# z3lx/waifu2x-tensorrt

Measured on AMD Instinct MI355X. Metric: upscaled MPix/s, 1080p->4K swin_unet/art fp16, higher is better.
Workload: dtype f16; 1 GPU; configs[2]: swin_unet/art scale4 noise3 batch4 tile256 fp16, 1920x1080 frame, blend=0.0625 (45 tiles, 12 batches); synthetic-weight graph of that architecture, frame resident in HBM; frames_per_rank=132, parallelism=frame-sharded x1, no collectives; timing barrier over gloo, mode=frames, tiles_per_network_pass=48, tile_groups_per_pass=2

## Files before the change

include/w2x/c_api.h:

```cpp
#ifndef W2X_C_API_H
#define W2X_C_API_H

#include <stddef.h>
#include <stdint.h>

#ifdef __cplusplus
extern "C" {
#endif

typedef struct w2x_engine w2x_engine;

enum { W2X_PRECISION_TF32 = 0, W2X_PRECISION_FP16 = 1, W2X_PRECISION_FP32 = 2 };

enum { W2X_RESIZE_BICUBIC = 0, W2X_RESIZE_BILINEAR = 1 };
enum { W2X_YUV_BT601 = 0, W2X_YUV_BT709 = 1, W2X_YUV_BT2020 = 2 };
enum { W2X_YUV_LIMITED = 0, W2X_YUV_FULL = 1 };

typedef struct w2x_build_config {
    int deviceId, precision;
    int minBatchSize, optBatchSize, maxBatchSize;
    int minChannels, optChannels, maxChannels;
    int minWidth, optWidth, maxWidth;
    int minHeight, optHeight, maxHeight;
} w2x_build_config;
// ... 20 lines not shown
int w2x_render16_resized(w2x_engine* e, const uint16_t* src, int rows, int cols, size_t src_step, uint16_t* dst, int dst_rows, int dst_cols, size_t dst_step, int filter);
int w2x_render_strip(w2x_engine* e, const uint8_t* src, int rows, int cols, size_t src_step, uint8_t* dst, size_t dst_step, int part, int parts);
int w2x_render_sharded(w2x_engine* const* engines, int count, const uint8_t* src, int rows, int cols, size_t src_step, uint8_t* dst, size_t dst_step);
int w2x_shard_plan(int in_w, int in_h, int out_w, int out_h, int tile_in, int tile_out, int scaling, double overlap_x, double overlap_y,
                   int part, int parts, int* out16);
int w2x_shard_compute(w2x_engine* e, const uint8_t* src, int rows, int cols, size_t src_step, int part, int parts);
const void* w2x_shard_slab(w2x_engine* e, size_t* bytes);
int w2x_shard_finish(w2x_engine* e, uint8_t* dst, int out_rows, int out_cols, size_t dst_step, int part, int parts, const void* const* slabs, const int* devices);
int w2x_ipc_export(const void* device_ptr, uint8_t* out64);
void* w2x_ipc_open(const uint8_t* handle64, int device);
void w2x_ipc_close(void* p);
int w2x_render_sequence(w2x_engine* e, const uint8_t* const* srcs, int rows, int cols, size_t src_step, uint8_t* const* dsts, size_t dst_step, int count);
int w2x_render_sequence_resized(w2x_engine* e, const uint8_t* const* srcs, int rows, int cols, size_t src_step, uint8_t* const* dsts, int dst_rows, int dst_cols, size_t dst_step,
                                int count, int filter);
int w2x_render_yuv(w2x_engine* e, const void* const* src_planes, const size_t* src_steps, int rows, int cols, int src_bits,
                   void* const* dst_planes, const size_t* dst_steps, int dst_rows, int dst_cols, int dst_bits, int matrix, int range);
int w2x_render_sequence_yuv(w2x_engine* e, const void* const* src_planes, const size_t* src_steps, int rows, int cols, int src_bits,
                            void* const* dst_planes, const size_t* dst_steps, int dst_rows, int dst_cols, int dst_bits, int count, int matrix, int range);
int w2x_render_yuv_resized(w2x_engine* e, const void* const* src_planes, const size_t* src_steps, int rows, int cols, int src_bits,
                           void* const* dst_planes, const size_t* dst_steps, int dst_rows, int dst_cols, int dst_bits, int matrix, int range, int filter);
int w2x_render_sequence_yuv_resized(w2x_engine* e, const void* const* src_planes, const size_t* src_steps, int rows, int cols, int src_bits,
                                    void* const* dst_planes, const size_t* dst_steps, int dst_rows, int dst_cols, int dst_bits, int count, int matrix, int range, int filter);
int w2x_render_rgba(w2x_engine* e, const uint8_t* src, int rows, int cols, size_t src_step, uint8_t* dst, size_t dst_step, int bleed, int skip_uniform_alpha);
int w2x_alpha_bleed_device(w2x_engine* e, const uint8_t* bgra, int rows, int cols, size_t bgra_step, uint8_t* bgr, size_t bgr_step, int radius);
void* w2x_alloc_host(w2x_engine* e, size_t bytes);
void w2x_free_host(w2x_engine* e, void* data);
int w2x_pin_host(w2x_engine* e, void* data, size_t bytes);
void w2x_unpin_host(w2x_engine* e, void* data);
int w2x_strip_plan(int in_w, int in_h, int out_w, int out_h, int tile_in, int tile_out, int scaling, double overlap_x, double overlap_y,
                   int part, int parts, int* out4);
int w2x_infer(w2x_engine* e, const float* input_nchw, float* output_nchw);
int w2x_output_tile_size(w2x_engine* e);
double w2x_plan_flops(w2x_engine* e);
int w2x_pass_tiles(w2x_engine* e);
float w2x_last_render_ms(w2x_engine* e);
float w2x_bench_resident(w2x_engine* e, int iters);
int w2x_resident_output(w2x_engine* e, void* dst, size_t bytes);
int w2x_profile_frame(w2x_engine* e, double* out, int cap);
int w2x_op_times(w2x_engine* e, double* out, int cap);

int w2x_calculate_tiles(int in_w, int in_h, int out_w, int out_h, int tile_in, int tile_out, int scaling,
                        double overlap_x, double overlap_y, int* in_rects, int* out_rects, int cap);
int w2x_tile_weights(int which, int overlap_x, int overlap_y, int size, float* out);
int w2x_resize_weights(int in, int out, int filter, int* first, float* weights, int cap);
int w2x_yuv_plane_sizes(int rows, int cols, int bits, int* plane_rows, int* plane_cols, size_t* plane_bytes);
int w2x_alpha_bleed(const uint8_t* bgr, size_t bgr_step, const uint8_t* alpha, size_t alpha_step, int rows, int cols, int radius, uint8_t* out, size_t out_step);
int w2x_describe_plan(const char* onnx_path, int batch, int tile, char* buf, size_t cap);
int w2x_describe_plan_precision(const char* onnx_path, int batch, int tile, int precision, char* buf, size_t cap);
int w2x_write_engine_file(const char* onnx_path, int batch, int tile, const char* out_path);
int w2x_validate_engine_file(const char* path, char* buf, size_t cap);
enum { W2X_EXTENT_INTS = 25 };
int w2x_dead_skip_extents(const char* onnx_path, int batch, int tile, int in_w, int in_h, int scaling, double overlap_x, double overlap_y, int tile_index, int tta,
                          int* out, int cap);
int w2x_device_pci_bus_id(int device, char* buf, size_t cap);
void w2x_sha256_hex(const void* data, size_t len, char* out);
const char* w2x_version(void);
int w2x_debug_set(const char* name, int value);

#ifdef __cplusplus
}
#endif
#endif
```

waifu2x-tensorrt_amd/__init__.py:

```python
from .engine import (BuildConfig, RenderConfig, Img2Img, Precision, Severity, lib, lib_path,
                     calculate_tiles, strip_plan, shard_plan, render_sharded, device_pci_bus_id, ipc_open, ipc_close, tile_weights, resize_weights, yuv_plane_sizes, alpha_bleed, describe_plan, dead_skip_extents, write_engine_file, validate_engine_file, sha256_hex, W2xError,
                     debug_switches)

__all__ = ["BuildConfig", "RenderConfig", "Img2Img", "Precision", "Severity", "lib", "lib_path",
           "calculate_tiles", "strip_plan", "shard_plan", "render_sharded", "device_pci_bus_id", "ipc_open", "ipc_close", "tile_weights", "resize_weights", "yuv_plane_sizes", "alpha_bleed", "describe_plan", "dead_skip_extents", "write_engine_file", "validate_engine_file", "sha256_hex", "W2xError", "debug_switches"]
```

waifu2x-tensorrt_amd/csrc/c_api.cpp:

```cpp
#include "../../include/w2x/c_api.h"
#include <mutex>

#include <cstring>
#include <fstream>
#include <vector>
#include <string>

#include "../../include/w2x/img2img.h"
#include "liveness.h"
#include "lower.h"
#include "sha256.h"
#include "tiles.h"
#include "kernels.h"

struct w2x_engine {
    w2x::Img2Img engine;
    w2x_message_fn msg = nullptr; void* msg_user = nullptr;
    w2x_progress_fn prog = nullptr; void* prog_user = nullptr;
};

extern "C" {

w2x_engine* w2x_create(void) { try { return new w2x_engine; } catch (...) { return nullptr; } }
void w2x_destroy(w2x_engine* e) { delete e; }

void w2x_set_message_callback(w2x_engine* e, w2x_message_fn fn, void* user) {
    if (!e) return;
    e->msg = fn; e->msg_user = user;
    if (fn) e->engine.setMessageCallback([e](w2x::Severity s, const std::string& m) { if (e->msg) e->msg((int)s, m.c_str(), e->msg_user); });
    else e->engine.setMessageCallback(nullptr);
}
void w2x_set_progress_callback(w2x_engine* e, w2x_progress_fn fn, void* user) {
    if (!e) return;
    e->prog = fn; e->prog_user = user;
    if (fn) e->engine.setProgressCallback([e](int c, int t, double s) { if (e->prog) e->prog(c, t, s, e->prog_user); });
    else e->engine.setProgressCallback(nullptr);
}

int w2x_build(w2x_engine* e, const char* onnx_path, const w2x_build_config* c) {
    if (!e || !onnx_path || !c) return 0;
    w2x::BuildConfig b;
    b.deviceId = c->deviceId; b.precision = c->precision == W2X_PRECISION_FP16 ? w2x::Precision::FP16 : c->precision == W2X_PRECISION_FP32 ? w2x::Precision::FP32 : w2x::Precision::TF32;
    b.minBatchSize = c->minBatchSize; b.optBatchSize = c->optBatchSize; b.maxBatchSize = c->maxBatchSize;
    b.minChannels = c->minChannels; b.optChannels = c->optChannels; b.maxChannels = c->maxChannels;
    b.minWidth = c->minWidth; b.optWidth = c->optWidth; b.maxWidth = c->maxWidth;
    b.minHeight = c->minHeight; b.optHeight = c->optHeight; b.maxHeight = c->maxHeight;
    return e->engine.build(onnx_path, b) ? 1 : 0;
}

int w2x_load(w2x_engine* e, const char* onnx_path, const w2x_render_config* c) {
    if (!e || !onnx_path || !c) return 0;
    w2x::RenderConfig r;
    r.deviceId = c->deviceId; r.precision = c->precision == W2X_PRECISION_FP16 ? w2x::Precision::FP16 : c->precision == W2X_PRECISION_FP32 ? w2x::Precision::FP32 : w2x::Precision::TF32;
    r.batchSize = c->batchSize; r.channels = c->channels; r.height = c->height; r.width = c->width; r.scaling = c->scaling;
    r.overlapX = c->overlapX; r.overlapY = c->overlapY; r.tta = c->tta != 0; r.ttaBugCompat = c->ttaBugCompat != 0;
    return e->engine.load(onnx_path, r) ? 1 : 0;
}

int w2x_render(w2x_engine* e, const uint8_t* src, int rows, int cols, size_t src_step, uint8_t* dst, size_t dst_step) {
    if (!e) return 0;
    w2x::Image s; s.data = const_cast<uint8_t*>(src); s.rows = rows; s.cols = cols; s.step = src_step;
    w2x::Image d; d.data = dst; d.step = dst_step;
    const int sc = e->engine.scaling();
    d.rows = rows * sc; d.cols = cols * sc;
    return e->engine.render(s, d) ? 1 : 0;
}
// ... 258 lines not shown
        if (!f.is_open()) return 0;
        f.write((const char*)bytes.data(), (std::streamsize)bytes.size());
        return f.good() ? 1 : 0;
    } catch (const std::exception&) { return 0; }
}

int w2x_device_pci_bus_id(int device, char* buf, size_t cap) { return buf && cap >= 16 && w2x::device_pci_bus_id(device, buf, cap) ? 1 : 0; }

void w2x_sha256_hex(const void* data, size_t len, char* out) {
    std::string h = w2x::sha256_hex(data, len);
    memcpy(out, h.c_str(), 65);
}

const char* w2x_version(void) { return "w2x-hip 0.1 (gfx950)"; }

int w2x_dead_skip_extents(const char* onnx_path, int batch, int tile, int in_w, int in_h, int scaling, double overlap_x, double overlap_y, int tile_index, int tta,
                          int* out, int cap) {
    try {
        static std::mutex mu;
        static std::string key;
        static w2x::Plan plan;
        std::lock_guard<std::mutex> lock(mu);
        const std::string k = std::string(onnx_path ? onnx_path : "") + "|" + std::to_string(batch) + "|" + std::to_string(tile);
        if (k != key) { plan = w2x::build_plan(onnx_path, batch, 3, tile, tile, false); plan.userB = batch; key = k; }
        const int nops = (int)plan.ops.size();
        if (!out || cap < nops * W2X_EXTENT_INTS) return -nops;
        int kept_w = plan.Tout, kept_h = plan.Tout;
        bool all = tta != 0 || tile_index < 0 || w2x::switches().no_dead_skip;
        if (tile_index >= 0) {
            const w2x::TileGrid g = w2x::calculate_tiles(in_w, in_h, in_w * scaling, in_h * scaling, tile, tile, plan.Tout, plan.Tout, scaling, overlap_x, overlap_y);
            if (tile_index >= g.count) return 0;
            kept_w = g.out[tile_index].w; kept_h = g.out[tile_index].h;
        }
        const std::vector<w2x::OpExtent> ext = w2x::dead_skip_extents(plan, kept_w, kept_h, all);
        for (int i = 0; i < nops; ++i) {
            const w2x::Op& op = plan.ops[i]; const w2x::OpExtent& e = ext[i];
            int* o = out + (size_t)i * W2X_EXTENT_INTS;
            int in_t = -1, out_t = -1, res_t = -1, kh = 1, kw = 1, stride = 1, x0 = 0, y0 = 0, r = 1;
            if (op.kind == w2x::OP_GEMM) {
                in_t = op.g.a.t; out_t = op.g.out.t; res_t = op.g.res.t; x0 = op.g.a.x0; y0 = op.g.a.y0;
                if (op.g.amode == w2x::A_CONV) { kh = op.g.kh; kw = op.g.kw; stride = op.g.stride; }
                if (op.g.omode == w2x::O_PIXSHUF) r = op.g.r;
            } else if (op.kind == w2x::OP_MLP) { in_t = op.m.x; out_t = op.m.y; }
            else if (op.kind == w2x::OP_SWINATTN) { in_t = op.sa.x; out_t = op.sa.y; }
            auto dim = [&](int t, bool w) { return t >= 0 && t < (int)plan.tensors.size() ? (w ? plan.tensors[t].W : plan.tensors[t].H) : 0; };
            const int v[W2X_EXTENT_INTS] = {op.kind, e.x.n, e.y.n, e.x.c, e.x.w, e.y.c, e.y.w, e.rx, e.ry, e.ws, in_t, out_t, res_t, kh, kw, stride, x0, y0, r,
                                            dim(in_t, true), dim(in_t, false), dim(out_t, true), dim(out_t, false), (int)e.live_units(), (int)e.total_units()};
            for (int k = 0; k < W2X_EXTENT_INTS; ++k) o[k] = v[k];
        }
        return nops;
    } catch (const std::exception&) { return 0; }
}

int w2x_debug_set(const char* name, int value) { return w2x::set_switch(name, value) ? 1 : 0; }

}
```

waifu2x-tensorrt_amd/csrc/engine.cpp:

```cpp
#include <hip/hip_runtime.h>
#include <dlfcn.h>

#include <algorithm>
#include <array>
#include <chrono>
#include <cmath>
#include <cstdio>
#include <cstdlib>
#include <cstring>
#include <deque>
#include <filesystem>
#include <fstream>
#include <map>
#include <sstream>
#include <tuple>

#include "../../include/w2x/img2img.h"
#include "common.h"
#include "fragorder.h"
#include "kernels.h"
#include "liveness.h"
#include "lower.h"
#include "plan.h"
#include "sha256.h"
#include "switches.h"
#include "tiles.h"

#define W2X_LOG(sev, message) impl->log(sev, message, __FUNCTION__, __LINE__)
#define W2X_LOG_AS(who, sev, message) impl->log(sev, message, who, __LINE__)

namespace w2x {

namespace {

inline void hipAssert(hipError_t e) {
    if (e != hipSuccess) throw std::runtime_error(hipGetErrorString(e));
}

std::string hipGetDeviceName(int deviceId) {
    hipDeviceProp_t prop{};
    hipAssert(hipGetDeviceProperties(&prop, deviceId));
    std::string arch = prop.gcnArchName;
    return arch + " x" + std::to_string(prop.multiProcessorCount);
}

int physical_device(int logical) {
    std::vector<int> map;
    if (const char* e = getenv("W2X_DEVICE_MAP")) { std::stringstream ss(e); std::string tok; while (std::getline(ss, tok, ',')) if (!tok.empty()) map.push_back(atoi(tok.c_str())); }
    return logical >= 0 && logical < (int)map.size() ? map[logical] : logical;
}

struct DeviceGuard {
    int prev = -1, dev = -1;
    explicit DeviceGuard(int d) : dev(d) {
        if (d < 0) return;
        if (hipGetDevice(&prev) != hipSuccess) { (void)hipGetLastError(); prev = -1; }
        if (prev != d) hipAssert(hipSetDevice(d));
    }
    ~DeviceGuard() { if (dev >= 0 && prev >= 0 && prev != dev) (void)hipSetDevice(prev); }
    DeviceGuard(const DeviceGuard&) = delete;
    DeviceGuard& operator=(const DeviceGuard&) = delete;
};

std::string device_ordinal_problem(int logical, int physical) {
    int count = 0;
    if (hipGetDeviceCount(&count) != hipSuccess) { (void)hipGetLastError(); count = 0; }
    if (count <= 0) return "no HIP device is visible to this process (hipGetDeviceCount = 0): this library has no CPU path";
    if (physical >= 0 && physical < count) return "";
    std::string m = "device id " + std::to_string(logical);
    if (physical != logical) m += " (W2X_DEVICE_MAP -> " + std::to_string(physical) + ")";
    return m + " does not exist: this process sees " + std::to_string(count) + " HIP device" + (count == 1 ? "" : "s") + " (valid ids 0.." + std::to_string(count - 1) + ")";
}

}
bool device_pci_bus_id(int deviceId, char* buf, size_t cap) {
    const int dev = physical_device(deviceId);
// ... 101 lines not shown
    void log(Severity s, const std::string& m) { if (messageCallback) messageCallback(s, m); }
    void log(Severity s, const std::string& m, const std::string& fn, int line) { if (messageCallback) messageCallback(s, "[" + fn + "@" + std::to_string(line) + "] " + m); }
    void log(int current, int total, double speed) { if (progressCallback) progressCallback(current, total, speed); }

    bool loaded = false;
    int device = -1;
    bool poison = false;
    bool check_general = false;
    bool use_graphs = true;
    Plan plan;
    RenderConfig cfg;
    hipStream_t stream = nullptr;
    hipEvent_t ev0 = nullptr, ev1 = nullptr;
    int (*roctx_push)(const char*) = nullptr; int (*roctx_pop)() = nullptr;
    hipEvent_t ev_shard = nullptr;
    static constexpr int kMaxRenderParts = 4;
    hipEvent_t ev_part[kMaxRenderParts] = {nullptr, nullptr, nullptr, nullptr};
    int pipeline_parts = 3;
    size_t shard_halo_slots = 0;
    int shard_rows = 0, shard_cols = 0;
    hipStream_t gstream[3] = {nullptr, nullptr, nullptr};
    hipEvent_t ev_fork = nullptr, ev_join[3] = {nullptr, nullptr, nullptr};
    int groups = 2;
    std::vector<void*> tensors, blobs;
    std::vector<void*> frag_blobs;
    std::vector<void*> perm_blobs;
    std::vector<int> pool_blocks;
    void* arena_base = nullptr; size_t arena_bytes = 0;
    std::vector<GemmParams> gemm;
    int final_op = -1;
    enum LaunchKind { L_OP, L_HEAD, L_STEM, L_UP, L_MLP32, L_ATTN32 };
    struct Launch {
        LaunchKind kind = L_OP;
        int first = 0, last = 0;
        int timed = 0;
        double flops = 0;
        int family = 0;
        std::array<void*, 4> planes{{nullptr, nullptr, nullptr, nullptr}};
    };
    std::vector<Launch> launches;

    bool deep = false;
    uint8_t* d_frame = nullptr; size_t frame_cap = 0;
    uint8_t* d_out = nullptr; size_t out_cap = 0;
    void* d_slab = nullptr; size_t slab_cap = 0;
    void* d_slab2 = nullptr; size_t slab2_cap = 0;
    hipEvent_t ev_g0[2] = {nullptr, nullptr}, ev_cmp[2] = {nullptr, nullptr};
    bool rolling = false;
    bool rolling_ok = true;
    TileSlot* d_slots = nullptr; size_t slots_cap = 0;
    LiveExt* d_live = nullptr; size_t live_cap = 0, live_stride = 0;
    std::vector<LiveExt> h_live;
    std::map<std::pair<int, int>, std::vector<OpExtent>> live_cache;
    void upload_live(const TileGrid& grid, size_t count, hipStream_t on) {
        const size_t nops = plan.ops.size();
        if (!count || !nops) return;
        if (count > live_stride) {
            ensure(d_live, live_cap, (nops * count + 8) * sizeof(LiveExt));
            live_stride = count;
        }
        const bool all = switches().no_dead_skip || check_general || cfg.tta;
        std::map<std::pair<int, int>, int> tile_at;
        if (!all) for (int t = 0; t < grid.count; ++t) tile_at[{grid.in[t].x, grid.in[t].y}] = t;
        auto extents = [&](int w, int h) -> const std::vector<OpExtent>& {
            auto it = live_cache.find({w, h});
            if (it == live_cache.end()) it = live_cache.emplace(std::make_pair(w, h), dead_skip_extents(plan, w, h, false)).first;
            return it->second;
        };
        const std::vector<OpExtent>& whole = extents(plan.Tout, plan.Tout);
        h_live.resize(nops * count);
        for (size_t st = 0; st < count; ++st) {
            const TileSlot& sl = h_slots[st];
            const std::vector<OpExtent>* e = &whole;
            if (!all && sl.valid && sl.aug == 0) {
                const auto it = tile_at.find({sl.x, sl.y});
                if (it != tile_at.end()) e = &extents(grid.out[it->second].w, grid.out[it->second].h);
            }
            for (size_t i = 0; i < nops; ++i) {
                const OpExtent& x = (*e)[i];
                auto u16 = [](int v) { return (uint16_t)std::min(std::max(v, 0), 65535); };
                h_live[i * count + st] = x.all() ? LiveExt{65535, 0, 65535, 0} : LiveExt{u16(x.x.c), u16(x.x.w), u16(x.y.c), u16(x.y.w)};
            }
        }
        hipAssert(hipMemcpy2DAsync(d_live, live_stride * sizeof(LiveExt), h_live.data(), count * sizeof(LiveExt), count * sizeof(LiveExt), nops, hipMemcpyHostToDevice, on));
    }
    float *d_rampx = nullptr, *d_rampy = nullptr;
    int ovx = 0, ovy = 0;
    float* d_blob_in = nullptr; float* d_blob_out = nullptr;
    uint8_t* d_frame2 = nullptr; size_t frame2_cap = 0;
    uint8_t* d_out2 = nullptr; size_t out2_cap = 0;
    hipStream_t s_up = nullptr, s_dn = nullptr;
    hipEvent_t ev_up[2] = {nullptr, nullptr}, ev_comp[2] = {nullptr, nullptr}, ev_dn[2] = {nullptr, nullptr};
    float* d_canvas = nullptr; size_t canvas_cap = 0;
    struct ResizeTables {
        int inW = 0, inH = 0, outW = 0, outH = 0, filter = 0;
        int *fx = nullptr, *fy = nullptr; float *wx = nullptr, *wy = nullptr;
        int kx = 0, ky = 0, rows_max = 0;
    };
    std::deque<ResizeTables> rs_tables;
    const ResizeTables* rs = nullptr;
    struct YuvJob { YuvCoefs in, out; int in_bits = 8, out_bits = 8, key = 0; };
    const YuvJob* yuv = nullptr;
    uint8_t* d_bgr = nullptr; size_t bgr_cap = 0;
    uint8_t* d_alpha = nullptr; size_t alpha_cap = 0;
    unsigned* d_minmax = nullptr; unsigned* h_minmax = nullptr;
    hipEvent_t ev_minmax = nullptr;
    bool rgba = false;
    std::vector<void*> pinned;
    std::vector<void*> host_allocs;
    std::vector<TileSlot> h_slots;

    bool profiling = false;
    struct Stamp { int kind; hipEvent_t a, b; double flops; int op; };
    std::vector<double> op_ms;
    std::vector<Stamp> stamps;
    void stamp_begin(int kind, double flops, int op = -1) {
        if (!profiling) return;
        Stamp st{kind, nullptr, nullptr, flops, op};
        hipAssert(hipEventCreate(&st.a)); hipAssert(hipEventCreate(&st.b));
        hipAssert(hipEventRecord(st.a, stream));
        stamps.push_back(st);
    }
    void stamp_end() { if (profiling) hipAssert(hipEventRecord(stamps.back().b, stream)); }

    void ensure_copy_streams() {
        if (s_up) return;
        hipAssert(hipStreamCreateWithFlags(&s_up, hipStreamNonBlocking));
        hipAssert(hipStreamCreateWithFlags(&s_dn, hipStreamNonBlocking));
        for (int b = 0; b < 2; ++b) { hipAssert(hipEventCreateWithFlags(&ev_up[b], hipEventDisableTiming)); hipAssert(hipEventCreateWithFlags(&ev_comp[b], hipEventDisableTiming)); hipAssert(hipEventCreateWithFlags(&ev_dn[b], hipEventDisableTiming)); }
    }

    bool one_part_stale = false;
    void one_part_slots() {
        if (!one_part_stale) return;
        const int steps = cfg.tta ? 8 : 1, B = plan.B, S = plan.B / plan.userB;
        const int batchCount = (int)std::lround(std::ceil((double)(last_strip.tile_count * steps) / plan.userB));
        const size_t stepCount = (size_t)((batchCount + S - 1) / S) * B;
        h_slots.resize(stepCount);
        for (size_t st = 0; st < stepCount; ++st) {
            const int ti = (int)(st / steps), aug = (int)(st % steps);
            TileSlot sl{0, 0, aug, 0};
            if (ti < last_strip.tile_count) { sl.x = last_grid.in[last_strip.first_tile + ti].x; sl.y = last_grid.in[last_strip.first_tile + ti].y; sl.valid = 1; }
            h_slots[st] = sl;
        }
        ensure(d_slots, slots_cap, stepCount * sizeof(TileSlot));
        hipAssert(hipMemcpy(d_slots, h_slots.data(), stepCount * sizeof(TileSlot), hipMemcpyHostToDevice));
        upload_live(last_grid, stepCount, stream);
        hipAssert(hipStreamSynchronize(stream));
        ensure(d_slab, slab_cap, stepCount * plan.Tout * plan.Tout * 4 * plan.elt);
        one_part_stale = false;
    }
    int last_rows = 0, last_cols = 0, last_batches = 0;
    TileGrid last_grid;
    StripPlan last_strip;
    float last_ms = 0.f;

    static constexpr int kRgbaKey = 64;
    using GraphKey = std::tuple<const void*, const void*, const void*, const void*, int, int, int, int>;
    struct PassGraphs { hipGraphExec_t g[4] = {nullptr, nullptr, nullptr, nullptr}; int n = 0; };
    std::map<GraphKey, PassGraphs> graphs;
    std::map<GraphKey, int> graph_seen;
    long graph_replays = 0, eager_passes = 0;
    void drop_graphs() {
        for (auto& kv : graphs) for (int k = 0; k < kv.second.n; ++k) if (kv.second.g[k]) (void)hipGraphExecDestroy(kv.second.g[k]);
        graphs.clear(); graph_seen.clear();
    }

    ~Impl() {
        release();
        for (void* h : host_allocs) if (hipHostFree(h) != hipSuccess) (void)hipGetLastError();
    }

    void release() {
        std::unique_ptr<DeviceGuard> guard;
        if (device >= 0) { try { guard.reset(new DeviceGuard(device)); } catch (...) {} }
        drop_graphs();
        if (arena_base) { (void)hipFree(arena_base); arena_base = nullptr; }
        for (void* p : blobs) if (p) (void)hipFree(p);
        for (void* p : frag_blobs) if (p) (void)hipFree(p);
        frag_blobs.clear();
        for (void* p : perm_blobs) if (p) (void)hipFree(p);
        perm_blobs.clear();
        for (const Launch& L : launches) for (void* p : L.planes) if (p) (void)hipFree(p);
        launches.clear();
        tensors.clear(); blobs.clear(); gemm.clear();
        for (void* h : pinned) if (hipHostUnregister(h) != hipSuccess) (void)hipGetLastError();
        pinned.clear();
        for (hipEvent_t* e : {&ev_up[0], &ev_up[1], &ev_comp[0], &ev_comp[1], &ev_dn[0], &ev_dn[1]}) if (*e) { (void)hipEventDestroy(*e); *e = nullptr; }
        if (s_up) { (void)hipStreamDestroy(s_up); s_up = nullptr; }
        if (s_dn) { (void)hipStreamDestroy(s_dn); s_dn = nullptr; }
        frame2_cap = out2_cap = 0;
        for (ResizeTables& t : rs_tables) for (void* q : {(void*)t.fx, (void*)t.fy, (void*)t.wx, (void*)t.wy}) if (q) (void)hipFree(q);
        rs_tables.clear(); rs = nullptr;
        if (d_canvas) { (void)hipFree(d_canvas); d_canvas = nullptr; }
        canvas_cap = 0;
        for (void** q : {(void**)&d_bgr, (void**)&d_alpha, (void**)&d_minmax}) if (*q) { (void)hipFree(*q); *q = nullptr; }
        bgr_cap = alpha_cap = 0; rgba = false;
        if (h_minmax) { if (hipHostFree(h_minmax) != hipSuccess) (void)hipGetLastError(); h_minmax = nullptr; }
        if (ev_minmax) { (void)hipEventDestroy(ev_minmax); ev_minmax = nullptr; }
        for (void** p : {(void**)&d_frame, (void**)&d_out, (void**)&d_frame2, (void**)&d_out2, &d_slab, &d_slab2, (void**)&d_slots, (void**)&d_live, (void**)&d_rampx, (void**)&d_rampy, (void**)&d_blob_in, (void**)&d_blob_out})
            if (*p) { (void)hipFree(*p); *p = nullptr; }
        frame_cap = out_cap = slab_cap = slab2_cap = slots_cap = 0;
        live_cap = live_stride = 0; live_cache.clear();
        shard_rows = shard_cols = 0; shard_halo_slots = 0; rolling = false; one_part_stale = false;
        last_rows = last_cols = last_batches = 0;
        if (ev0) { (void)hipEventDestroy(ev0); ev0 = nullptr; }
        if (ev1) { (void)hipEventDestroy(ev1); ev1 = nullptr; }
        if (ev_shard) { (void)hipEventDestroy(ev_shard); ev_shard = nullptr; }
        for (hipEvent_t& e : ev_part) if (e) { (void)hipEventDestroy(e); e = nullptr; }
        for (hipEvent_t& e : ev_g0) if (e) { (void)hipEventDestroy(e); e = nullptr; }
        for (hipEvent_t& e : ev_cmp) if (e) { (void)hipEventDestroy(e); e = nullptr; }
        if (ev_fork) { (void)hipEventDestroy(ev_fork); ev_fork = nullptr; }
        for (hipEvent_t& e : ev_join) if (e) { (void)hipEventDestroy(e); e = nullptr; }
        for (hipStream_t& st : gstream) if (st) { (void)hipStreamDestroy(st); st = nullptr; }
        if (stream) { (void)hipStreamDestroy(stream); stream = nullptr; }
        loaded = false;
    }

    TView tview(const View& v) const {
        TView t;
        if (v.t < 0) return t;
        const TensorDesc& d = plan.tensors[v.t];
        t.p = tensors[v.t]; t.Hs = d.H; t.Ws = d.W; t.Cs = d.C; t.y0 = v.y0; t.x0 = v.x0;
        return t;
    }

    struct TensorUse { std::array<int, 6> rd; std::array<int, 3> wr; };
    static TensorUse tensor_use(const Op& op) {
        TensorUse u; u.rd.fill(-1); u.wr.fill(-1);
        switch (op.kind) {
            case OP_GEMM: u.rd = {{op.g.a.t, op.g.res.t, op.g.res2.t, op.g.stats_in, op.g.se_scale, op.g.res_scale}}; u.wr = {{op.g.out.t, op.g.stats_out, op.g.pool_out}}; break;
            case OP_ATTN: u.rd[0] = op.at.qkv; u.wr[0] = op.at.out; break;
            case OP_SE: u.rd[0] = op.se.pool; u.wr[0] = op.se.scale; break;
            case OP_SCALE_ADD: u.rd = {{op.se.pool, op.se.scale, -1, -1, -1, -1}}; u.wr[0] = op.se.pool; break;
            case OP_MLP: u.rd[0] = op.m.x; u.wr = {{op.m.y, op.m.stats_out, -1}}; break;
            case OP_SWINATTN: u.rd[0] = op.sa.x; u.wr = {{op.sa.y, op.sa.stats_out, -1}}; break;
            default: break;
        }
        return u;
    }
    struct Lifetimes { std::vector<int> first, last; };
    Lifetimes lifetimes(const std::vector<Launch>& ls) const {
        const int nops = (int)plan.ops.size();
        Lifetimes lt{std::vector<int>(plan.tensors.size(), nops), std::vector<int>(plan.tensors.size(), -1)};
        for (const Launch& L : ls)
            for (int i = L.first; i <= L.last; ++i) {
                const TensorUse u = tensor_use(plan.ops[i]);
                auto touch = [&](int t) { if (t >= 0) { lt.first[t] = std::min(lt.first[t], L.first); lt.last[t] = std::max(lt.last[t], L.last); } };
                for (int t : u.rd) touch(t);
                for (int t : u.wr) touch(t);
            }
        lt.first[plan.in_tensor] = -1;
        lt.last[plan.out_tensor] = nops;
        return lt;
    }
    static bool passes_on(const Lifetimes& lt, int t, int i) { return t >= 0 && lt.first[t] == i && lt.last[t] == i + 1; }
// ... 216 lines not shown
        }
        if (final_op < 0) throw std::runtime_error("plan: the output tensor is not produced by a fused op");
        auto head_supported = [&](const GemmParams& g) {
            return g.wt_frag && g.out.Cs == 4 && g.a.y0 == 0 && g.a.x0 == 0 && g.a.Ws == g.aW && (long)g.a.Hs * g.a.Ws == g.Mrows && g.Mrows % 32 == 0 && g.aW >= 32 && pixgemm_supported(g) &&
                   (!g.has_clip || (f16_to_f32(f32_to_f16(g.clip_lo)) == g.clip_lo && f16_to_f32(f32_to_f16(g.clip_hi)) == g.clip_hi));
        };
        launches.clear();
        for (const Launch& L : candidates) {
            const GemmParams& p = gemm[L.last]; const GemmParams& q = gemm[L.first];
            const bool ok = L.kind == L_HEAD ? head_supported(p) : L.kind == L_STEM ? conv48_stem_supported(p, q) || conv3_stem_supported(p, q) : L.kind == L_UP ? conv3_up_supported(p, q) : true;
            if (ok) launches.push_back(L);
            else for (int i = L.first; i <= L.last; ++i) launches.push_back(launch(L_OP, i, i));
        }
        for (Launch& L : launches)
            if (L.kind == L_MLP32 || L.kind == L_ATTN32) {
                const GemmOp& g1 = plan.ops[L.first].g; const GemmOp& g2 = plan.ops[L.last].g;
                upload_planes(plan.blobs[g1.w].data, g1.N, g1.K, L.planes[0], L.planes[1]);
                upload_planes(plan.blobs[g2.w].data, g2.N, g2.K, L.planes[2], L.planes[3]);
            }
        hipAssert(hipStreamSynchronize(stream));
    }

    int ng_now = 1;
    size_t arena_part() const { return ((arena_bytes / ng_now) + 255) / 256 * 256; }
    uint8_t* group_ptr(const void* full, int grp) const {
        return full ? (uint8_t*)arena_base + (size_t)grp * arena_part() + (size_t)((const uint8_t*)full - (const uint8_t*)arena_base) / ng_now : nullptr;
    }
    void run_network(void* out_override, int live = -1, int grp = -1, hipStream_t s = nullptr, const LiveExt* ext = nullptr) {
        if (!s) s = stream;
        const int cap = grp < 0 ? plan.B : plan.B / ng_now;
        if (live < 0 || live > cap) live = cap;
        auto tp = [&](int t) -> uint8_t* { return t < 0 ? nullptr : grp < 0 ? (uint8_t*)tensors[t] : group_ptr(tensors[t], grp); };
        auto lv = [&](int i) -> const LiveExt* { return ext ? ext + (size_t)i * live_stride : nullptr; };
        auto gp = [&](int i) {
            GemmParams p = gemm[i];
            p.B = live;
            if (grp >= 0) {
                auto shift = [&](auto*& ptr) { ptr = (std::remove_reference_t<decltype(ptr)>)group_ptr(ptr, grp); };
                shift(p.a.p); shift(p.res.p); shift(p.res2.p); shift(p.out.p); shift(p.stats_in); shift(p.stats_out); shift(p.pool_out); shift(p.a_scale); shift(p.res_scale);
            }
            if (i == final_op && out_override) p.out.p = out_override;
            return p;
        };
        for (const Launch& L : launches) try {
            const Op& op = plan.ops[L.first];
            struct Range { Impl* e; bool on; ~Range() { if (on) e->roctx_pop(); } } range{this, roctx_push != nullptr};
            if (range.on) roctx_push(launch_label(L).c_str());
            auto issue = [&](auto&& f) { stamp_begin(L.family, L.flops, L.timed); hipAssert(f()); stamp_end(); };
            switch (L.kind) {
                case L_HEAD: {
                    const GemmParams g = gp(L.last);
                    MlpParams p = mlp_params(op, live, tp);
                    p.live = lv(L.last);
                    p.ti_w = g.wt_frag; p.ti_b = g.bias; p.ti_out = g.out.p; p.ti_Hs = g.out.Hs; p.ti_Ws = g.out.Ws; p.ti_Mrows = g.Mrows; p.ti_aW = g.aW;
                    p.ti_clip = g.has_clip; p.ti_lo = g.clip_lo; p.ti_hi = g.clip_hi;
                    issue([&] { return launch_mlp(p, s); });
                    break;
                }
                case L_STEM: case L_UP: {
                    const GemmParams p = gp(L.last), q = gp(L.first);
                    issue([&] { return L.kind == L_UP ? launch_conv3_up(p, q, s) : q.N == 48 ? launch_conv48_stem(p, q, s) : launch_conv3_stem(p, q, s); });
                    break;
                }
                case L_MLP32: {
                    const GemmParams p = gp(L.first), q = gp(L.last);
                    Mlp32Params m;
                    m.x = (const float*)p.a.p; m.y = (float*)q.out.p; m.M = (long)live * p.Mrows; m.C = p.K; m.stats_in = p.stats_in;
                    m.w1h = L.planes[0]; m.w1l = L.planes[1]; m.w2h = L.planes[2]; m.w2l = L.planes[3];
                    m.b1 = p.bias; m.b2 = q.bias; m.stats_out = q.stats_out; m.eps_out = q.ln_eps;
                    issue([&] { return launch_mlp32(m, s); });
                    break;
                }
                case L_ATTN32: {
                    const GemmParams p = gp(L.first), q = gp(L.last);
                    const AttnOp& a = plan.ops[L.first + 1].at;
                    SwinAttn32Params m;
                    m.x = (const float*)p.a.p; m.y = (float*)q.out.p; m.res = (const float*)q.res.p; m.B = live; m.nwin = a.nwin; m.C = p.K; m.pix_per_item = p.Mrows;
                    m.table_in = p.win_table; m.table_out = q.win_table; m.stats_in = p.stats_in;
                    m.wqkv_h = L.planes[0]; m.wqkv_l = L.planes[1]; m.wproj_h = L.planes[2]; m.wproj_l = L.planes[3];
                    m.bqkv = p.bias; m.bproj = q.bias; m.scale = a.scale; m.bias = (const float*)blobs[a.bias]; m.maskid = (const int*)blobs[a.maskid];
                    m.stats_out = q.stats_out; m.eps_out = q.ln_eps;
                    issue([&] { return launch_swinattn32(m, s); });
                    break;
                }
                case L_OP: switch (op.kind) {
                    case OP_GEMM: {
                        const GemmParams p = gp(L.first);
                        if (op.g.pool_out >= 0) pool_blocks[op.g.pool_out] = plan.elt == 2 && conv3_supported(p) ? conv3_tiles(p) : 0;
                        issue([&] { return plan.elt == 4 ? launch_gemm_f32(p, s, cfg.precision == Precision::FP32) : pixgemm_supported(p) ? launch_pixgemm(p, s) : conv3_supported(p) ? launch_conv3(p, s) : conv3h_supported(p) ? launch_conv3h(p, s) : conv48_supported(p) ? launch_conv48(p, s) : stem_supported(p) ? launch_stem(p, s) : launch_gemm(p, s); });
                        if (check_general && plan.elt == 2 && (pixgemm_supported(p) || conv3_supported(p) || conv3h_supported(p) || conv48_supported(p) || stem_supported(p))) check_against_general(p, L.first, live);
                        break;
                    }
                    case OP_ATTN: {
                        const AttnOp& a = op.at;
                        AttnParams p;
                        p.qkv = tp(a.qkv); p.out = tp(a.out); p.B = live; p.nwin = a.nwin; p.heads = a.heads; p.hd = a.hd;
                        p.ntok = a.ws * a.ws; p.scale = a.scale; p.bias = blobs[a.bias]; p.maskid = (const int*)blobs[a.maskid];
                        issue([&] { return plan.elt == 4 ? launch_attn_f32(p, s) : launch_attn(p, s); });
                        break;
                    }
                    case OP_SWINATTN: {
                        const SwinAttnOp& a = op.sa;
                        const TensorDesc& d = plan.tensors[a.x];
                        SwinAttnParams p;
                        p.x = tp(a.x); p.y = tp(a.y); p.table = (const int*)blobs[a.table]; p.H = a.H; p.W = a.W; p.ry = a.ry; p.rx = a.rx; p.B = live; p.nwin = a.nwin; p.C = a.C; p.hd = a.hd;
                        p.wqkv = blobs[a.wqkv]; p.bqkv = (const float*)blobs[a.bqkv]; p.scale = a.scale; p.bias32 = (const float*)blobs[a.bias]; p.maskid = (const int*)blobs[a.maskid];
// ... 50 lines not shown
        return p;
    }
    void check_against_general(const GemmParams& p, int i, int live) {
        const Op& op = plan.ops[i];
        const TensorDesc& od = plan.tensors[op.g.out.t];
        const size_t n = (size_t)live * od.H * od.W * od.C;
        std::vector<uint16_t> a(n), b(n);
        void* tmp = nullptr;
        hipAssert(hipMalloc(&tmp, n * 2));
        hipAssert(hipStreamSynchronize(stream));
        hipAssert(hipMemcpy(a.data(), p.out.p, n * 2, hipMemcpyDeviceToHost));
        hipAssert(hipMemcpy(tmp, p.out.p, n * 2, hipMemcpyDeviceToDevice));
        GemmParams q = p; q.out.p = tmp; q.pool_out = nullptr;
        hipAssert(launch_gemm(q, stream));
        hipAssert(hipStreamSynchronize(stream));
        hipAssert(hipMemcpy(b.data(), tmp, n * 2, hipMemcpyDeviceToHost));
        hipAssert(hipFree(tmp));
        double md = 0; size_t at = 0, bad = 0;
        for (size_t k = 0; k < n; ++k) { const double d = std::fabs(f16_to_f32(a[k]) - f16_to_f32(b[k])); if (d > 0.01) ++bad; if (d > md) { md = d; at = k; } }
        log(Severity::warn, "pixgemm check op " + std::to_string(i) + " [" + op.name + "]: max|d|=" + std::to_string(md) + " at pixel " + std::to_string(at / od.C) +
            " ch " + std::to_string(at % od.C) + " (x=" + std::to_string(at / od.C % od.W) + ", y=" + std::to_string(at / od.C / od.W % od.H) + "), " + std::to_string(bad) + " of " + std::to_string(n) + " off by > 0.01");
    }

    template <class T> void ensure(T*& p, size_t& cap, size_t bytes) {
        if (bytes <= cap) return;
        drop_graphs();
        if (p) hipAssert(hipFree(p));
        p = nullptr; cap = 0;
        hipAssert(hipMalloc((void**)&p, bytes));
        cap = bytes;
    }

    void run_frame(int rows, int cols, const TileGrid& grid, bool report, const StripPlan& sp) {
        run_passes(rows, cols, sp.tile_count, 0, report, 0, true);
        if (rs) { compose_canvas(rows, cols, grid, stream); if (yuv) resample_yuv(stream); else resample(stream); return; }
        if (yuv) { compose_yuv(rows, cols, grid, stream); return; }
        compose_rect(rows, cols, grid, sp.x0, sp.x1, 0, 0, sp.first_tile);
    }

    bool can_roll(int tile_count) const {
        const int steps = cfg.tta ? 8 : 1, B = plan.B;
        const int last_live = tile_count * steps - (tile_count * steps - 1) / B * B;
        return rolling_ok && groups == 2 && use_graphs && !profiling && !check_general && !poison && gstream[0] && last_live >= 8 && B % 2 == 0;
    }
    void run_rolling_frame(int rows, int cols, const TileGrid& grid, const StripPlan& sp, int which, hipEvent_t out_free) {
        for (int k = 0; k < 2; ++k) {
            if (!ev_g0[k]) hipAssert(hipEventCreateWithFlags(&ev_g0[k], hipEventDisableTiming));
            if (!ev_cmp[k]) hipAssert(hipEventCreateWithFlags(&ev_cmp[k], hipEventDisableTiming));
        }
        struct Swap { Impl* e; void* slab; size_t cap; bool on; ~Swap() { if (on) { std::swap(e->d_slab, e->d_slab2); std::swap(e->slab_cap, e->slab2_cap); } e->rolling = false; } } sw{this, d_slab, slab_cap, which == 1};
        if (which == 1) { std::swap(d_slab, d_slab2); std::swap(slab_cap, slab2_cap); }
        rolling = true;
        hipAssert(hipStreamWaitEvent(stream, ev_cmp[which], 0));
        run_passes(rows, cols, sp.tile_count, 0, false, 0, true);
        hipAssert(hipEventRecord(ev_g0[which], stream));
        hipStream_t s2 = gstream[0];
        hipAssert(hipStreamWaitEvent(s2, ev_g0[which], 0));
        if (rs) {
            compose_canvas(rows, cols, grid, s2);
            hipAssert(hipEventRecord(ev_cmp[which], s2));
            if (out_free) hipAssert(hipStreamWaitEvent(s2, out_free, 0));
            if (yuv) resample_yuv(s2); else resample(s2);
            return;
        }
        if (out_free) hipAssert(hipStreamWaitEvent(s2, out_free, 0));
        if (yuv) compose_yuv(rows, cols, grid, s2);
        else compose_rect(rows, cols, grid, sp.x0, sp.x1, 0, 0, sp.first_tile, s2);
        hipAssert(hipEventRecord(ev_cmp[which], s2));
    }
    void end_rolling() { hipAssert(hipEventRecord(ev_join[0], gstream[0])); hipAssert(hipStreamWaitEvent(stream, ev_join[0], 0)); }
    void drain_after_error() {
        rolling = false;
        for (hipStream_t st : {s_up, s_dn, gstream[0], stream}) if (st && hipStreamSynchronize(st) != hipSuccess) (void)hipGetLastError();
    }

    void run_passes(int rows, int cols, int tile_count, size_t slab_slot0, bool report, size_t slots_off, bool fresh, int batch0 = 0, int batch_total = 0, int pass0 = 0, int pass1 = -1) {
        const int B = plan.B, T = plan.T, To = plan.Tout;
        const int steps = cfg.tta ? 8 : 1;
        const int userB = plan.userB, S = B / userB;
        const int batchCount = (int)std::lround(std::ceil((double)(tile_count * steps) / userB));
        const int passCount = (batchCount + S - 1) / S;
        const size_t slot_bytes = (size_t)To * To * 4 * plan.elt;
        if (poison && fresh) {
            hipAssert(hipMemsetAsync(arena_base, 0x7E, arena_bytes, stream));
            hipAssert(hipMemsetAsync(d_slab, 0x7E, slab_cap, stream));
        }
        const bool graphable = use_graphs && !profiling && !check_general;
        for (int bi = pass0; bi < (pass1 < 0 ? passCount : std::min(pass1, passCount)); ++bi) {
            const auto t0 = std::chrono::steady_clock::now();
            const int live = std::max(0, std::min(B, tile_count * steps - bi * B));
            void* const slab_out = (uint8_t*)d_slab + (slab_slot0 + (size_t)bi * B) * slot_bytes;
            GatherParams gp0;
            gp0.frame = d_frame; gp0.rows = rows; gp0.cols = cols; gp0.step = (size_t)cols * 3 * (deep ? 2 : 1); gp0.deep = deep ? 1 : 0;
            gp0.out = tensors[plan.in_tensor]; gp0.slots = d_slots + slots_off + (size_t)bi * B; gp0.B = B; gp0.T = T; gp0.fp32 = plan.elt == 4;
            const int NG = groups;
            struct NgReset { int& r; ~NgReset() { r = 1; } } ng_reset{ng_now};
            ng_now = NG;
            const bool split = NG > 1 && !profiling && !check_general && live >= 4 * NG && B % NG == 0 && (size_t)NG * arena_part() <= arena_bytes + 1024;
            ng_now = 1;
            int first[5] = {0, 0, 0, 0, 0};
            for (int grp = 0; grp < NG; ++grp) first[grp + 1] = first[grp] + live / NG + (grp < live % NG ? 1 : 0);
            if (split) {
                if (!ev_fork) hipAssert(hipEventCreateWithFlags(&ev_fork, hipEventDisableTiming));
                for (int k = 0; k + 1 < NG; ++k) if (!gstream[k]) {
                    hipAssert(hipStreamCreateWithFlags(&gstream[k], hipStreamNonBlocking));
                    hipAssert(hipEventCreateWithFlags(&ev_join[k], hipEventDisableTiming));
                }
            }
            auto group_stream = [&](int grp) { return grp ? gstream[grp - 1] : stream; };
            auto gather = [&](const GatherParams& gp, hipStream_t gs) {
                if (rgba) {
                    GatherRgbaParams rp;
                    rp.bgr = d_bgr; rp.bgr_step = (size_t)cols * 3; rp.alpha = d_alpha; rp.alpha_step = (size_t)cols; rp.rows = rows; rp.cols = cols;
                    rp.out = gp.out; rp.fp32 = gp.fp32; rp.slots = gp.slots; rp.B = gp.B; rp.T = gp.T;
                    hipAssert(launch_gather_rgba(rp, gs));
                    return;
                }
                if (!yuv) { hipAssert(launch_gather(gp, gs)); return; }
                GatherYuvParams yp;
                yp.src = yuv_layout(d_frame, rows, cols, yuv->in_bits); yp.k = yuv->in;
                yp.out = gp.out; yp.fp32 = gp.fp32; yp.slots = gp.slots; yp.B = gp.B; yp.T = gp.T;
                hipAssert(launch_gather_yuv(yp, gs));
            };
            auto gather_group = [&](int grp, hipStream_t gs) {
                GatherParams gp = gp0;
                gp.out = group_ptr(tensors[plan.in_tensor], grp); gp.slots = gp0.slots + (size_t)first[grp]; gp.B = first[grp + 1] - first[grp];
                gather(gp, gs);
            };
            const LiveExt* const ext0 = d_live && slots_off + (size_t)(bi + 1) * B <= live_stride ? d_live + slots_off + (size_t)bi * B : nullptr;
            auto network_group = [&](int grp, hipStream_t gs) { run_network((uint8_t*)slab_out + (size_t)first[grp] * slot_bytes, first[grp + 1] - first[grp], grp, gs, ext0 ? ext0 + first[grp] : nullptr); };
            auto fork = [&] { hipAssert(hipEventRecord(ev_fork, stream)); for (int grp = 1; grp < NG; ++grp) hipAssert(hipStreamWaitEvent(gstream[grp - 1], ev_fork, 0)); };
            auto join = [&] { for (int grp = 1; grp < NG; ++grp) { hipAssert(hipEventRecord(ev_join[grp - 1], gstream[grp - 1])); hipAssert(hipStreamWaitEvent(stream, ev_join[grp - 1], 0)); } };
            auto run_pass = [&] {
                if (!split) {
                    stamp_begin(3, 0);
                    gather(gp0, stream);
                    stamp_end();
                    run_network(slab_out, live, -1, nullptr, ext0);
                    return;
                }
                ng_now = NG;
                for (int grp = 0; grp < NG; ++grp) gather_group(grp, stream);
                fork();
                for (int grp = 0; grp < NG; ++grp) network_group(grp, group_stream(grp));
                join();
                ng_now = 1;
            };
            auto run_group = [&](int grp) { ng_now = NG; gather_group(grp, group_stream(grp)); network_group(grp, group_stream(grp)); ng_now = 1; };
            const bool per_group = split;
            const bool no_join = rolling && split;
            auto run_eager = [&] { if (per_group) { fork(); for (int grp = 0; grp < NG; ++grp) run_group(grp); if (!no_join) join(); } else { if (rolling && gstream[0]) { join(); } run_pass(); } };
            if (!graphable) run_eager();
            else {
                const GraphKey key{d_frame, d_slots + slots_off + (size_t)bi * B, slab_out, arena_base, rows, cols, live, rgba ? kRgbaKey : yuv ? yuv->key : deep ? 1 : 0};
                auto replay = [&](const PassGraphs& pg) {
                    if (pg.n == 1) { if (rolling && gstream[0]) join(); hipAssert(hipGraphLaunch(pg.g[0], stream)); return; }
                    fork();
                    for (int grp = 0; grp < pg.n; ++grp) hipAssert(hipGraphLaunch(pg.g[grp], group_stream(grp)));
                    if (!no_join) join();
                };
                auto it = graphs.find(key);
                if (it != graphs.end()) { replay(it->second); ++graph_replays; }
                else if (graph_seen.size() >= 4096 && !graph_seen.count(key)) { graph_seen.clear(); run_eager(); ++eager_passes; }
                else if (graph_seen[key]++ == 0 && !(rolling && !graphs.empty())) { run_eager(); ++eager_passes; }
                else {
                    if (graphs.size() >= 1024) drop_graphs();
                    PassGraphs pg;
                    std::string why;
                    const int ncap = per_group ? NG : 1;
                    for (int c = 0; c < ncap && why.empty(); ++c) {
                        hipStream_t cs = per_group ? group_stream(c) : stream;
                        hipGraph_t graph = nullptr; hipGraphExec_t exec = nullptr;
                        hipError_t ge = hipStreamBeginCapture(cs, hipStreamCaptureModeThreadLocal);
                        if (ge != hipSuccess) { why = std::string("begin capture: ") + hipGetErrorString(ge); break; }
                        try { if (per_group) run_group(c); else run_pass(); } catch (const std::exception& e) { why = std::string("capture: ") + e.what(); }
                        ge = hipStreamEndCapture(cs, &graph);
                        if (why.empty() && ge != hipSuccess) why = std::string("end capture: ") + hipGetErrorString(ge);
                        if (why.empty()) { ge = hipGraphInstantiate(&exec, graph, nullptr, nullptr, 0); if (ge != hipSuccess) why = std::string("instantiation: ") + hipGetErrorString(ge); }
                        if (graph) (void)hipGraphDestroy(graph);
                        if (why.empty()) pg.g[pg.n++] = exec;
                    }
                    if (!why.empty()) {
                        (void)hipGetLastError();
                        for (int c = 0; c < pg.n; ++c) (void)hipGraphExecDestroy(pg.g[c]);
                        use_graphs = false;
                        log(Severity::warn, "hipGraph " + why + " - passes stay on plain launches");
                        run_eager(); ++eager_passes;
                    } else {
                        graphs[key] = pg;
                        replay(pg); ++graph_replays;
                    }
                }
            }
            if (report) {
                const auto t1 = std::chrono::steady_clock::now();
                const double ms = std::chrono::duration<double, std::milli>(t1 - t0).count();
                for (int k = bi * S; k < std::min((bi + 1) * S, batchCount); ++k)
                    log(batch0 + k + 1, batch_total > 0 ? batch_total : batchCount, 1000.0 * S / std::max(ms, 1e-6));
            }
        }
        last_batches = batch0 + batchCount;
    }

    void compose_rect(int rows, int cols, const TileGrid& grid, int x0, int x1, int y0, int y1, long first_tile, hipStream_t on = nullptr) {
        const int To = plan.Tout;
        ComposeParams cp;
        cp.tiles = d_slab; cp.fp32 = plan.elt == 4; cp.dst = d_out; cp.dst_step = (size_t)cols * cfg.scaling * 3 * (deep ? 2 : 1); cp.deep = deep ? 1 : 0;
        cp.outW = cols * cfg.scaling; cp.outH = rows * cfg.scaling; cp.To = To;
        cp.nx = grid.nx; cp.ny = grid.ny; cp.stride_x = To - grid.outOvX; cp.stride_y = To - grid.outOvY;
        const bool overlapping = cfg.overlapX != 0 || cfg.overlapY != 0;
        cp.ovx = overlapping ? ovx : 0; cp.ovy = overlapping ? ovy : 0;
        cp.ramp_x = d_rampx; cp.ramp_y = d_rampy; cp.tta = cfg.tta ? 1 : 0; cp.tta_bug_compat = cfg.ttaBugCompat ? 1 : 0;
        cp.x0 = x0; cp.x1 = x1; cp.y0 = y0; cp.y1 = y1; cp.first_tile = first_tile;
        stamp_begin(4, 0);
        hipAssert(launch_compose(cp, on ? on : stream));
        stamp_end();
    }

    void compose_canvas(int rows, int cols, const TileGrid& grid, hipStream_t on) {
        const int To = plan.Tout;
        ComposeParams cp;
        cp.tiles = d_slab; cp.fp32 = plan.elt == 4;
        cp.outW = cols * cfg.scaling; cp.outH = rows * cfg.scaling; cp.To = To;
        cp.nx = grid.nx; cp.ny = grid.ny; cp.stride_x = To - grid.outOvX; cp.stride_y = To - grid.outOvY;
        const bool overlapping = cfg.overlapX != 0 || cfg.overlapY != 0;
        cp.ovx = overlapping ? ovx : 0; cp.ovy = overlapping ? ovy : 0;
        cp.ramp_x = d_rampx; cp.ramp_y = d_rampy; cp.tta = cfg.tta ? 1 : 0; cp.tta_bug_compat = cfg.ttaBugCompat ? 1 : 0;
        hipAssert(launch_compose_canvas(cp, d_canvas, on));
    }
    void compose_yuv(int rows, int cols, const TileGrid& grid, hipStream_t on) {
        const int To = plan.Tout;
        ComposeYuvParams yp;
        ComposeParams& cp = yp.c;
        cp.tiles = d_slab; cp.fp32 = plan.elt == 4;
        cp.outW = cols * cfg.scaling; cp.outH = rows * cfg.scaling; cp.To = To;
        cp.nx = grid.nx; cp.ny = grid.ny; cp.stride_x = To - grid.outOvX; cp.stride_y = To - grid.outOvY;
        const bool overlapping = cfg.overlapX != 0 || cfg.overlapY != 0;
        cp.ovx = overlapping ? ovx : 0; cp.ovy = overlapping ? ovy : 0;
        cp.ramp_x = d_rampx; cp.ramp_y = d_rampy; cp.tta = cfg.tta ? 1 : 0; cp.tta_bug_compat = cfg.ttaBugCompat ? 1 : 0;
        yp.dst = yuv_layout(d_out, cp.outH, cp.outW, yuv->out_bits); yp.k = yuv->out;
        stamp_begin(4, 0);
        hipAssert(launch_compose_yuv(yp, on));
        stamp_end();
    }
    void upload_and_bleed(const Image& src, int radius) {
        const int rows = src.rows, cols = src.cols;
        ensure(d_frame, frame_cap, (size_t)rows * cols * 4);
        ensure(d_bgr, bgr_cap, (size_t)rows * cols * 3);
        ensure(d_alpha, alpha_cap, (size_t)rows * cols);
        if (!d_minmax) hipAssert(hipMalloc((void**)&d_minmax, 2 * sizeof(unsigned)));
        hipAssert(hipMemcpy2DAsync(d_frame, (size_t)cols * 4, src.data, src.step, (size_t)cols * 4, rows, hipMemcpyHostToDevice, stream));
        hipAssert(hipMemsetAsync(d_minmax, 0, 2 * sizeof(unsigned), stream));
        AlphaBleedParams bp;
        bp.bgra = d_frame; bp.step = (size_t)cols * 4; bp.rows = rows; bp.cols = cols; bp.radius = radius;
        bp.bgr = d_bgr; bp.bgr_step = (size_t)cols * 3; bp.alpha = d_alpha; bp.alpha_step = (size_t)cols; bp.minmax = d_minmax;
        hipAssert(launch_alpha_bleed(bp, stream));
    }
    void compose_rgba(int rows, int cols, const TileGrid& grid, size_t alpha_slot0, bool uniform, unsigned value) {
        const int To = plan.Tout;
        ComposeRgbaParams rp;
        ComposeParams& cp = rp.c;
        cp.tiles = d_slab; cp.fp32 = plan.elt == 4; cp.dst = d_out; cp.dst_step = (size_t)cols * cfg.scaling * 4;
        cp.outW = cols * cfg.scaling; cp.outH = rows * cfg.scaling; cp.To = To;
        cp.nx = grid.nx; cp.ny = grid.ny; cp.stride_x = To - grid.outOvX; cp.stride_y = To - grid.outOvY;
        const bool overlapping = cfg.overlapX != 0 || cfg.overlapY != 0;
        cp.ovx = overlapping ? ovx : 0; cp.ovy = overlapping ? ovy : 0;
        cp.ramp_x = d_rampx; cp.ramp_y = d_rampy; cp.tta = cfg.tta ? 1 : 0; cp.tta_bug_compat = cfg.ttaBugCompat ? 1 : 0;
        rp.alpha_tiles = uniform ? nullptr : (const uint8_t*)d_slab + alpha_slot0 * (size_t)To * To * 4 * plan.elt;
        rp.alpha_value = value;
        hipAssert(launch_compose_rgba(rp, stream));
    }
    void sequence_slots(const TileGrid& grid, const StripPlan& sp) {
        const int steps = cfg.tta ? 8 : 1, B = plan.B, S = plan.B / plan.userB;
        const int batchCount = (int)std::lround(std::ceil((double)(sp.tile_count * steps) / plan.userB));
        const int stepCount = ((batchCount + S - 1) / S) * B;
        h_slots.resize(stepCount);
        for (int st = 0; st < stepCount; ++st) {
            int ti = st / steps, aug = st % steps;
            TileSlot sl{0, 0, aug, 0};
            if (ti < sp.tile_count) { sl.x = grid.in[ti].x; sl.y = grid.in[ti].y; sl.valid = 1; }
            h_slots[st] = sl;
        }
        ensure(d_slots, slots_cap, (size_t)stepCount * sizeof(TileSlot));
        hipAssert(hipMemcpyAsync(d_slots, h_slots.data(), (size_t)stepCount * sizeof(TileSlot), hipMemcpyHostToDevice, stream));
        upload_live(grid, (size_t)stepCount, stream);
        ensure(d_slab, slab_cap, (size_t)stepCount * plan.Tout * plan.Tout * 4 * plan.elt);
        hipAssert(hipStreamSynchronize(stream));
    }
    template <class Up, class Down>
    float run_sequence(int count, int rows, int cols, const TileGrid& grid, const StripPlan& sp, const Up& up, const Down& down) {
        uint8_t* const frames[2] = {d_frame, d_frame2};
        uint8_t* const outs[2] = {d_out, d_out2};
        struct Restore { Impl* im; uint8_t* f; uint8_t* o; ~Restore() { im->d_frame = f; im->d_out = o; } } restore{this, frames[0], outs[0]};
        const bool roll = count > 1 && can_roll(sp.tile_count);
        if (roll) ensure(d_slab2, slab2_cap, slab_cap);
        hipAssert(hipStreamSynchronize(stream));
        hipAssert(hipEventRecord(ev0, stream));
        for (int i = 0; i < count; ++i) {
            const int b = i & 1;
            if (i >= 2) hipAssert(hipStreamWaitEvent(s_up, ev_comp[b], 0));
            up(i, frames[b], s_up);
            hipAssert(hipEventRecord(ev_up[b], s_up));
            hipAssert(hipStreamWaitEvent(stream, ev_up[b], 0));
            d_frame = frames[b]; d_out = outs[b];
            if (roll) {
                run_rolling_frame(rows, cols, grid, sp, b, i >= 2 ? ev_dn[b] : nullptr);
                hipAssert(hipEventRecord(ev_comp[b], gstream[0]));
            } else {
                if (i >= 2) hipAssert(hipStreamWaitEvent(stream, ev_dn[b], 0));
                run_frame(rows, cols, grid, false, sp);
                hipAssert(hipEventRecord(ev_comp[b], stream));
            }
            hipAssert(hipStreamWaitEvent(s_dn, ev_comp[b], 0));
            down(i, outs[b], s_dn);
            hipAssert(hipEventRecord(ev_dn[b], s_dn));
        }
        if (roll) end_rolling();
        hipAssert(hipEventRecord(ev1, stream));
        hipAssert(hipStreamSynchronize(s_dn));
        hipAssert(hipStreamSynchronize(stream));
        hipAssert(hipStreamSynchronize(s_up));
        float total_ms = 0.f;
        hipAssert(hipEventElapsedTime(&total_ms, ev0, ev1));
        return total_ms;
    }
    static YuvPlanes yuv_layout(uint8_t* base, int rows, int cols, int bits) {
        const size_t bps = bits > 8 ? 2 : 1;
        const int cw = (cols + 1) / 2, ch = (rows + 1) / 2;
        YuvPlanes f;
        f.rows = rows; f.cols = cols; f.bits = bits;
        f.step[0] = ((size_t)cols * bps + 15) / 16 * 16; f.step[1] = f.step[2] = ((size_t)cw * bps + 15) / 16 * 16;
        f.p[0] = base; f.p[1] = base + f.step[0] * rows; f.p[2] = f.p[1] + f.step[1] * ch;
        return f;
    }
    static size_t yuv_bytes(int rows, int cols, int bits) { const YuvPlanes f = yuv_layout(nullptr, rows, cols, bits); return f.step[0] * rows + 2 * f.step[1] * ((rows + 1) / 2); }
    void resample(hipStream_t on) {
        ResampleParams rp;
        rp.canvas = d_canvas; rp.inW = rs->inW; rp.inH = rs->inH;
        rp.dst = d_out; rp.dst_step = (size_t)rs->outW * 3 * (deep ? 2 : 1); rp.deep = deep ? 1 : 0;
        rp.outW = rs->outW; rp.outH = rs->outH;
        rp.fx = rs->fx; rp.wx = rs->wx; rp.kx = rs->kx; rp.fy = rs->fy; rp.wy = rs->wy; rp.ky = rs->ky; rp.rows_max = rs->rows_max;
        hipAssert(launch_resample(rp, on));
    }
    void resample_yuv(hipStream_t on) {
        ResampleYuvParams rp;
        rp.canvas = d_canvas; rp.inW = rs->inW; rp.inH = rs->inH;
        rp.outW = rs->outW; rp.outH = rs->outH;
        rp.fx = rs->fx; rp.wx = rs->wx; rp.kx = rs->kx; rp.fy = rs->fy; rp.wy = rs->wy; rp.ky = rs->ky; rp.rows_max = rs->rows_max;
        rp.dst = yuv_layout(d_out, rs->outH, rs->outW, yuv->out_bits); rp.k = yuv->out;
        hipAssert(launch_resample_yuv(rp, on));
    }
    const ResizeTables* resize_tables(int inW, int inH, int outW, int outH, int filter) {
        for (const ResizeTables& t : rs_tables) if (t.inW == inW && t.inH == inH && t.outW == outW && t.outH == outH && t.filter == filter) return &t;
        if (rs_tables.size() >= 16) {
            for (ResizeTables& t : rs_tables) for (void* q : {(void*)t.fx, (void*)t.fy, (void*)t.wx, (void*)t.wy}) if (q) hipAssert(hipFree(q));
            rs_tables.clear();
        }
// ... 138 lines not shown
    impl->poison = sw.poison;
    impl->check_general = sw.check_general;
    impl->use_graphs = !sw.no_graph;
    impl->rolling_ok = !sw.no_rolling;
    impl->pipeline_parts = std::min(Impl::kMaxRenderParts, std::max(1, sw.render_parts));
    if (const std::string nd = switches_nondefault(); !nd.empty()) W2X_LOG(warn, "Switches off their defaults: " + nd + ".");
    if (sw.roctx && !impl->roctx_push) {
        if (void* h = dlopen("libroctx64.so", RTLD_NOW | RTLD_GLOBAL)) {
            impl->roctx_push = (int (*)(const char*))dlsym(h, "roctxRangePushA");
            impl->roctx_pop = (int (*)())dlsym(h, "roctxRangePop");
            if (!impl->roctx_push || !impl->roctx_pop) impl->roctx_push = nullptr;
        }
        if (!impl->roctx_push) W2X_LOG(warn, "W2X_ROCTX is set but libroctx64.so could not be loaded: no marker ranges.");
    }
    try {
        impl->plan = Plan::deserialize((const uint8_t*)engineBuffer.data(), engineBuffer.size());
    } catch (const std::exception& e) {
        W2X_LOG(error, "Failed to deserialize engine from buffer: " + std::string(e.what()) + ".");
        return false;
    }
    if (!optimized) {
        W2X_LOG(warn, "Engine \"" + enginePath + "\" is compatible with but not optimized for the render configuration; specialising the plan for batch " +
                          std::to_string(config.batchSize) + ", tile " + std::to_string(config.width) + "x" + std::to_string(config.height) + ".");
        try {
            impl->plan = lower_for_shape(modelPath, config.batchSize, config.channels, config.height, config.width, config.precision != Precision::FP16);
        } catch (const std::exception& e) {
            W2X_LOG(error, "Failed to set input tensor shape: " + std::string(e.what()) + ".");
            return false;
        }
    }
    const Plan& plan = impl->plan;
    if ((plan.elt == 4) != (config.precision != Precision::FP16)) {
        W2X_LOG(error, "Failed to deserialize engine from buffer: precision of the plan differs from the engine's configuration.");
        return false;
    }
    if (plan.userB != config.batchSize || plan.B % std::max(plan.userB, 1) || plan.Cin != config.channels || plan.T != config.height || plan.T != config.width) {
        W2X_LOG(error, "Failed to set input tensor shape.");
        return false;
    }
    hipAssert(hipStreamCreateWithFlags(&impl->stream, hipStreamNonBlocking));
    hipAssert(hipEventCreate(&impl->ev0));
    hipAssert(hipEventCreate(&impl->ev1));
    impl->groups = sw.groups;
    impl->ensure_copy_streams();
    if (impl->groups > 1) { hipAssert(hipStreamCreateWithFlags(&impl->gstream[0], hipStreamNonBlocking)); hipAssert(hipEventCreateWithFlags(&impl->ev_join[0], hipEventDisableTiming)); }
    try {
        impl->upload_plan(config.precision);
    } catch (const std::exception& e) {
        W2X_LOG(error, "Failed to allocate resources: " + std::string(e.what()) + ".");
        impl->release();
        return false;
    }
    impl->cfg = config;
    int folds[Impl::L_ATTN32 + 1] = {};
    for (const Impl::Launch& L : impl->launches) ++folds[L.kind];
    W2X_LOG(info, "Loaded \"" + enginePath + "\": " + std::to_string(plan.ops.size()) + " ops, " + std::to_string(plan.B) + " tiles per pass, activation arena " +
                      std::to_string(impl->arena_bytes >> 20) + " MiB" +
                      (folds[Impl::L_STEM] ? ", " + std::to_string(folds[Impl::L_STEM]) + " stem folded into the launch of the convolution behind it" : "") +
                      (folds[Impl::L_UP] ? ", " + std::to_string(folds[Impl::L_UP]) + " transposed convolution folded into the launch of the convolution behind it" : "") +
                      (folds[Impl::L_HEAD] ? ", image head folded into the last MLP launch" : "") +
                      (folds[Impl::L_ATTN32] + folds[Impl::L_MLP32] ? ", " + std::to_string(folds[Impl::L_ATTN32]) + " attention and " + std::to_string(folds[Impl::L_MLP32]) + " MLP branches as fused fp32-row launches." : "."));
    impl->ovx = (int)std::lround(plan.T * config.scaling * config.overlapX);
    impl->ovy = (int)std::lround(plan.T * config.scaling * config.overlapY);
    if (config.overlapX != 0 || config.overlapY != 0) {
        auto rx = blend_ramp(impl->ovx), ry = blend_ramp(impl->ovy);
        hipAssert(hipMalloc((void**)&impl->d_rampx, std::max<size_t>(rx.size(), 1) * sizeof(float)));
        hipAssert(hipMalloc((void**)&impl->d_rampy, std::max<size_t>(ry.size(), 1) * sizeof(float)));
        hipAssert(hipMemcpy(impl->d_rampx, rx.data(), rx.size() * sizeof(float), hipMemcpyHostToDevice));
        hipAssert(hipMemcpy(impl->d_rampy, ry.data(), ry.size() * sizeof(float), hipMemcpyHostToDevice));
    }
    impl->loaded = true;
    return true;
} catch (const std::exception& e) {
    W2X_LOG(error, "Engine load failed unexpectedly: " + std::string(e.what()) + ".");
    impl->release();
    return false;
}

bool Img2Img::render(const Image& src, Image& dst) { return renderPart(src, dst, 0, 1, "render"); }

bool Img2Img::renderResized(const Image& src, Image& dst, ResizeFilter filter) {
    return renderPart(src, dst, 0, 1, "renderResized", filter == ResizeFilter::Bilinear ? 1 : 0);
}

bool Img2Img::renderStrip(const Image& src, Image& dst, int part, int parts) { return renderPart(src, dst, part, parts, "renderStrip"); }

bool Img2Img::renderPart(const Image& src, Image& dst, int part, int parts, const char* who, int resizeFilter) try {
    if (!impl->loaded) { W2X_LOG_AS(who, error, "Render called before a successful load."); return false; }
    DeviceGuard guard(impl->device);
    if (parts <= 0 || part < 0 || part >= parts) { W2X_LOG_AS(who, error, "Invalid strip index."); return false; }
    const RenderConfig& cfg = impl->cfg;
    const Plan& plan = impl->plan;
    const int rows = src.rows, cols = src.cols, s = cfg.scaling;
    if ((src.depth != 8 && src.depth != 16) || dst.depth != src.depth) { W2X_LOG_AS(who, error, "Input and output images must both be 8-bit or both 16-bit."); return false; }
    const size_t bps = src.depth / 8;
    if (!src.data || rows <= 0 || cols <= 0 || src.step < (size_t)cols * 3 * bps) { W2X_LOG_AS(who, error, "Input image is empty or has an invalid step."); return false; }
    const bool resized = resizeFilter >= 0 && !(dst.rows == rows * s && dst.cols == cols * s);
    if (resized) {
        const std::string why = impl->resize_problem(src, dst, resizeFilter);
        if (!why.empty()) { W2X_LOG_AS(who, error, why); return false; }
        if (!dst.data || dst.step < (size_t)dst.cols * 3 * bps) { W2X_LOG_AS(who, error, "Output image is empty or has an invalid step."); return false; }
    } else if (!dst.data || dst.rows != rows * s || dst.cols != cols * s || dst.step < (size_t)dst.cols * 3 * bps) {
        W2X_LOG_AS(who, error, "Output image has invalid size: expected " + std::to_string(cols * s) + "x" + std::to_string(rows * s) + ".");
        return false;
    }
    hipStream_t stream = impl->stream;
// ... 5 lines not shown
        impl->ensure_canvas((size_t)rows * s * cols * s * 3 * sizeof(float));
    }
    impl->deep = bps == 2;
    TileGrid grid = calculate_tiles(cols, rows, cols * s, rows * s, plan.T, plan.T, plan.Tout, plan.Tout, s, cfg.overlapX, cfg.overlapY);
    if (grid.count <= 0) { W2X_LOG_AS(who, error, "Tile grid is empty."); return false; }
    for (const Rect& r : grid.out) if (r.w <= 0 || r.h <= 0) { W2X_LOG_AS(who, error, "Tile grid does not fit the output (scaling does not match the model)."); return false; }
    const StripPlan sp = strip_plan(grid, cols * s, plan.Tout, part, parts);
    if (sp.tile_count == 0) return true;
    const int steps = cfg.tta ? 8 : 1, B = plan.B, S = plan.B / plan.userB;
    constexpr int kMaxParts = Impl::kMaxRenderParts;
    int npart = 1;
    int first_of[kMaxParts + 1] = {0, sp.tile_count, 0, 0, 0};
    if (parts == 1 && !resized && impl->pipeline_parts > 1 && sp.tile_count >= 16 && grid.outOvX < plan.Tout - grid.outOvX && grid.outOvY < plan.Tout - grid.outOvY) {
        int q = 1; while ((q * steps) % plan.userB) ++q;
        const int want = std::min({impl->pipeline_parts, kMaxParts, sp.tile_count / 8});
        int n = 0;
        const int body = want >= 2 ? (sp.tile_count - std::max(8, sp.tile_count / 5)) / q * q : 0;
        for (int k = 1; k < want; ++k) {
            const int t = k + 1 == want ? body : (int)((long)k * body / (want - 1)) / q * q;
            if (t > first_of[n] && t < sp.tile_count) first_of[++n] = t;
        }
        first_of[++n] = sp.tile_count;
        npart = n;
    }
    int tiles_of[kMaxParts] = {}, batches_of[kMaxParts] = {}, batches_before[kMaxParts] = {};
    size_t slots_off[kMaxParts] = {}; size_t stepTotal = 0; int batch_total = 0;
    for (int k = 0; k < npart; ++k) {
        tiles_of[k] = first_of[k + 1] - first_of[k];
        batches_of[k] = (int)std::lround(std::ceil((double)(tiles_of[k] * steps) / plan.userB));
        batches_before[k] = batch_total; batch_total += batches_of[k];
        slots_off[k] = stepTotal;
        stepTotal += (size_t)((batches_of[k] + S - 1) / S) * B;
    }
    int x_split = cols;
    if (npart > 1) {
        int xm = 0;
        for (int t = 0; t < first_of[1]; ++t) xm = std::max(xm, grid.in[sp.first_tile + t].x + plan.T);
        if (xm > 0 && xm < cols - 64) x_split = xm;
    }
    hipAssert(hipMemcpy2DAsync(impl->d_frame, (size_t)cols * 3 * bps, src.data, src.step, (size_t)x_split * 3 * bps, rows, hipMemcpyHostToDevice, stream));
    impl->h_slots.resize(stepTotal);
    for (int k = 0; k < npart; ++k) {
        const int t0 = first_of[k];
        const size_t n = (k + 1 < npart ? slots_off[k + 1] : stepTotal) - slots_off[k];
        for (size_t st = 0; st < n; ++st) {
            const int ti = (int)(st / steps), aug = (int)(st % steps);
            TileSlot sl{0, 0, aug, 0};
            if (ti < tiles_of[k]) { sl.x = grid.in[sp.first_tile + t0 + ti].x; sl.y = grid.in[sp.first_tile + t0 + ti].y; sl.valid = 1; }
            impl->h_slots[slots_off[k] + st] = sl;
        }
    }
    impl->ensure(impl->d_slots, impl->slots_cap, stepTotal * sizeof(TileSlot));
    hipAssert(hipMemcpyAsync(impl->d_slots, impl->h_slots.data(), stepTotal * sizeof(TileSlot), hipMemcpyHostToDevice, stream));
    impl->upload_live(grid, stepTotal, stream);
    const size_t one_part_steps = (size_t)(((int)std::lround(std::ceil((double)(sp.tile_count * steps) / plan.userB)) + S - 1) / S) * B;
    impl->ensure(impl->d_slab, impl->slab_cap, std::max((size_t)first_of[npart - 1] * steps + (stepTotal - slots_off[npart - 1]), one_part_steps) * plan.Tout * plan.Tout * 4 * plan.elt);

    hipAssert(hipEventRecord(impl->ev0, stream));
    if (npart == 1) {
        impl->run_frame(rows, cols, grid, true, sp);
        hipAssert(hipEventRecord(impl->ev1, stream));
        const int dx0 = resized ? 0 : sp.x0, dx1 = resized ? dst.cols : sp.x1;
        hipAssert(hipMemcpy2DAsync(dst.data + (size_t)dx0 * 3 * bps, dst.step, impl->d_out + (size_t)dx0 * 3 * bps, (size_t)dst.cols * 3 * bps, (size_t)(dx1 - dx0) * 3 * bps, dst.rows, hipMemcpyDeviceToHost, stream));
        hipAssert(hipStreamSynchronize(stream));
    } else {
        impl->ensure_copy_streams();
        for (int k = 0; k < npart; ++k) if (!impl->ev_part[k]) hipAssert(hipEventCreateWithFlags(&impl->ev_part[k], hipEventDisableTiming));
        ShardPlan part_plan[kMaxParts];
        for (int k = 0; k < npart; ++k) {
            ShardPlan q; q.first_tile = first_of[k]; q.tile_count = tiles_of[k];
            const int sx = plan.Tout - grid.outOvX, sy = plan.Tout - grid.outOvY;
            auto x_of = [&](int i) { return i >= grid.nx ? cols * s : i * sx; };
            auto y_of = [&](int j) { return j >= grid.ny ? rows * s : j * sy; };
            auto add = [&](int i0, int i1, int j0, int j1) { if (i0 < i1 && j0 < j1) q.rect[q.nrect++] = Rect{x_of(i0), y_of(j0), x_of(i1) - x_of(i0), y_of(j1) - y_of(j0)}; };
            const int t0 = q.first_tile, t1 = t0 + q.tile_count;
            const int c0 = t0 / grid.ny, r0 = t0 % grid.ny, c1 = t1 / grid.ny, r1 = t1 % grid.ny;
            if (c0 == c1) add(c0, c0 + 1, r0, r1);
            else { int full0 = c0; if (r0) { add(c0, c0 + 1, r0, grid.ny); full0 = c0 + 1; } add(full0, c1, 0, grid.ny); if (r1) add(c1, c1 + 1, 0, r1); }
            part_plan[k] = q;
        }
        hipStream_t dn = impl->s_up;
        auto download_part = [&](int k) {
            hipAssert(hipStreamWaitEvent(dn, impl->ev_part[k], 0));
            for (int r = 0; r < part_plan[k].nrect; ++r) {
                const Rect& rc = part_plan[k].rect[r];
                hipAssert(hipMemcpy2DAsync(dst.data + (size_t)rc.y * dst.step + (size_t)rc.x * 3 * bps, dst.step, impl->d_out + ((size_t)rc.y * dst.cols + rc.x) * 3 * bps, (size_t)dst.cols * 3 * bps,
                                           (size_t)rc.w * 3 * bps, rc.h, hipMemcpyDeviceToHost, dn));
            }
        };
        bool roll = true;
        for (int k = 0; k < npart; ++k) roll = roll && impl->can_roll(tiles_of[k]);
        struct Unroll { Impl* e; ~Unroll() { e->rolling = false; } } unroll{impl.get()};
        if (roll) for (int k = 0; k < 2; ++k) if (!impl->ev_g0[k]) hipAssert(hipEventCreateWithFlags(&impl->ev_g0[k], hipEventDisableTiming));
        for (int k = 0; k < npart; ++k) {
            if (k == 1 && x_split < cols) hipAssert(hipStreamWaitEvent(stream, impl->ev_up[0], 0));
            impl->rolling = roll;
            impl->run_passes(rows, cols, tiles_of[k], (size_t)first_of[k] * steps, true, slots_off[k], k == 0, batches_before[k], batch_total);
            impl->rolling = false;
            if (k == 0 && x_split < cols) {
                hipAssert(hipMemcpy2DAsync(impl->d_frame + (size_t)x_split * 3 * bps, (size_t)cols * 3 * bps, src.data + (size_t)x_split * 3 * bps, src.step, (size_t)(cols - x_split) * 3 * bps, rows,
                                           hipMemcpyHostToDevice, impl->s_dn));
                hipAssert(hipEventRecord(impl->ev_up[0], impl->s_dn));
            }
            hipStream_t cs = stream;
            if (roll) {
                cs = impl->gstream[0];
                hipAssert(hipEventRecord(impl->ev_g0[k & 1], stream));
// ... 231 lines not shown

bool ipc_export(const void* device_ptr, uint8_t out[64]) {
    static_assert(sizeof(hipIpcMemHandle_t) <= 64, "handle size");
    hipIpcMemHandle_t h;
    if (!device_ptr || hipIpcGetMemHandle(&h, const_cast<void*>(device_ptr)) != hipSuccess) { (void)hipGetLastError(); return false; }
    memset(out, 0, 64); memcpy(out, &h, sizeof(h));
    return true;
}
void* ipc_open(const uint8_t handle[64], int deviceId) {
    const int dev = physical_device(deviceId);
    if (!device_ordinal_problem(deviceId, dev).empty()) return nullptr;
    DeviceGuard guard(dev);
    hipIpcMemHandle_t h; memcpy(&h, handle, sizeof(h));
    void* p = nullptr;
    if (hipIpcOpenMemHandle(&p, h, hipIpcMemLazyEnablePeerAccess) != hipSuccess) { (void)hipGetLastError(); return nullptr; }
    return p;
}
void ipc_close(void* p) { if (p && hipIpcCloseMemHandle(p) != hipSuccess) (void)hipGetLastError(); }

bool Img2Img::renderSequence(const Image* srcs, Image* dsts, int count) { return runSequence(srcs, dsts, count, -1, "renderSequence"); }

bool Img2Img::renderSequenceResized(const Image* srcs, Image* dsts, int count, ResizeFilter filter) {
    return runSequence(srcs, dsts, count, filter == ResizeFilter::Bilinear ? 1 : 0, "renderSequenceResized");
}

bool Img2Img::runSequence(const Image* srcs, Image* dsts, int count, int resizeFilter, const char* who) try {
    if (!impl->loaded) { W2X_LOG_AS(who, error, "Render called before a successful load."); return false; }
    if (count <= 0) return true;
    DeviceGuard guard(impl->device);
    const RenderConfig& cfg = impl->cfg;
    const Plan& plan = impl->plan;
    const int rows = srcs[0].rows, cols = srcs[0].cols, s = cfg.scaling;
    for (int i = 0; i < count; ++i) if (srcs[i].depth != 8 || dsts[i].depth != 8) { W2X_LOG_AS(who, error, std::string(who) + " takes 8-bit frames (16-bit images go through render())."); return false; }
    const int out_rows = resizeFilter >= 0 ? dsts[0].rows : rows * s, out_cols = resizeFilter >= 0 ? dsts[0].cols : cols * s;
    const bool resized = resizeFilter >= 0 && !(out_rows == rows * s && out_cols == cols * s);
    if (resized) {
        const std::string why = impl->resize_problem(srcs[0], dsts[0], resizeFilter);
        if (!why.empty()) { W2X_LOG_AS(who, error, why); return false; }
    }
    impl->deep = false;
    for (int i = 0; i < count; ++i) {
        if (!srcs[i].data || srcs[i].rows != rows || srcs[i].cols != cols || srcs[i].step < (size_t)cols * 3 || rows <= 0 || cols <= 0) { W2X_LOG_AS(who, error, "Input images must be non-empty and of one size."); return false; }
        if (!dsts[i].data || dsts[i].rows != out_rows || dsts[i].cols != out_cols || dsts[i].step < (size_t)out_cols * 3) { W2X_LOG_AS(who, error, "Output image has invalid size: expected " + std::to_string(out_cols) + "x" + std::to_string(out_rows) + "."); return false; }
    }
    hipStream_t stream = impl->stream;
    impl->ensure_copy_streams();
    const size_t in_bytes = (size_t)rows * cols * 3, out_bytes = (size_t)out_rows * out_cols * 3;
    impl->ensure(impl->d_frame, impl->frame_cap, in_bytes);   impl->ensure(impl->d_frame2, impl->frame2_cap, in_bytes);
    impl->ensure(impl->d_out, impl->out_cap, out_bytes);      impl->ensure(impl->d_out2, impl->out2_cap, out_bytes);
    TileGrid grid = calculate_tiles(cols, rows, cols * s, rows * s, plan.T, plan.T, plan.Tout, plan.Tout, s, cfg.overlapX, cfg.overlapY);
    if (grid.count <= 0) { W2X_LOG_AS(who, error, "Tile grid is empty."); return false; }
    for (const Rect& r : grid.out) if (r.w <= 0 || r.h <= 0) { W2X_LOG_AS(who, error, "Tile grid does not fit the output (scaling does not match the model)."); return false; }
    const StripPlan sp = strip_plan(grid, cols * s, plan.Tout, 0, 1);
    impl->sequence_slots(grid, sp);

    struct ResizeScope { Img2Img::Impl* e; ~ResizeScope() { e->rs = nullptr; } } resize_scope{impl.get()};
    if (resized) {
        impl->rs = impl->resize_tables(cols * s, rows * s, out_cols, out_rows, resizeFilter);
        impl->ensure_canvas((size_t)rows * s * cols * s * 3 * sizeof(float));
    }
    const float total_ms = impl->run_sequence(count, rows, cols, grid, sp,
        [&](int i, uint8_t* dev, hipStream_t on) { hipAssert(hipMemcpy2DAsync(dev, (size_t)cols * 3, srcs[i].data, srcs[i].step, (size_t)cols * 3, rows, hipMemcpyHostToDevice, on)); },
        [&](int i, uint8_t* dev, hipStream_t on) { hipAssert(hipMemcpy2DAsync(dsts[i].data, dsts[i].step, dev, (size_t)out_cols * 3, (size_t)out_cols * 3, out_rows, hipMemcpyDeviceToHost, on)); });
    impl->last_ms = total_ms / count;
    impl->last_rows = rows; impl->last_cols = cols; impl->last_grid = grid; impl->last_strip = sp;
    if (resized) impl->last_rows = impl->last_cols = 0;
    return true;
} catch (const std::exception& e) {
    impl->drain_after_error();
    W2X_LOG_AS(who, error, "Render failed unexpectedly: " + std::string(e.what()) + ".");
    return false;
}

bool Img2Img::renderYuv(const YuvImage& src, YuvImage& dst, YuvFormat format) { return runSequenceYuv(&src, &dst, 1, format, -1, "renderYuv"); }

bool Img2Img::renderSequenceYuv(const YuvImage* srcs, YuvImage* dsts, int count, YuvFormat format) {
    return runSequenceYuv(srcs, dsts, count, format, -1, "renderSequenceYuv");
}

bool Img2Img::renderYuvResized(const YuvImage& src, YuvImage& dst, YuvFormat format, ResizeFilter filter) {
    return runSequenceYuv(&src, &dst, 1, format, filter == ResizeFilter::Bilinear ? 1 : filter == ResizeFilter::Bicubic ? 0 : 2, "renderYuvResized");
}

bool Img2Img::renderSequenceYuvResized(const YuvImage* srcs, YuvImage* dsts, int count, YuvFormat format, ResizeFilter filter) {
    return runSequenceYuv(srcs, dsts, count, format, filter == ResizeFilter::Bilinear ? 1 : filter == ResizeFilter::Bicubic ? 0 : 2, "renderSequenceYuvResized");
}

bool Img2Img::runSequenceYuv(const YuvImage* srcs, YuvImage* dsts, int count, YuvFormat format, int resizeFilter, const char* who) try {
    if (!impl->loaded) { W2X_LOG_AS(who, error, "Render called before a successful load."); return false; }
    if (count <= 0) return true;
    if (!srcs || !dsts) { W2X_LOG_AS(who, error, "No frames given."); return false; }
    DeviceGuard guard(impl->device);
    const RenderConfig& cfg = impl->cfg;
    const Plan& plan = impl->plan;
    const int matrix = (int)format.matrix, range = (int)format.range;
    if (matrix < 0 || matrix > 2) { W2X_LOG_AS(who, error, "Unknown YUV matrix " + std::to_string(matrix) + "."); return false; }
    if (range < 0 || range > 1) { W2X_LOG_AS(who, error, "Unknown YUV range " + std::to_string(range) + "."); return false; }
    const int rows = srcs[0].rows, cols = srcs[0].cols, s = cfg.scaling, in_bits = srcs[0].bits, out_bits = dsts[0].bits;
    if ((in_bits != 8 && in_bits != 10) || (out_bits != 8 && out_bits != 10)) { W2X_LOG_AS(who, error, "YUV frames must have 8 or 10 bits."); return false; }
    if (rows <= 0 || cols <= 0) { W2X_LOG_AS(who, error, "Input image is empty."); return false; }
    const int out_rows = resizeFilter >= 0 ? dsts[0].rows : rows * s, out_cols = resizeFilter >= 0 ? dsts[0].cols : cols * s;
    const bool resized = resizeFilter >= 0 && !(out_rows == rows * s && out_cols == cols * s);
    if (resizeFilter >= 0) {
        const std::string why = impl->resize_problem(rows, cols, out_rows, out_cols, resizeFilter);
        if (!why.empty()) { W2X_LOG_AS(who, error, why); return false; }
    }
    auto planes_ok = [](const YuvImage& f) {
// ... 281 lines not shown
```

waifu2x-tensorrt_amd/csrc/k_mlp96q.hip:

```cpp
#include "kernels.h"
#ifndef W2X_GELU_DEG
#define W2X_GELU_DEG 4
#endif

#include <algorithm>

#ifndef W2X_MLP_EXP
#define W2X_MLP_EXP 0
#endif
#ifndef W2X_MLP_PREFETCH
#define W2X_MLP_PREFETCH 1
#endif
#ifndef W2X_MLP96_PRIO
#define W2X_MLP96_PRIO 1
#endif
#ifndef W2X_MLP_STAGGER
#define W2X_MLP_STAGGER 0
#endif
#ifndef W2X_MLP_PFCH
#define W2X_MLP_PFCH 5
#endif

namespace w2x {
namespace {

typedef _Float16 half8 __attribute__((ext_vector_type(8)));
typedef _Float16 half4 __attribute__((ext_vector_type(4)));
typedef _Float16 half2v __attribute__((ext_vector_type(2)));
typedef float float4v __attribute__((ext_vector_type(4)));
typedef float float2v __attribute__((ext_vector_type(2)));
typedef float float16v __attribute__((ext_vector_type(16)));
typedef unsigned uint4v __attribute__((ext_vector_type(4)));

constexpr size_t kMaxBufBytes = 0xFFF00000u;
__device__ __forceinline__ __amdgpu_buffer_rsrc_t make_rsrc(const void* p, unsigned bytes) {
    return __builtin_amdgcn_make_buffer_rsrc(const_cast<void*>(p), 0, bytes, 0x00020000);
}

__device__ __forceinline__ float2v splat2(float c) { return (float2v){c, c}; }
#ifdef W2X_GELU_SCALAR
__device__ __forceinline__ float gelu_fast1(float x) {
    const float u = fminf(fabsf(x), 6.5f);
    float q = fmaf(-2.992485764e-05f, u, 7.398797018e-04f);
    q = fmaf(q, u, -7.977479093e-03f);
    q = fmaf(q, u, 5.323820859e-02f);
    q = fmaf(q, u, 4.589156733e-01f);
    q = fmaf(q, u, 1.151147085e+00f);
    return fmaf(-0.5f * u, __builtin_amdgcn_exp2f(-(q * u)), fmaxf(x, 0.f));
}
__device__ __forceinline__ float2v gelu_fast2(float2v x) { return (float2v){gelu_fast1(x[0]), gelu_fast1(x[1])}; }
#else
__device__ __forceinline__ float2v gelu_fast2(float2v x) {
    const float2v u = {fminf(fabsf(x[0]), 6.5f), fminf(fabsf(x[1]), 6.5f)};
// ... 231 lines not shown
            const int nch = ch + 1 < NCH ? ch + 1 : 0;
#pragma unroll
            for (int i = 0; i < NF; ++i) {
                if (!(W2X_MLP_EXP & 4)) acc2[i >> 1] = __builtin_amdgcn_mfma_f32_32x32x16_f16(wr[i], a2[i & 1], acc2[i >> 1], 0, 0, 0);
                else acc2[i >> 1][i] += (float)a2[i & 1][0] + (float)wr[i][1];
                if (!(W2X_MLP_EXP & 8)) wr[i] = *(const half8*)(WL + (size_t)(nch * NF + i) * 512);
                W2X_RING_FENCE();
            }
        }
#if defined(W2X_MLP96_PRIO) && (W2X_MLP96_PRIO == 1 || W2X_MLP96_PRIO >= 4)
        __builtin_amdgcn_s_setprio(0);
#elif defined(W2X_MLP96_PRIO) && W2X_MLP96_PRIO == 2
        __builtin_amdgcn_s_setprio(1);
#endif
        W2X_PHASE_FENCE();
        half8 wfh[2][3];
        if (TOIMG) {
#pragma unroll
            for (int t = 0; t < 2; ++t)
#pragma unroll
                for (int ks = 0; ks < 3; ++ks) wfh[t][ks] = *(const half8*)((const _Float16*)p.ti_w + lane * 8 + (size_t)(t * 3 + ks) * 512);
            W2X_RING_FENCE();
        }
        half8 xres[NP];
#pragma unroll
        for (int k = 0; k < NP; ++k) {
            const int idx = k * 64 + lane, r = idx / PPR, c = idx - r * PPR;
            xres[k] = *(const half8*)(Xw + r * LDX + c * 8);
        }
        W2X_PHASE_FENCE();
#pragma unroll
        for (int nt = 0; nt < NT; ++nt)
#pragma unroll
            for (int q = 0; q < 4; ++q)
                *(half4*)(Xw + r32 * LDX + nt * 32 + q * 8 + h * 4) = (half4){(_Float16)acc2[nt][4 * q], (_Float16)acc2[nt][4 * q + 1], (_Float16)acc2[nt][4 * q + 2], (_Float16)acc2[nt][4 * q + 3]};
        W2X_PHASE_FENCE();
        const unsigned yo = (unsigned)row0 * (C * 2) + lane * 16u;
#pragma unroll
        for (int k = 0; k < NP; ++k) {
            const int idx = k * 64 + lane, r = idx / PPR, c = idx - r * PPR;
            const half8 o = *(const half8*)(Xw + r * LDX + c * 8) + xres[k];
            if (TOIMG) *(half8*)(Xw + r * LDX + c * 8) = o;
            else if (!(W2X_MLP_EXP & 32)) __builtin_amdgcn_raw_buffer_store_b128(__builtin_bit_cast(uint4v, o), YB, yo + k * 1024u, 0, W2X_ST_AUX);
        }
        if (TOIMG) {
            W2X_PHASE_FENCE();
            const int fr16 = lane & 15, g4 = lane >> 4;
            const _Float16* Wt = (const _Float16*)p.ti_w + lane * 8;
            const int row0i = __builtin_amdgcn_readfirstlane((int)(row0 + p.ti_row0));
            const int bimg = row0i / p.ti_Mrows, ml0 = row0i - bimg * p.ti_Mrows;
            const int oy0 = ml0 / p.ti_aW, ox0 = ml0 - oy0 * p.ti_aW;
            _Float16* __restrict__ Og = (_Float16*)p.ti_out + (size_t)bimg * p.ti_Hs * p.ti_Ws * 4;
            const half2v lo2 = {(_Float16)p.ti_lo, (_Float16)p.ti_lo}, hi2 = {(_Float16)p.ti_hi, (_Float16)p.ti_hi};
#pragma unroll
            for (int th = 0; th < 2; ++th) {
                half8 wf[2][3];
#pragma unroll
                for (int t = 0; t < 2; ++t)
#pragma unroll
                    for (int ks = 0; ks < 3; ++ks) wf[t][ks] = th == 0 ? wfh[t][ks] : *(const half8*)(Wt + (size_t)((2 + t) * 3 + ks) * 512);
                float4v acc[2][2];
#pragma unroll
                for (int t = 0; t < 2; ++t) {
                    const float4v b = *(const float4v*)(p.ti_b + (2 * th + t) * 16 + g4 * 4);
#pragma unroll
                    for (int tt = 0; tt < 2; ++tt) acc[t][tt] = b;
                }
#pragma unroll
                for (int tt = 0; tt < 2; ++tt)
#pragma unroll
                    for (int ks = 0; ks < 3; ++ks) {
                        const half8 xa = *(const half8*)(Xw + (tt * 16 + fr16) * LDX + ks * 32 + g4 * 8);
#pragma unroll
                        for (int t = 0; t < 2; ++t) acc[t][tt] = __builtin_amdgcn_mfma_f32_16x16x32_f16(wf[t][ks], xa, acc[t][tt], 0, 0, 0);
                    }
#pragma unroll
                for (int tt = 0; tt < 2; ++tt) {
                    int ox = ox0 + tt * 16 + fr16, oy = oy0;
                    if (ox >= p.ti_aW) { ox -= p.ti_aW; ++oy; }
                    const bool ok = row0 + tt * 16 + fr16 < p.M;
#pragma unroll
                    for (int t = 0; t < 2; ++t) {
                        half2v v01 = {(_Float16)acc[t][tt][0], (_Float16)acc[t][tt][1]}, v23 = {(_Float16)acc[t][tt][2], (_Float16)acc[t][tt][3]};
                        if (p.ti_clip) {
                            asm("v_pk_max_f16 %0, %1, %2\n\tv_pk_min_f16 %0, %0, %3" : "=&v"(v01) : "v"(v01), "v"(lo2), "v"(hi2));
                            asm("v_pk_max_f16 %0, %1, %2\n\tv_pk_min_f16 %0, %0, %3" : "=&v"(v23) : "v"(v23), "v"(lo2), "v"(hi2));
                        }
                        const half4 px = {v01[0], v01[1], v23[0], v23[1]};
                        if (ok) *(half4*)(Og + ((size_t)(oy * 4 + 2 * th + t) * p.ti_Ws + ox * 4 + g4) * 4) = px;
                    }
                }
            }
        }
        if (!TOIMG && p.stats_out) {
#pragma unroll
            for (int k = 0; k < NP; ++k) {
                const int idx = k * 64 + lane, r = idx / PPR, c = idx - r * PPR;
                *(half8*)(Xw + r * LDX + c * 8) = *(const half8*)(Xw + r * LDX + c * 8) + xres[k];
            }
        }
        W2X_PHASE_FENCE();
        if (!TOIMG && p.stats_out && lane < nrows) {
            float s = 0.f, q = 0.f;
#pragma unroll
            for (int c = 0; c < PPR; ++c) sum_sq8(*(const half8*)(Xw + lane * LDX + c * 8), s, q);
            const float mean = s * (1.f / C);
            p.stats_out[2 * (row0 + lane)] = mean;
            p.stats_out[2 * (row0 + lane) + 1] = __builtin_amdgcn_rsqf(fmaxf(q * (1.f / C) - mean * mean, 0.f) + p.eps_out);
        }
        W2X_PHASE_FENCE();
    }
#undef W2X_FETCH
}

}

bool mlp96q_supported(const MlpParams& p) { return p.C == C && p.w1_frag && p.w2_frag && p.frag32 && (!p.ti_w || (p.ti_b && p.ti_out && !p.stats_out && p.ti_Mrows > 0 && p.ti_Mrows % RW == 0 && p.ti_aW >= RW && p.M < 0x7FFFFFFFl &&
                                                                 (!p.ti_clip || ((float)(_Float16)p.ti_lo == p.ti_lo && (float)(_Float16)p.ti_hi == p.ti_hi)))); }

hipError_t launch_mlp96q(const MlpParams& p, hipStream_t s) {
    static unsigned lds_ok = 0;
    static unsigned lds_ok_t = 0;
    if (hipError_t e = p.ti_w ? ensure_dynamic_lds((const void*)mlp96q_kernel<true>, SMEM96Q, lds_ok_t) : ensure_dynamic_lds((const void*)mlp96q_kernel<false>, SMEM96Q, lds_ok); e != hipSuccess) return e;
    static int cus[32] = {0};
    int dev = 0;
    if (hipError_t e = hipGetDevice(&dev); e != hipSuccess) return e;
    int ncu = __atomic_load_n(&cus[dev & 31], __ATOMIC_RELAXED);
    if (ncu == 0) {
        if (hipError_t e = hipDeviceGetAttribute(&ncu, hipDeviceAttributeMultiprocessorCount, dev); e != hipSuccess) return e;
        __atomic_store_n(&cus[dev & 31], ncu, __ATOMIC_RELAXED);
    }
    const long max_tiles = std::min<long>((long)(kMaxBufBytes / (RW * C * 2)), 0xFFFFFFFFl / (RW * C * 2) - (long)ncu * NWV);
    const long max_rows = max_tiles * RW;
    for (long r0 = 0; r0 < p.M; r0 += max_rows) {
        MlpParams q = p;
        q.M = std::min(max_rows, p.M - r0);
        q.x = (const char*)p.x + (size_t)r0 * C * 2; q.y = (char*)p.y + (size_t)r0 * C * 2;
        if (p.stats_out) q.stats_out = p.stats_out + 2 * r0;
        q.live_row0 = p.live_row0 + r0;
        const long ntiles = (q.M + RW - 1) / RW;
        const int grid = (int)std::min<long>((ntiles + NWV - 1) / NWV, ncu);
        if ((ntiles + (long)grid * NWV) * (long)(RW * C * 2) > 0xFFFFFFFFl) return hipErrorInvalidValue;
        if (p.ti_w) {
            q.ti_row0 = r0;
            hipLaunchKernelGGL(mlp96q_kernel<true>, dim3(grid), dim3(NTHR), SMEM96Q, s, q, (int)ntiles);
        } else hipLaunchKernelGGL(mlp96q_kernel<false>, dim3(grid), dim3(NTHR), SMEM96Q, s, q, (int)ntiles);
        if (hipError_t e = hipGetLastError(); e != hipSuccess) return e;
    }
    return hipSuccess;
}

}
```

waifu2x-tensorrt_amd/csrc/k_prepost.hip:

```cpp
#include "kernels.h"
#include "prepost_device.h"

namespace w2x {
namespace {

template <typename P>
__global__ __launch_bounds__(256) void gather_kernel(const GatherParams p) {
    const int T = p.T;
    const long total = (long)p.B * T * T;
    const float inv255 = (float)(1.0 / 255.0), inv65535 = (float)(1.0 / 65535.0);
    for (long i = (long)blockIdx.x * blockDim.x + threadIdx.x; i < total; i += (long)gridDim.x * blockDim.x) {
        int b = (int)(i / ((long)T * T));
        int rem = (int)(i - (long)b * T * T);
        int y = rem / T, x = rem - y * T;
        TileSlot sl = p.slots[b];
        P v = make_px<P>(0.f, 0.f, 0.f);
        if (sl.valid) {
            int sy, sx;
            aug_src(sl.aug, T - 1, y, x, sy, sx);
            int fy = min(max(sl.y + sy, 0), p.rows - 1);
            int fx = min(max(sl.x + sx, 0), p.cols - 1);
            if (!p.deep) {
                const uint8_t* px = p.frame + (size_t)fy * p.step + (size_t)fx * 3;
                v = make_px<P>((float)px[2] * inv255, (float)px[1] * inv255, (float)px[0] * inv255);
            } else {
                const uint16_t* px = (const uint16_t*)(p.frame + (size_t)fy * p.step) + (size_t)fx * 3;
                v = make_px<P>((float)px[2] * inv65535, (float)px[1] * inv65535, (float)px[0] * inv65535);
            }
        }
        *((P*)p.out + i) = v;
    }
}

template <typename P>
__device__ __forceinline__ unsigned compose_pixel(const ComposeParams& p, const P* tiles, int X, int Y) {
    float a0, a1, a2;
    compose_pixel_sums<P>(p, tiles, X, Y, a0, a1, a2);
    return quantize_bgr(a0, a1, a2);
}

typedef _Float16 half8 __attribute__((ext_vector_type(8)));

#ifndef W2X_COMPOSE_ROWS
#define W2X_COMPOSE_ROWS 4
#endif
#ifndef W2X_COMPOSE_THREADS
#define W2X_COMPOSE_THREADS 64
#endif
constexpr int kComposeRows = W2X_COMPOSE_ROWS, kComposeThreads = W2X_COMPOSE_THREADS;
template <typename P>
__global__ __launch_bounds__(kComposeThreads) void compose_kernel(const ComposeParams p) {
    constexpr bool kHalf = sizeof(P) == 8;
    const int x1 = p.x1 > 0 ? p.x1 : p.outW, sw = x1 - p.x0;
    const int gw = (sw + 3) >> 2;
    const int xg = blockIdx.x * kComposeThreads + threadIdx.x;
    if (xg >= gw) return;
    const P* tiles = (const P*)p.tiles;
    const int To = p.To, n = To - 1;
    const int X = p.x0 + 4 * xg;
    const int np = min(4, x1 - X);
    int a0 = X - To + 1; a0 = a0 <= 0 ? 0 : (a0 + p.stride_x - 1) / p.stride_x;
    int b0 = X + 3 - To + 1; b0 = b0 <= 0 ? 0 : (b0 + p.stride_x - 1) / p.stride_x;
    const int a1 = min(p.nx - 1, X / p.stride_x), b1 = min(p.nx - 1, (X + 3) / p.stride_x);
    const bool fast_col = kHalf && np == 4 && !p.tta && !p.deep && a0 == b0 && a1 == b1;
    const int Y0 = p.y0 + blockIdx.y * kComposeRows, Y1 = min(p.y1 > 0 ? p.y1 : p.outH, Y0 + kComposeRows);
    for (int Y = Y0; Y < Y1; ++Y) {
        uint8_t* d = p.dst + (size_t)Y * p.dst_step + (size_t)X * 3;
        unsigned px[4] = {0u, 0u, 0u, 0u};
        if (p.deep) {
            uint16_t* d16 = (uint16_t*)(p.dst + (size_t)Y * p.dst_step) + (size_t)X * 3;
            for (int k = 0; k < np; ++k) {
                float r, g, b;
                compose_pixel_sums<P>(p, tiles, X + k, Y, r, g, b);
                d16[3 * k] = (uint16_t)min(max(__float2int_rn(b * 65535.f), 0), 65535);
                d16[3 * k + 1] = (uint16_t)min(max(__float2int_rn(g * 65535.f), 0), 65535);
                d16[3 * k + 2] = (uint16_t)min(max(__float2int_rn(r * 65535.f), 0), 65535);
            }
            continue;
        }
        const bool fast = fast_col && (((size_t)d) & 3) == 0;
        if (fast) {
            int j0 = Y - To + 1; j0 = j0 <= 0 ? 0 : (j0 + p.stride_y - 1) / p.stride_y;
            const int j1 = min(p.ny - 1, Y / p.stride_y);
            float acc[4][3] = {};
            for (int ti = a0; ti <= a1; ++ti) {
                const int ox = ti * p.stride_x, lx = X - ox;
                const int rw = ox + To > p.outW ? p.outW - ox : To;
                for (int tj = j0; tj <= j1; ++tj) {
                    const int oy = tj * p.stride_y, ly = Y - oy;
                    const int rh = oy + To > p.outH ? p.outH - oy : To;
                    const long tile = (long)ti * p.ny + tj - p.first_tile;
                    const half4* tp = (const half4*)p.tiles + tile * (long)To * To + (long)ly * To + lx;
                    half4 h[4];
                    if ((((size_t)tp) & 15) == 0) { const half8 u0 = *(const half8*)tp, u1 = *(const half8*)(tp + 2);
                        h[0] = (half4){u0[0], u0[1], u0[2], u0[3]}; h[1] = (half4){u0[4], u0[5], u0[6], u0[7]}; h[2] = (half4){u1[0], u1[1], u1[2], u1[3]}; h[3] = (half4){u1[4], u1[5], u1[6], u1[7]}; }
                    else { h[0] = tp[0]; h[1] = tp[1]; h[2] = tp[2]; h[3] = tp[3]; }
                    const bool wl = ox > 0, wt = oy > 0 && ly < p.ovy, wr = ox + rw < p.outW, wb = oy + rh < p.outH && n - ly < p.ovy;
                    const float fy_t = wt ? p.ramp_y[ly] : 1.f, fy_b = wb ? p.ramp_y[n - ly] : 1.f;
#pragma unroll
                    for (int k = 0; k < 4; ++k) {
                        float v0 = (float)h[k][0], v1 = (float)h[k][1], v2 = (float)h[k][2];
                        if (p.ovx || p.ovy) {
                            const int lk = lx + k;
                            if (wl && lk < p.ovx) { float w = p.ramp_x[lk]; v0 *= w; v1 *= w; v2 *= w; }
                            if (wt) { v0 *= fy_t; v1 *= fy_t; v2 *= fy_t; }
                            if (wr && n - lk < p.ovx) { float w = p.ramp_x[n - lk]; v0 *= w; v1 *= w; v2 *= w; }
                            if (wb) { v0 *= fy_b; v1 *= fy_b; v2 *= fy_b; }
                        }
                        acc[k][0] += v0; acc[k][1] += v1; acc[k][2] += v2;
                    }
                }
            }
#pragma unroll
            for (int k = 0; k < 4; ++k) px[k] = quantize_bgr(acc[k][0], acc[k][1], acc[k][2]);
            unsigned* dw = (unsigned*)d;
            dw[0] = px[0] | px[1] << 24;
            dw[1] = px[1] >> 8 | px[2] << 16;
            dw[2] = px[2] >> 16 | px[3] << 8;
        } else {
            for (int k = 0; k < np; ++k) {
                const unsigned v = compose_pixel<P>(p, tiles, X + k, Y);
                d[3 * k] = (uint8_t)v; d[3 * k + 1] = (uint8_t)(v >> 8); d[3 * k + 2] = (uint8_t)(v >> 16);
            }
        }
    }
}

template <typename P>
__global__ __launch_bounds__(256) void compose_canvas_kernel(const ComposeParams p, float* canvas) {
    const int x1 = p.x1 > 0 ? p.x1 : p.outW, y1 = p.y1 > 0 ? p.y1 : p.outH;
    const int X = p.x0 + blockIdx.x * 256 + threadIdx.x;
    if (X >= x1) return;
    const size_t plane = (size_t)p.outW * p.outH;
    for (int Y = p.y0 + blockIdx.y; Y < y1; Y += gridDim.y) {
        float r, g, b;
        compose_pixel_sums<P>(p, (const P*)p.tiles, X, Y, r, g, b);
        const size_t i = (size_t)Y * p.outW + X;
        canvas[i] = r; canvas[plane + i] = g; canvas[2 * plane + i] = b;
    }
}

__device__ __forceinline__ float yuv_sample(const YuvPlanes& f, int pl, int y, int x) {
    const uint8_t* row = f.p[pl] + (size_t)y * f.step[pl];
    return f.bits > 8 ? (float)((const uint16_t*)row)[x] : (float)row[x];
}

template <typename P>
__global__ __launch_bounds__(256) void gather_yuv_kernel(const GatherYuvParams p) {
    const int T = p.T;
    const long total = (long)p.B * T * T;
    const int rows = p.src.rows, cols = p.src.cols, ch = (rows + 1) >> 1, cw = (cols + 1) >> 1;
    const YuvCoefs& k = p.k;
    for (long i = (long)blockIdx.x * blockDim.x + threadIdx.x; i < total; i += (long)gridDim.x * blockDim.x) {
        int b = (int)(i / ((long)T * T));
        int rem = (int)(i - (long)b * T * T);
        int y = rem / T, x = rem - y * T;
        TileSlot sl = p.slots[b];
        P v = make_px<P>(0.f, 0.f, 0.f);
        if (sl.valid) {
            int sy, sx;
            aug_src(sl.aug, T - 1, y, x, sy, sx);
            const int fy = min(max(sl.y + sy, 0), rows - 1), fx = min(max(sl.x + sx, 0), cols - 1);
            const int ck = fy >> 1, cj = fx >> 1;
            const bool odd_y = fy & 1;
            const int r0 = odd_y ? ck : max(ck - 1, 0), r1 = odd_y ? min(ck + 1, ch - 1) : ck;
            const float w0 = odd_y ? 0.75f : 0.25f, w1 = odd_y ? 0.25f : 0.75f;
            const int c1 = (fx & 1) ? min(cj + 1, cw - 1) : cj;
            const float u = w0 * (0.5f * (yuv_sample(p.src, 1, r0, cj) + yuv_sample(p.src, 1, r0, c1))) + w1 * (0.5f * (yuv_sample(p.src, 1, r1, cj) + yuv_sample(p.src, 1, r1, c1)));
            const float w = w0 * (0.5f * (yuv_sample(p.src, 2, r0, cj) + yuv_sample(p.src, 2, r0, c1))) + w1 * (0.5f * (yuv_sample(p.src, 2, r1, cj) + yuv_sample(p.src, 2, r1, c1)));
            const float Y = (yuv_sample(p.src, 0, fy, fx) - k.y_off) * k.y_mul, cb = (u - k.c_off) * k.c_mul, cr = (w - k.c_off) * k.c_mul;
            const float R = Y + k.r_cr * cr, G = Y + k.g_cb * cb + k.g_cr * cr, B = Y + k.b_cb * cb;
            v = make_px<P>(fminf(fmaxf(R, 0.f), 1.f), fminf(fmaxf(G, 0.f), 1.f), fminf(fmaxf(B, 0.f), 1.f));
        }
        *((P*)p.out + i) = v;
    }
}

__device__ __forceinline__ unsigned yuv_code(float off, float scale, float v, int maxcode) { return (unsigned)min(max(__float2int_rn(off + scale * v), 0), maxcode); }
// ... 147 lines not shown
        const int cp = (int)(i % pc);
        const int b = (int)(i / pc / HW);
        float4v v = *((float4v*)x + i);
        const float* sc = scale + b * Cs + cp * 4;
#pragma unroll
        for (int e = 0; e < 4; ++e) v[e] *= sc[e];
        *((float4v*)x + i) = v;
    }
}

template <typename P>
__global__ __launch_bounds__(256) void blob_to_nhwc_kernel(const float* nchw, P* out, int B, int T) {
    const long total = (long)B * T * T;
    for (long i = (long)blockIdx.x * blockDim.x + threadIdx.x; i < total; i += (long)gridDim.x * blockDim.x) {
        int b = (int)(i / ((long)T * T));
        long rem = i - (long)b * T * T;
        const float* s = nchw + (long)b * 3 * T * T + rem;
        out[i] = make_px<P>(s[0], s[(long)T * T], s[2L * T * T]);
    }
}

template <typename P>
__global__ __launch_bounds__(256) void nhwc_to_blob_kernel(const P* in, float* nchw, int B, int T) {
    const long total = (long)B * T * T;
    for (long i = (long)blockIdx.x * blockDim.x + threadIdx.x; i < total; i += (long)gridDim.x * blockDim.x) {
        int b = (int)(i / ((long)T * T));
        long rem = i - (long)b * T * T;
        const P v = in[i];
        float* d = nchw + (long)b * 3 * T * T + rem;
        d[0] = (float)v[0]; d[(long)T * T] = (float)v[1]; d[2L * T * T] = (float)v[2];
    }
}

inline unsigned grid_for(long total) { long g = (total + 255) / 256; return (unsigned)(g > 8192 ? 8192 : (g < 1 ? 1 : g)); }

}

hipError_t launch_gather(const GatherParams& p, hipStream_t s) {
    const dim3 grid(grid_for((long)p.B * p.T * p.T));
    if (p.fp32) hipLaunchKernelGGL(gather_kernel<float4v>, grid, dim3(256), 0, s, p);
    else hipLaunchKernelGGL(gather_kernel<half4>, grid, dim3(256), 0, s, p);
    return hipGetLastError();
}
hipError_t launch_compose(const ComposeParams& p, hipStream_t s) {
    const int gw = (((p.x1 > 0 ? p.x1 : p.outW) - p.x0) + 3) / 4;
    if (gw <= 0 || p.outH <= 0) return hipSuccess;
    const int nrows = (p.y1 > 0 ? p.y1 : p.outH) - p.y0;
    if (nrows <= 0) return hipSuccess;
    const dim3 grid((unsigned)((gw + kComposeThreads - 1) / kComposeThreads), (unsigned)((nrows + kComposeRows - 1) / kComposeRows));
    if (p.fp32) hipLaunchKernelGGL(compose_kernel<float4v>, grid, dim3(kComposeThreads), 0, s, p);
    else hipLaunchKernelGGL(compose_kernel<half4>, grid, dim3(kComposeThreads), 0, s, p);
    return hipGetLastError();
}
hipError_t launch_compose_canvas(const ComposeParams& p, float* canvas, hipStream_t s) {
    const int w = (p.x1 > 0 ? p.x1 : p.outW) - p.x0, h = (p.y1 > 0 ? p.y1 : p.outH) - p.y0;
    if (w <= 0 || h <= 0) return hipSuccess;
    const dim3 grid((unsigned)((w + 255) / 256), (unsigned)(h < 65535 ? h : 65535));
    if (p.fp32) hipLaunchKernelGGL(compose_canvas_kernel<float4v>, grid, dim3(256), 0, s, p, canvas);
    else hipLaunchKernelGGL(compose_canvas_kernel<half4>, grid, dim3(256), 0, s, p, canvas);
    return hipGetLastError();
}
hipError_t launch_gather_yuv(const GatherYuvParams& p, hipStream_t s) {
    const dim3 grid(grid_for((long)p.B * p.T * p.T));
    if (p.fp32) hipLaunchKernelGGL(gather_yuv_kernel<float4v>, grid, dim3(256), 0, s, p);
    else hipLaunchKernelGGL(gather_yuv_kernel<half4>, grid, dim3(256), 0, s, p);
    return hipGetLastError();
}
hipError_t launch_compose_yuv(const ComposeYuvParams& p, hipStream_t s) {
    const int cw = (p.c.outW + 1) / 2, ch = (p.c.outH + 1) / 2;
    if (cw <= 0 || ch <= 0) return hipSuccess;
    const int runs = (cw + kYuvSites - 1) / kYuvSites;
    const dim3 grid((unsigned)((runs + kYuvThreads - 1) / kYuvThreads), (unsigned)(ch < 65535 ? ch : 65535));
    if (p.c.fp32) hipLaunchKernelGGL(compose_yuv_kernel<float4v>, grid, dim3(kYuvThreads), 0, s, p);
    else hipLaunchKernelGGL(compose_yuv_kernel<half4>, grid, dim3(kYuvThreads), 0, s, p);
    return hipGetLastError();
}
hipError_t launch_se(const SeParams& p, hipStream_t s) {
    const int threads = 1024, slices = threads / p.C > 0 ? threads / p.C : 1;
    hipLaunchKernelGGL(se_kernel, dim3(p.B), dim3(threads), (p.C + p.Cmid + slices * p.C) * sizeof(float), s, p);
    return hipGetLastError();
}
hipError_t launch_scale(void* x, const float* scale, int B, int HW, int Cs, bool fp32, hipStream_t s) {
    if (fp32) hipLaunchKernelGGL(scale32_kernel, dim3(grid_for((long)B * HW * (Cs / 4))), dim3(256), 0, s, (float*)x, scale, B, (long)HW, Cs);
    else hipLaunchKernelGGL(scale_kernel, dim3(grid_for((long)B * HW * (Cs / 8))), dim3(256), 0, s, (_Float16*)x, scale, B, (long)HW, Cs);
    return hipGetLastError();
}
hipError_t launch_blob_to_nhwc(const float* nchw, void* out, int B, int T, bool fp32, hipStream_t s) {
    const dim3 grid(grid_for((long)B * T * T));
    if (fp32) hipLaunchKernelGGL(blob_to_nhwc_kernel<float4v>, grid, dim3(256), 0, s, nchw, (float4v*)out, B, T);
    else hipLaunchKernelGGL(blob_to_nhwc_kernel<half4>, grid, dim3(256), 0, s, nchw, (half4*)out, B, T);
    return hipGetLastError();
}
hipError_t launch_nhwc_to_blob(const void* in, float* nchw, int B, int T, bool fp32, hipStream_t s) {
    const dim3 grid(grid_for((long)B * T * T));
    if (fp32) hipLaunchKernelGGL(nhwc_to_blob_kernel<float4v>, grid, dim3(256), 0, s, (const float4v*)in, nchw, B, T);
    else hipLaunchKernelGGL(nhwc_to_blob_kernel<half4>, grid, dim3(256), 0, s, (const half4*)in, nchw, B, T);
    return hipGetLastError();
}

}
```

waifu2x-tensorrt_amd/csrc/kernels.h:

```cpp
#pragma once
#include <hip/hip_runtime.h>

#include "support.h"
#include "switches.h"
#include <cstdint>

namespace w2x {

constexpr int kGemmBM = 128;

inline hipError_t ensure_dynamic_lds(const void* fn, int bytes, unsigned& done_mask) {
    int dev = 0;
    hipError_t e = hipGetDevice(&dev);
    if (e != hipSuccess) return e;
    const unsigned bit = 1u << (dev & 31);
    if (__atomic_load_n(&done_mask, __ATOMIC_ACQUIRE) & bit) return hipSuccess;
    e = hipFuncSetAttribute(fn, hipFuncAttributeMaxDynamicSharedMemorySize, bytes);
    if (e == hipSuccess) __atomic_fetch_or(&done_mask, bit, __ATOMIC_RELEASE);
    return e;
}

#ifndef W2X_ST_AUX
#define W2X_ST_AUX 2
#endif
#ifndef W2X_LD_LAST_AUX
#define W2X_LD_LAST_AUX 2
#endif
#ifdef __HIPCC__
template <class T> __device__ __forceinline__ void w2x_store_out(T* p, const T v) {
#if W2X_ST_AUX == 2
    __builtin_nontemporal_store(v, p);
#else
    *p = v;
#endif
}
#endif

struct LiveExt { uint16_t cx, wx, cy, wy; };
#ifdef __HIPCC__
__device__ __forceinline__ LiveExt live_ext_load(const LiveExt* t, int slot) {
    typedef const unsigned long long __attribute__((address_space(4)))* cptr;
    const unsigned long long v = ((cptr)(unsigned long long)t)[slot];
    return LiveExt{(uint16_t)v, (uint16_t)(v >> 16), (uint16_t)(v >> 32), (uint16_t)(v >> 48)};
}
__device__ __forceinline__ bool live_token(const LiveExt e, int x, int y, int W, int H) { return (x < e.cx || x >= W - e.wx) && (y < e.cy || y >= H - e.wy); }
__device__ __forceinline__ bool live_rows(const LiveExt* t, long r0, int n, int W, int H) {
    const int HW = W * H;
    if (n > HW) return true;
    const int img = (int)(r0 / HW);
    int r = (int)(r0 - (long)img * HW);
    LiveExt e = live_ext_load(t, img);
    for (int left = n; left > 0;) {
        if (r >= HW) { r -= HW; e = live_ext_load(t, img + 1); }
        const int y = r / W, x0 = r - y * W, x1 = x0 + left < W ? x0 + left : W;
        if ((y < e.cy || y >= H - e.wy) && (x0 < e.cx || x1 > W - e.wx)) return true;
        left -= x1 - x0; r += x1 - x0;
    }
    return false;
}
#endif

struct TView {
    void* p = nullptr;
    int Hs = 0, Ws = 0, Cs = 0;
    int y0 = 0, x0 = 0;
};

struct GemmParams {
    TView a;
    int amode = 0, kh = 1, kw = 1, stride = 1;
    int B = 0, Mrows = 0, aW = 0;
    const int* win_table = nullptr;
    int K = 0, N = 0, Kw = 0;
    const void* wt = nullptr;
    const void* wt_frag = nullptr;
    const void* wt_perm = nullptr;
    const float* bias = nullptr;
    const float* csum = nullptr;
    const float* stats_in = nullptr;
    int ln = 0;
    int act = 0; float alpha = 0.f;
    int has_clip = 0; float clip_lo = 0.f, clip_hi = 0.f;
    const float* a_scale = nullptr;
    const float* res_scale = nullptr;
    TView res, res2;
    TView out;
    int omode = 0, r = 1, Cout = 0;
    float* stats_out = nullptr; float ln_eps = 1e-5f;
    float* pool_out = nullptr;
};

struct AttnParams {
    const void* qkv = nullptr; void* out = nullptr;
    int B = 0, nwin = 0, heads = 0, hd = 0, ntok = 0;
    float scale = 1.f;
    const void* bias = nullptr;
    const int* maskid = nullptr;
};

struct MlpParams {
    const void* x = nullptr; void* y = nullptr;
    long M = 0; int C = 0;
    const void* w1 = nullptr;
    const float* b1 = nullptr;
    const void* w2 = nullptr;
    const float* b2 = nullptr;
    float eps = 1e-5f;
    float* stats_out = nullptr; float eps_out = 1e-5f;
    const void* w1_frag = nullptr; const void* w2_frag = nullptr;
    bool frag32 = false;
    const void* ti_w = nullptr;
    const float* ti_b = nullptr;
    void* ti_out = nullptr; int ti_Hs = 0, ti_Ws = 0, ti_Mrows = 0, ti_aW = 0;
    int ti_clip = 0; float ti_lo = 0.f, ti_hi = 0.f;
    long ti_row0 = 0;
    const LiveExt* live = nullptr; int live_W = 0, live_H = 0;
    long live_row0 = 0;
};

struct SwinAttnParams {
    const void* x = nullptr; void* y = nullptr;
    const int* table = nullptr;
    int H = 0, W = 0, ry = -1, rx = -1;
    int B = 0, nwin = 0, C = 0, hd = 0;
    const void* wqkv = nullptr;
    const float* bqkv = nullptr;
    float scale = 1.f;
    const float* bias32 = nullptr;
    const int* maskid = nullptr;
    const void* wproj = nullptr;
    const float* bproj = nullptr;
    float eps = 1e-5f;
    float* stats_out = nullptr; float eps_out = 1e-5f;
    const void* wqkv_frag = nullptr; const void* wproj_frag = nullptr;
    const LiveExt* live = nullptr;
};

struct SeParams {
    const float* pool = nullptr; float* scale = nullptr;
    int B = 0, C = 0, Cs = 0, Cmid = 0; float inv_count = 0.f;
    int nblocks = 0, Mrows = 0;
    const float *w1 = nullptr, *b1 = nullptr, *w2 = nullptr, *b2 = nullptr;
};

struct TileSlot { int x, y, aug, valid; };

struct GatherParams {
    const uint8_t* frame = nullptr; int rows = 0, cols = 0; size_t step = 0;
    int deep = 0;
    void* out = nullptr;
    int fp32 = 0;
    const TileSlot* slots = nullptr;
    int B = 0, T = 0;
};

struct ComposeParams {
    const void* tiles = nullptr;
    int fp32 = 0;
    uint8_t* dst = nullptr; size_t dst_step = 0;
    int deep = 0;
    int outW = 0, outH = 0;
    int To = 0;
    int nx = 0, ny = 0;
    int stride_x = 0, stride_y = 0;
    int ovx = 0, ovy = 0;
    const float* ramp_x = nullptr;
    const float* ramp_y = nullptr;
    int tta = 0;
    int tta_bug_compat = 0;
    int x0 = 0, x1 = 0; long first_tile = 0;
// ... 1 lines not shown
};

hipError_t launch_gemm(const GemmParams& p, hipStream_t s);
bool pixgemm_supported(const GemmParams& p);
hipError_t launch_pixgemm(const GemmParams& p, hipStream_t s);
bool conv3_supported(const GemmParams& p);
bool stem_supported(const GemmParams& p);
hipError_t launch_stem(const GemmParams& p, hipStream_t s);
hipError_t launch_conv3(const GemmParams& p, hipStream_t s);
bool conv3h_supported(const GemmParams& p);
hipError_t launch_conv3h(const GemmParams& p, hipStream_t s);
bool conv48_supported(const GemmParams& p);
hipError_t launch_conv48(const GemmParams& p, hipStream_t s);
bool conv48_stem_supported(const GemmParams& p, const GemmParams& ps);
hipError_t launch_conv48_stem(const GemmParams& p, const GemmParams& ps, hipStream_t s);
bool conv3_stem_supported(const GemmParams& p, const GemmParams& ps);
hipError_t launch_conv3_stem(const GemmParams& p, const GemmParams& ps, hipStream_t s);
bool conv3_up_supported(const GemmParams& p, const GemmParams& q);
hipError_t launch_conv3_up(const GemmParams& p, const GemmParams& q, hipStream_t s);
int conv3_tiles(const GemmParams& p);
hipError_t launch_attn(const AttnParams& p, hipStream_t s);
hipError_t launch_gemm_f32(const GemmParams& p, hipStream_t s, bool exact);
hipError_t launch_attn_f32(const AttnParams& p, hipStream_t s);
struct Mlp32Params {
    const float* x = nullptr; float* y = nullptr;
    long M = 0; int C = 0;
    const float* stats_in = nullptr;
    const void *w1h = nullptr, *w1l = nullptr, *w2h = nullptr, *w2l = nullptr;
    const float *b1 = nullptr, *b2 = nullptr;
    float* stats_out = nullptr; float eps_out = 1e-5f;
};
bool mlp32_supported(int C);
hipError_t launch_mlp32(const Mlp32Params& p, hipStream_t s);
struct SwinAttn32Params {
    const float* x = nullptr; float* y = nullptr; const float* res = nullptr;
    int B = 0, nwin = 0, C = 0;
    long pix_per_item = 0;
    const int* table_in = nullptr; const int* table_out = nullptr;
    const float* stats_in = nullptr;
    const void *wqkv_h = nullptr, *wqkv_l = nullptr, *wproj_h = nullptr, *wproj_l = nullptr;
    const float *bqkv = nullptr, *bproj = nullptr;
    float scale = 1.f;
    const float* bias = nullptr; const int* maskid = nullptr;
    float* stats_out = nullptr; float eps_out = 1e-5f;
};
bool swinattn32_supported(int C, int heads, int hd, int ntok);
hipError_t launch_swinattn32(const SwinAttn32Params& p, hipStream_t s);
hipError_t launch_mlp(const MlpParams& p, hipStream_t s);
hipError_t launch_swin_attn(const SwinAttnParams& p, hipStream_t s);
hipError_t launch_se(const SeParams& p, hipStream_t s);
hipError_t launch_scale(void* x, const float* scale, int B, int HW, int Cs, bool fp32, hipStream_t s);
hipError_t launch_gather(const GatherParams& p, hipStream_t s);
hipError_t launch_compose(const ComposeParams& p, hipStream_t s);
hipError_t launch_compose_canvas(const ComposeParams& p, float* canvas, hipStream_t s);
struct ResampleParams {
    const float* canvas = nullptr; int inW = 0, inH = 0;
    uint8_t* dst = nullptr; size_t dst_step = 0; int deep = 0;
    int outW = 0, outH = 0;
    const int* fx = nullptr; const float* wx = nullptr; int kx = 0;
    const int* fy = nullptr; const float* wy = nullptr; int ky = 0;
    int rows_max = 0;
};
constexpr int kResampleRows = 16, kResampleCols = 64;
int resample_rows_max(const int* fy, int outH, int inH, int ky);
hipError_t launch_resample(const ResampleParams& p, hipStream_t s);
struct YuvPlanes {
    uint8_t* p[3] = {nullptr, nullptr, nullptr}; size_t step[3] = {0, 0, 0};
    int rows = 0, cols = 0, bits = 8;
};
struct YuvCoefs {
    float y_off = 0.f, y_mul = 0.f, c_off = 0.f, c_mul = 0.f;
    float y_scale = 0.f, c_scale = 0.f;
    float kr = 0.f, kg = 0.f, kb = 0.f;
    float r_cr = 0.f, g_cb = 0.f, g_cr = 0.f, b_cb = 0.f;
    float cb_div = 0.f, cr_div = 0.f;
    int maxcode = 255;
};
inline YuvCoefs yuv_coefs(int matrix, int full_range, int bits) {
    const double kr = matrix == 0 ? 0.299 : matrix == 1 ? 0.2126 : 0.2627, kb = matrix == 0 ? 0.114 : matrix == 1 ? 0.0722 : 0.0593, kg = 1.0 - kr - kb;
    const double q = (double)(1 << (bits - 8)), top = (double)((1 << bits) - 1);
    const double y_off = full_range ? 0.0 : 16.0 * q, y_scale = full_range ? top : 219.0 * q;
    const double c_off = full_range ? (double)(1 << (bits - 1)) : 128.0 * q, c_scale = full_range ? top : 224.0 * q;
    YuvCoefs k;
    k.y_off = (float)y_off; k.y_mul = (float)(1.0 / y_scale); k.c_off = (float)c_off; k.c_mul = (float)(1.0 / c_scale);
    k.y_scale = (float)y_scale; k.c_scale = (float)c_scale;
    k.kr = (float)kr; k.kg = (float)kg; k.kb = (float)kb;
    k.r_cr = (float)(2.0 * (1.0 - kr)); k.b_cb = (float)(2.0 * (1.0 - kb));
    k.g_cb = (float)(-2.0 * (1.0 - kb) * kb / kg); k.g_cr = (float)(-2.0 * (1.0 - kr) * kr / kg);
    k.cb_div = (float)(1.0 / (2.0 * (1.0 - kb))); k.cr_div = (float)(1.0 / (2.0 * (1.0 - kr)));
    k.maxcode = (1 << bits) - 1;
    return k;
}
struct GatherYuvParams {
    YuvPlanes src; YuvCoefs k;
    void* out = nullptr; int fp32 = 0;
    const TileSlot* slots = nullptr;
    int B = 0, T = 0;
};
hipError_t launch_gather_yuv(const GatherYuvParams& p, hipStream_t s);
struct ComposeYuvParams {
    ComposeParams c;
    YuvPlanes dst; YuvCoefs k;
};
constexpr int kYuvSites = 4, kYuvThreads = 64;
hipError_t launch_compose_yuv(const ComposeYuvParams& p, hipStream_t s);
struct AlphaBleedParams {
// ... 60 lines not shown
```

waifu2x-tensorrt_amd/csrc/prepost_device.h:

```cpp
#pragma once
#include "kernels.h"

namespace w2x {
namespace {

typedef _Float16 half4 __attribute__((ext_vector_type(4)));
typedef _Float16 half8 __attribute__((ext_vector_type(8)));
typedef float float4v __attribute__((ext_vector_type(4)));
template <typename P> __device__ __forceinline__ P make_px(float r, float g, float b);
template <> __device__ __forceinline__ half4 make_px<half4>(float r, float g, float b) { return (half4){(_Float16)r, (_Float16)g, (_Float16)b, (_Float16)0.f}; }
template <> __device__ __forceinline__ float4v make_px<float4v>(float r, float g, float b) { return (float4v){r, g, b, 0.f}; }

__device__ __forceinline__ void aug_src(int k, int n, int y, int x, int& sy, int& sx) {
    switch (k) {
        default: sy = y; sx = x; break;
        case 1: sy = n - y; sx = x; break;
        case 2: sy = y; sx = n - x; break;
        case 3: sy = x; sx = n - y; break;
        case 4: sy = n - y; sx = n - x; break;
        case 5: sy = n - x; sx = y; break;
        case 6: sy = n - x; sx = n - y; break;
        case 7: sy = x; sx = y; break;
    }
}
__device__ __forceinline__ void deaug_src(int k, int n, int y, int x, int& sy, int& sx) {
    switch (k) {
        default: sy = y; sx = x; break;
        case 1: sy = n - y; sx = x; break;
        case 2: sy = y; sx = n - x; break;
        case 3: sy = n - x; sx = y; break;
        case 4: sy = n - y; sx = n - x; break;
        case 5: sy = x; sx = n - y; break;
        case 6: sy = n - x; sx = n - y; break;
        case 7: sy = x; sx = y; break;
    }
}

__device__ __forceinline__ unsigned quantize_bgr(float r, float g, float b) {
    const unsigned B = (unsigned)min(max(__float2int_rn(b * 255.f), 0), 255), G = (unsigned)min(max(__float2int_rn(g * 255.f), 0), 255),
                   R = (unsigned)min(max(__float2int_rn(r * 255.f), 0), 255);
    return B | G << 8 | R << 16;
}
template <typename P>
__device__ __forceinline__ void compose_pixel_sums(const ComposeParams& p, const P* tiles, int X, int Y, float& r0, float& r1, float& r2) {
    const int To = p.To, n = To - 1;
    const int steps = p.tta ? 8 : 1;
    int i0 = X - To + 1; i0 = i0 <= 0 ? 0 : (i0 + p.stride_x - 1) / p.stride_x;
    int i1 = min(p.nx - 1, X / p.stride_x);
    int j0 = Y - To + 1; j0 = j0 <= 0 ? 0 : (j0 + p.stride_y - 1) / p.stride_y;
    int j1 = min(p.ny - 1, Y / p.stride_y);
    float acc0 = 0.f, acc1 = 0.f, acc2 = 0.f;
    for (int ti = i0; ti <= i1; ++ti) {
        const int ox = ti * p.stride_x, lx = X - ox;
        const int rw = ox + To > p.outW ? p.outW - ox : To;
        for (int tj = j0; tj <= j1; ++tj) {
            const int oy = tj * p.stride_y, ly = Y - oy;
// ... 35 lines not shown
```

waifu2x-tensorrt_amd/csrc/support.cpp:

```cpp
#include "support.h"

namespace w2x {

bool swin_attn_supported(int C, int heads, int hd, int ws) {
    return ws == 6 && heads * hd == C && ((C == 96 && hd == 16) || (C == 192 && hd == 32));
}
bool mlp_supported(int C) { return C == 96 || C == 192; }
bool gemm_row_stats_supported(int N) { return N == 32 || N == 48 || N == 64 || N == 96 || N == 128 || N == 192; }
bool attn_supported(int hd, int ntok) {
    if (ntok != 36 && ntok != 64) return false;
    return hd == 8 || hd == 16 || hd == 24 || hd == 32 || hd == 48 || hd == 64;
}

}

#include <algorithm>
#include <cstdlib>
#include <cstring>

#include "switches.h"

namespace w2x {

namespace {
struct Field { const char* name; int Switches::*i; bool Switches::*b; const char* env; int lo, hi; };
const Field kFields[] = {
    {"superbatch", &Switches::superbatch, nullptr, "W2X_SUPERBATCH", 0, 4096},
    {"groups", &Switches::groups, nullptr, "W2X_GROUPS", 1, 4},
    {"render_parts", &Switches::render_parts, nullptr, "W2X_RENDER_PARTS", 1, 4},
    {"no_graph", nullptr, &Switches::no_graph, "W2X_NO_GRAPH", 0, 1},
    {"no_rolling", nullptr, &Switches::no_rolling, "W2X_NO_ROLLING", 0, 1},
    {"poison", nullptr, &Switches::poison, "W2X_POISON", 0, 1},
    {"check_general", nullptr, &Switches::check_general, "W2X_CHECK_GENERAL", 0, 1},
    {"roctx", nullptr, &Switches::roctx, "W2X_ROCTX", 0, 1},
    {"no_fuse", nullptr, &Switches::no_fuse, nullptr, 0, 1},
    {"no_fuse_attn", nullptr, &Switches::no_fuse_attn, nullptr, 0, 1},
    {"no_se_fold", nullptr, &Switches::no_se_fold, nullptr, 0, 1},
    {"no_fuse_head", nullptr, &Switches::no_fuse_head, nullptr, 0, 1},
    {"no_fuse_stem", nullptr, &Switches::no_fuse_stem, nullptr, 0, 1},
    {"no_fuse_up", nullptr, &Switches::no_fuse_up, nullptr, 0, 1},
    {"no_conv3h_walk", nullptr, &Switches::no_conv3h_walk, nullptr, 0, 1},
    {"no_pixgemm", nullptr, &Switches::no_pixgemm, nullptr, 0, 1},
    {"no_conv3", nullptr, &Switches::no_conv3, nullptr, 0, 1},
    {"no_conv3h", nullptr, &Switches::no_conv3h, nullptr, 0, 1},
    {"no_conv48", nullptr, &Switches::no_conv48, nullptr, 0, 1},
    {"no_stem", nullptr, &Switches::no_stem, nullptr, 0, 1},
    {"attn_valu", nullptr, &Switches::attn_valu, nullptr, 0, 1},
    {"no_dead_skip", nullptr, &Switches::no_dead_skip, nullptr, 0, 1},
};
void assign(Switches& s, const Field& f, long v) {
    v = std::min<long>(f.hi, std::max<long>(f.lo, v));
    if (f.i) s.*(f.i) = (int)v; else s.*(f.b) = v != 0;
}
}

Switches& switches() { static Switches s; return s; }

void switches_from_env() {
    Switches& s = switches();
    const Switches d;
    for (const Field& f : kFields) {
        if (!f.env) continue;
        const char* e = getenv(f.env);
        if (f.i) s.*(f.i) = e ? (int)std::min<long>(f.hi, std::max<long>(f.lo, atol(e))) : d.*(f.i);
        else s.*(f.b) = e != nullptr;
    }
}

bool set_switch(const char* name, long value) {
    if (!name) return false;
    for (const Field& f : kFields) if (!strcmp(f.name, name)) { assign(switches(), f, value); return true; }
    return false;
}

std::string switches_nondefault() {
    const Switches& s = switches();
    const Switches d;
    std::string out;
    for (const Field& f : kFields) {
        const bool same = f.i ? s.*(f.i) == d.*(f.i) : s.*(f.b) == d.*(f.b);
        if (same) continue;
        if (!out.empty()) out += ' ';
        out += f.name;
        if (f.i) out += "=" + std::to_string(s.*(f.i));
    }
    return out;
}

}
```

waifu2x-tensorrt_amd/csrc/switches.h:

```cpp
#pragma once
#include <string>

namespace w2x {

struct Switches {
    int superbatch = 0;
    int groups = 2;
    int render_parts = 3;
    bool no_graph = false;
    bool no_rolling = false;
    bool poison = false;
    bool check_general = false;
    bool roctx = false;
    bool no_fuse = false;
    bool no_fuse_attn = false;
    bool no_se_fold = false;
    bool no_fuse_head = false;
    bool no_fuse_stem = false;
    bool no_fuse_up = false;
    bool no_conv3h_walk = false;
    bool no_pixgemm = false, no_conv3 = false, no_conv3h = false, no_conv48 = false, no_stem = false;
    bool attn_valu = false;
    bool no_dead_skip = false;
};

Switches& switches();
void switches_from_env();
bool set_switch(const char* name, long value);
std::string switches_nondefault();

}
```

waifu2x-tensorrt_amd/engine.py:

```python
from __future__ import annotations

import ctypes as C
import enum
import os
from dataclasses import dataclass

import numpy as np

_HERE = os.path.dirname(os.path.abspath(__file__))
lib_path = os.path.join(_HERE, "libw2x.so")


class W2xError(RuntimeError):
    pass


class Precision(enum.IntEnum):
    TF32 = 0
    FP16 = 1
    FP32 = 2


RESIZE_FILTERS = {"bicubic": 0, "bilinear": 1}

# ... 104 lines not shown
    L.w2x_set_progress_callback.argtypes = [vp, _PROG_FN, vp]
    L.w2x_build.argtypes = [vp, C.c_char_p, C.POINTER(_BuildConfig)]; L.w2x_build.restype = C.c_int
    L.w2x_load.argtypes = [vp, C.c_char_p, C.POINTER(_RenderConfig)]; L.w2x_load.restype = C.c_int
    L.w2x_render.argtypes = [vp, vp, C.c_int, C.c_int, C.c_size_t, vp, C.c_size_t]; L.w2x_render.restype = C.c_int
    L.w2x_render16.argtypes = [vp, vp, C.c_int, C.c_int, C.c_size_t, vp, C.c_size_t]; L.w2x_render16.restype = C.c_int
    L.w2x_render_resized.argtypes = [vp, vp, C.c_int, C.c_int, C.c_size_t, vp, C.c_int, C.c_int, C.c_size_t, C.c_int]; L.w2x_render_resized.restype = C.c_int
    L.w2x_render16_resized.argtypes = [vp, vp, C.c_int, C.c_int, C.c_size_t, vp, C.c_int, C.c_int, C.c_size_t, C.c_int]; L.w2x_render16_resized.restype = C.c_int
    L.w2x_render_sequence_resized.argtypes = [vp, vp, C.c_int, C.c_int, C.c_size_t, vp, C.c_int, C.c_int, C.c_size_t, C.c_int, C.c_int]; L.w2x_render_sequence_resized.restype = C.c_int
    L.w2x_resize_weights.argtypes = [C.c_int, C.c_int, C.c_int, vp, vp, C.c_int]; L.w2x_resize_weights.restype = C.c_int
    L.w2x_render_yuv.argtypes = [vp, vp, vp, C.c_int, C.c_int, C.c_int, vp, vp, C.c_int, C.c_int, C.c_int, C.c_int, C.c_int]; L.w2x_render_yuv.restype = C.c_int
    L.w2x_render_sequence_yuv.argtypes = [vp, vp, vp, C.c_int, C.c_int, C.c_int, vp, vp, C.c_int, C.c_int, C.c_int, C.c_int, C.c_int, C.c_int]
    L.w2x_render_sequence_yuv.restype = C.c_int
    L.w2x_render_yuv_resized.argtypes = L.w2x_render_yuv.argtypes + [C.c_int]; L.w2x_render_yuv_resized.restype = C.c_int
    L.w2x_render_sequence_yuv_resized.argtypes = L.w2x_render_sequence_yuv.argtypes + [C.c_int]; L.w2x_render_sequence_yuv_resized.restype = C.c_int
    L.w2x_render_rgba.argtypes = [vp, vp, C.c_int, C.c_int, C.c_size_t, vp, C.c_size_t, C.c_int, C.c_int]; L.w2x_render_rgba.restype = C.c_int
    L.w2x_alpha_bleed_device.argtypes = [vp, vp, C.c_int, C.c_int, C.c_size_t, vp, C.c_size_t, C.c_int]; L.w2x_alpha_bleed_device.restype = C.c_int
    L.w2x_alpha_bleed.argtypes = [vp, C.c_size_t, vp, C.c_size_t, C.c_int, C.c_int, C.c_int, vp, C.c_size_t]; L.w2x_alpha_bleed.restype = C.c_int
    L.w2x_yuv_plane_sizes.argtypes = [C.c_int, C.c_int, C.c_int, vp, vp, vp]; L.w2x_yuv_plane_sizes.restype = C.c_int
    L.w2x_render_strip.argtypes = [vp, vp, C.c_int, C.c_int, C.c_size_t, vp, C.c_size_t, C.c_int, C.c_int]; L.w2x_render_strip.restype = C.c_int
    L.w2x_render_sequence.argtypes = [vp, vp, C.c_int, C.c_int, C.c_size_t, vp, C.c_size_t, C.c_int]; L.w2x_render_sequence.restype = C.c_int
    L.w2x_alloc_host.argtypes = [vp, C.c_size_t]; L.w2x_alloc_host.restype = vp
    L.w2x_free_host.argtypes = [vp, vp]; L.w2x_free_host.restype = None
    L.w2x_pin_host.argtypes = [vp, vp, C.c_size_t]; L.w2x_pin_host.restype = C.c_int
    L.w2x_unpin_host.argtypes = [vp, vp]; L.w2x_unpin_host.restype = None
    L.w2x_strip_plan.argtypes = [C.c_int] * 7 + [C.c_double, C.c_double, C.c_int, C.c_int, vp]; L.w2x_strip_plan.restype = C.c_int
    L.w2x_render_sharded.argtypes = [vp, C.c_int, vp, C.c_int, C.c_int, C.c_size_t, vp, C.c_size_t]; L.w2x_render_sharded.restype = C.c_int
    L.w2x_shard_compute.argtypes = [vp, vp, C.c_int, C.c_int, C.c_size_t, C.c_int, C.c_int]; L.w2x_shard_compute.restype = C.c_int
    L.w2x_shard_slab.argtypes = [vp, vp]; L.w2x_shard_slab.restype = vp
    L.w2x_shard_finish.argtypes = [vp, vp, C.c_int, C.c_int, C.c_size_t, C.c_int, C.c_int, vp, vp]; L.w2x_shard_finish.restype = C.c_int
    L.w2x_ipc_export.argtypes = [vp, vp]; L.w2x_ipc_export.restype = C.c_int
    L.w2x_ipc_open.argtypes = [vp, C.c_int]; L.w2x_ipc_open.restype = vp
    L.w2x_ipc_close.argtypes = [vp]; L.w2x_ipc_close.restype = None
    L.w2x_shard_plan.argtypes = [C.c_int] * 7 + [C.c_double, C.c_double, C.c_int, C.c_int, vp]; L.w2x_shard_plan.restype = C.c_int
    L.w2x_infer.argtypes = [vp, vp, vp]; L.w2x_infer.restype = C.c_int
    L.w2x_output_tile_size.argtypes = [vp]; L.w2x_output_tile_size.restype = C.c_int
    L.w2x_pass_tiles.argtypes = [vp]; L.w2x_pass_tiles.restype = C.c_int
    L.w2x_plan_flops.argtypes = [vp]; L.w2x_plan_flops.restype = C.c_double
    L.w2x_last_render_ms.argtypes = [vp]; L.w2x_last_render_ms.restype = C.c_float
    L.w2x_bench_resident.argtypes = [vp, C.c_int]; L.w2x_bench_resident.restype = C.c_float
    L.w2x_resident_output.argtypes = [vp, vp, C.c_size_t]; L.w2x_resident_output.restype = C.c_int
    L.w2x_profile_frame.argtypes = [vp, vp, C.c_int]; L.w2x_profile_frame.restype = C.c_int
    L.w2x_op_times.argtypes = [vp, vp, C.c_int]; L.w2x_op_times.restype = C.c_int
    L.w2x_calculate_tiles.argtypes = [C.c_int] * 7 + [C.c_double, C.c_double, vp, vp, C.c_int]; L.w2x_calculate_tiles.restype = C.c_int
    L.w2x_tile_weights.argtypes = [C.c_int, C.c_int, C.c_int, C.c_int, vp]; L.w2x_tile_weights.restype = C.c_int
    L.w2x_describe_plan.argtypes = [C.c_char_p, C.c_int, C.c_int, C.c_char_p, C.c_size_t]; L.w2x_describe_plan.restype = C.c_int
    L.w2x_describe_plan_precision.argtypes = [C.c_char_p, C.c_int, C.c_int, C.c_int, C.c_char_p, C.c_size_t]; L.w2x_describe_plan_precision.restype = C.c_int
    L.w2x_write_engine_file.argtypes = [C.c_char_p, C.c_int, C.c_int, C.c_char_p]; L.w2x_write_engine_file.restype = C.c_int
    L.w2x_validate_engine_file.argtypes = [C.c_char_p, C.c_char_p, C.c_size_t]; L.w2x_validate_engine_file.restype = C.c_int
    L.w2x_device_pci_bus_id.argtypes = [C.c_int, C.c_char_p, C.c_size_t]; L.w2x_device_pci_bus_id.restype = C.c_int
    L.w2x_sha256_hex.argtypes = [vp, C.c_size_t, C.c_char_p]
    L.w2x_version.restype = C.c_char_p
    L.w2x_debug_set.argtypes = [C.c_char_p, C.c_int]; L.w2x_debug_set.restype = C.c_int
    L.w2x_dead_skip_extents.argtypes = [C.c_char_p] + [C.c_int] * 5 + [C.c_double, C.c_double, C.c_int, C.c_int, vp, C.c_int]; L.w2x_dead_skip_extents.restype = C.c_int
    _lib = L
    return L


EXPORTED_SYMBOLS = [
    "w2x_create", "w2x_destroy", "w2x_set_message_callback", "w2x_set_progress_callback", "w2x_build", "w2x_load",
    "w2x_render", "w2x_render16", "w2x_infer", "w2x_output_tile_size", "w2x_plan_flops", "w2x_pass_tiles", "w2x_last_render_ms", "w2x_bench_resident", "w2x_resident_output", "w2x_profile_frame", "w2x_op_times",
    "w2x_render_resized", "w2x_render16_resized", "w2x_render_sequence_resized", "w2x_resize_weights",
    "w2x_render_yuv", "w2x_render_sequence_yuv", "w2x_yuv_plane_sizes", "w2x_render_yuv_resized", "w2x_render_sequence_yuv_resized",
    "w2x_render_rgba", "w2x_alpha_bleed_device", "w2x_alpha_bleed", "w2x_dead_skip_extents",
    "w2x_render_strip", "w2x_strip_plan", "w2x_render_sharded", "w2x_shard_plan", "w2x_shard_compute", "w2x_shard_slab", "w2x_shard_finish", "w2x_ipc_export", "w2x_ipc_open", "w2x_ipc_close", "w2x_render_sequence", "w2x_alloc_host", "w2x_free_host", "w2x_pin_host", "w2x_unpin_host", "w2x_calculate_tiles", "w2x_tile_weights", "w2x_describe_plan", "w2x_describe_plan_precision", "w2x_write_engine_file", "w2x_validate_engine_file", "w2x_device_pci_bus_id", "w2x_sha256_hex", "w2x_version", "w2x_debug_set"]


class Img2Img:

    def __init__(self):
        self._L = lib()
        self._h = self._L.w2x_create()
        if not self._h:
            raise W2xError("w2x_create failed")
        self.messages: list[tuple[int, str]] = []
        self._user_msg = None
        self._user_prog = None
        self._msg_cb = _MSG_FN(self._on_msg)
        self._prog_cb = _PROG_FN(self._on_prog)
        self._L.w2x_set_message_callback(self._h, self._msg_cb, None)
        self._L.w2x_set_progress_callback(self._h, self._prog_cb, None)

    def _on_msg(self, sev, msg, _):
        m = msg.decode(errors="replace")
        self.messages.append((sev, m))
        if self._user_msg:
            self._user_msg(Severity(sev), m)

    def _on_prog(self, cur, total, speed, _):
        if self._user_prog:
            self._user_prog(cur, total, speed)

    def close(self):
        if self._h:
            self._L.w2x_destroy(self._h)
            self._h = None

    def __del__(self):
        try:
            self.close()
        except Exception:
            pass

    def setMessageCallback(self, cb):
        self._user_msg = cb

    def setProgressCallback(self, cb):
        self._user_prog = cb

    def last_error(self) -> str:
        errs = [m for s, m in self.messages if s <= Severity.error]
        return errs[-1] if errs else ""

    def build(self, path: str, config: BuildConfig) -> bool:
        c = _BuildConfig(*[int(getattr(config, f[0])) for f in _BuildConfig._fields_])
        return bool(self._L.w2x_build(self._h, os.fsencode(path), C.byref(c)))

# ... 441 lines not shown
    if taps <= 0:
        raise W2xError(f"invalid resize {in_size} -> {out_size}")
    first = np.zeros(out_size, np.int32)
    w = np.zeros((out_size, taps), np.float32)
    if L.w2x_resize_weights(int(in_size), int(out_size), fid, first.ctypes.data, w.ctypes.data, w.size) != taps:
        raise W2xError("w2x_resize_weights failed")
    return first, w


def alpha_bleed(bgr: np.ndarray, alpha: np.ndarray, radius: int) -> np.ndarray:
    if bgr.dtype != np.uint8 or bgr.ndim != 3 or bgr.shape[2] != 3 or (bgr.size and (bgr.strides[2] != 1 or bgr.strides[1] != 3)):
        raise ValueError("bgr must be a uint8 [rows, cols, 3] array with packed pixels")
    if alpha.dtype != np.uint8 or alpha.shape != bgr.shape[:2] or (alpha.size and alpha.strides[1] != 1):
        raise ValueError("alpha must be a uint8 [rows, cols] array of the frame's size with packed rows")
    out = np.empty(bgr.shape, np.uint8)
    if not lib().w2x_alpha_bleed(bgr.ctypes.data if bgr.size else None, bgr.strides[0], alpha.ctypes.data if alpha.size else None, alpha.strides[0],
                                 bgr.shape[0], bgr.shape[1], int(radius), out.ctypes.data if out.size else None, out.strides[0]):
        raise W2xError(f"invalid alpha bleed: a {bgr.shape[1]}x{bgr.shape[0]} frame at radius {radius}")
    return out


def yuv_plane_sizes(rows: int, cols: int, bits: int):
    pr, pc, pb = (C.c_int * 3)(), (C.c_int * 3)(), (C.c_size_t * 3)()
    if not lib().w2x_yuv_plane_sizes(int(rows), int(cols), int(bits), pr, pc, pb):
        raise W2xError(f"invalid YUV frame {rows}x{cols} at {bits} bits")
    return list(pr), list(pc), list(pb)


def describe_plan(onnx_path, batch, tile, precision=None) -> str:
    L = lib()
    buf = C.create_string_buffer(1 << 20)
    ok = L.w2x_describe_plan_precision(os.fsencode(onnx_path), batch, tile, int(Precision.FP16 if precision is None else precision), buf, len(buf))
    s = buf.value.decode(errors="replace")
    if not ok:
        raise W2xError(s)
    return s


EXTENT_FIELDS = ("kind", "W", "H", "cx", "wx", "cy", "wy", "rx", "ry", "ws", "t_in", "t_out", "t_res", "kh", "kw", "stride", "x0", "y0", "r",
                 "in_W", "in_H", "out_W", "out_H", "live_units", "total_units")


def dead_skip_extents(onnx_path, batch, tile, in_w, in_h, scaling, overlap, tile_index, tta=False) -> list[dict]:
    L = lib()
    n = -L.w2x_dead_skip_extents(os.fsencode(onnx_path), batch, tile, in_w, in_h, scaling, float(overlap[0]), float(overlap[1]), int(tile_index), int(bool(tta)), None, 0)
    if n <= 0:
        raise W2xError("w2x_dead_skip_extents failed")
    out = np.zeros((n, len(EXTENT_FIELDS)), np.int32)
    if L.w2x_dead_skip_extents(os.fsencode(onnx_path), batch, tile, in_w, in_h, scaling, float(overlap[0]), float(overlap[1]), int(tile_index), int(bool(tta)), out.ctypes.data, out.size) != n:
        raise W2xError("w2x_dead_skip_extents failed")
    return [dict(zip(EXTENT_FIELDS, (int(v) for v in row))) for row in out]


def write_engine_file(onnx_path, batch, tile, out_path) -> bool:
    return bool(lib().w2x_write_engine_file(os.fsencode(onnx_path), batch, tile, os.fsencode(out_path)))


def validate_engine_file(path) -> tuple[bool, str]:
    buf = C.create_string_buffer(4096)
    ok = lib().w2x_validate_engine_file(os.fsencode(path), buf, len(buf))
    return bool(ok), buf.value.decode(errors="replace")


def sha256_hex(data: bytes) -> str:
    L = lib()
    out = C.create_string_buffer(65)
    L.w2x_sha256_hex(data, len(data), out)
    return out.value.decode()
```

Measured before the change: 4643 MPix/s.

## Write final head output directly to frame interior, compose only seam regions

The final MLP/head GEMM now writes tile interiors that need no blending straight into the uint8 output frame, using per-slot DirectSlot tables that hold base pointers and 4-pixel block spans. The compose pass is then limited to seam rectangles between tiles, using a cached SeamRect table and a new compose_seam kernel. This avoids writing the fp16 slab and reading it back for most output pixels. The cost is extra table uploads, more graph-key variants, a wait on out_free before rolling passes, and more complexity in the head kernel epilogue.

```diff
diff --git a/include/w2x/c_api.h b/include/w2x/c_api.h
--- a/include/w2x/c_api.h
+++ b/include/w2x/c_api.h
@@ -96,6 +96,7 @@
 enum { W2X_EXTENT_INTS = 25 };
 int w2x_dead_skip_extents(const char* onnx_path, int batch, int tile, int in_w, int in_h, int scaling, double overlap_x, double overlap_y, int tile_index, int tta,
                           int* out, int cap);
+int w2x_direct_span(int tile_out, int stride, int n, int ramp, int out, int index, int align4, int* b0, int* b1);
 int w2x_device_pci_bus_id(int device, char* buf, size_t cap);
 void w2x_sha256_hex(const void* data, size_t len, char* out);
 const char* w2x_version(void);
diff --git a/waifu2x-tensorrt_amd/__init__.py b/waifu2x-tensorrt_amd/__init__.py
--- a/waifu2x-tensorrt_amd/__init__.py
+++ b/waifu2x-tensorrt_amd/__init__.py
@@ -1,6 +1,6 @@
 from .engine import (BuildConfig, RenderConfig, Img2Img, Precision, Severity, lib, lib_path,
-                     calculate_tiles, strip_plan, shard_plan, render_sharded, device_pci_bus_id, ipc_open, ipc_close, tile_weights, resize_weights, yuv_plane_sizes, alpha_bleed, describe_plan, dead_skip_extents, write_engine_file, validate_engine_file, sha256_hex, W2xError,
+                     calculate_tiles, strip_plan, shard_plan, render_sharded, device_pci_bus_id, ipc_open, ipc_close, tile_weights, resize_weights, yuv_plane_sizes, alpha_bleed, describe_plan, dead_skip_extents, direct_span, write_engine_file, validate_engine_file, sha256_hex, W2xError,
                      debug_switches)
 
 __all__ = ["BuildConfig", "RenderConfig", "Img2Img", "Precision", "Severity", "lib", "lib_path",
-           "calculate_tiles", "strip_plan", "shard_plan", "render_sharded", "device_pci_bus_id", "ipc_open", "ipc_close", "tile_weights", "resize_weights", "yuv_plane_sizes", "alpha_bleed", "describe_plan", "dead_skip_extents", "write_engine_file", "validate_engine_file", "sha256_hex", "W2xError", "debug_switches"]
+           "calculate_tiles", "strip_plan", "shard_plan", "render_sharded", "device_pci_bus_id", "ipc_open", "ipc_close", "tile_weights", "resize_weights", "yuv_plane_sizes", "alpha_bleed", "describe_plan", "dead_skip_extents", "direct_span", "write_engine_file", "validate_engine_file", "sha256_hex", "W2xError", "debug_switches"]
diff --git a/waifu2x-tensorrt_amd/csrc/c_api.cpp b/waifu2x-tensorrt_amd/csrc/c_api.cpp
--- a/waifu2x-tensorrt_amd/csrc/c_api.cpp
+++ b/waifu2x-tensorrt_amd/csrc/c_api.cpp
@@ -12,6 +12,7 @@
 #include "sha256.h"
 #include "tiles.h"
 #include "kernels.h"
+#include "prepost_device.h"
 
 struct w2x_engine {
     w2x::Img2Img engine;
@@ -376,6 +377,13 @@
     } catch (const std::exception&) { return 0; }
 }
 
+int w2x_direct_span(int tile_out, int stride, int n, int ramp, int out, int index, int align4, int* b0, int* b1) {
+    if (!b0 || !b1) return 0;
+    const w2x::BlockSpan s = w2x::direct_span(tile_out, stride, n, ramp, out, index, align4 != 0);
+    *b0 = s.b0; *b1 = s.b1;
+    return 1;
+}
+
 int w2x_debug_set(const char* name, int value) { return w2x::set_switch(name, value) ? 1 : 0; }
 
 }
diff --git a/waifu2x-tensorrt_amd/csrc/engine.cpp b/waifu2x-tensorrt_amd/csrc/engine.cpp
--- a/waifu2x-tensorrt_amd/csrc/engine.cpp
+++ b/waifu2x-tensorrt_amd/csrc/engine.cpp
@@ -22,6 +22,7 @@
 #include "liveness.h"
 #include "lower.h"
 #include "plan.h"
+#include "prepost_device.h"
 #include "sha256.h"
 #include "switches.h"
 #include "tiles.h"
@@ -229,8 +230,9 @@
     LiveExt* d_live = nullptr; size_t live_cap = 0, live_stride = 0;
     std::vector<LiveExt> h_live;
     std::map<std::pair<int, int>, std::vector<OpExtent>> live_cache;
-    void upload_live(const TileGrid& grid, size_t count, hipStream_t on) {
+    void upload_live(const TileGrid& grid, size_t count, hipStream_t on, int direct_rows = 0, int direct_cols = 0) {
         const size_t nops = plan.ops.size();
+        direct_on = false;
         if (!count || !nops) return;
         if (count > live_stride) {
             ensure(d_live, live_cap, (nops * count + 8) * sizeof(LiveExt));
@@ -260,6 +262,86 @@
             }
         }
         hipAssert(hipMemcpy2DAsync(d_live, live_stride * sizeof(LiveExt), h_live.data(), count * sizeof(LiveExt), count * sizeof(LiveExt), nops, hipMemcpyHostToDevice, on));
+        upload_direct(grid, count, on, direct_rows > 0 && direct_cols > 0, direct_rows, direct_cols);
+    }
+    bool head_direct = false;
+    bool direct_on = false;
+    int direct_which = 0;
+    DirectSlot* d_direct = nullptr; size_t direct_cap = 0;
+    std::vector<DirectSlot> h_direct;
+    struct SeamTable { SeamRect* d = nullptr; int nrect = 0, units = 0; };
+    std::map<std::array<int, 13>, SeamTable> seam_tables;
+    void drop_seam_tables() {
+        for (auto& kv : seam_tables) if (kv.second.d) (void)hipFree(kv.second.d);
+        seam_tables.clear();
+    }
+    struct DirectGeom { int To, nx, ny, sx, sy, rx, ry, outW, outH; };
+    DirectGeom direct_geom(int rows, int cols, const TileGrid& grid) const {
+        const bool overlapping = cfg.overlapX != 0 || cfg.overlapY != 0;
+        return DirectGeom{plan.Tout, grid.nx, grid.ny, plan.Tout - grid.outOvX, plan.Tout - grid.outOvY, overlapping ? ovx : 0, overlapping ? ovy : 0, cols * cfg.scaling, rows * cfg.scaling};
+    }
+    void upload_direct(const TileGrid& grid, size_t count, hipStream_t on, bool want, int rows, int cols) {
+        direct_on = false;
+        if (!want || !head_direct || switches().no_direct_head || check_general || cfg.tta || deep || yuv || rgba || rs || !d_out) return;
+        const DirectGeom g = direct_geom(rows, cols, grid);
+        const size_t step = (size_t)g.outW * 3;
+        if (g.sx <= 0 || g.sy <= 0 || (step & 3) || step * g.outH > 0xFFF00000u || ((size_t)d_out & 3) || ((size_t)d_out2 & 3) || g.To / 4 > 65535) return;
+        ensure(d_direct, direct_cap, 2 * live_stride * sizeof(DirectSlot));
+        std::map<std::pair<int, int>, int> tile_at;
+        for (int t = 0; t < grid.count; ++t) tile_at[{grid.in[t].x, grid.in[t].y}] = t;
+        h_direct.assign(2 * count, DirectSlot{});
+        for (size_t st = 0; st < count; ++st) {
+            const TileSlot& sl = h_slots[st];
+            if (!sl.valid || sl.aug != 0) continue;
+            const auto it = tile_at.find({sl.x, sl.y});
+            if (it == tile_at.end()) continue;
+            const int ti = it->second / grid.ny, tj = it->second % grid.ny;
+            const BlockSpan bx = direct_span(g.To, g.sx, g.nx, g.rx, g.outW, ti, true), by = direct_span(g.To, g.sy, g.ny, g.ry, g.outH, tj, false);
+            if (bx.b1 <= bx.b0 || by.b1 <= by.b0) continue;
+            for (int w = 0; w < 2; ++w) {
+                uint8_t* const out = w ? d_out2 : d_out;
+                if (!out) continue;
+                DirectSlot& e = h_direct[w * count + st];
+                e.base = (unsigned long long)(size_t)(out + (size_t)tj * g.sy * step + (size_t)ti * g.sx * 3); e.step = (unsigned)step;
+                e.limit = (unsigned)(step * g.outH - ((size_t)tj * g.sy * step + (size_t)ti * g.sx * 3));
+                e.bx0 = (unsigned short)bx.b0; e.bx1 = (unsigned short)bx.b1; e.by0 = (unsigned short)by.b0; e.by1 = (unsigned short)by.b1;
+            }
+        }
+        hipAssert(hipMemcpy2DAsync(d_direct, live_stride * sizeof(DirectSlot), h_direct.data(), count * sizeof(DirectSlot), count * sizeof(DirectSlot), 2, hipMemcpyHostToDevice, on));
+        direct_on = true;
+    }
+    const SeamTable& seam_table(const DirectGeom& g, int x0, int x1, int y0, int y1) {
+        const std::array<int, 13> key{g.To, g.nx, g.ny, g.sx, g.sy, g.rx, g.ry, g.outW, g.outH, x0, x1, y0, y1};
+        auto it = seam_tables.find(key);
+        if (it != seam_tables.end()) return it->second;
+        if (seam_tables.size() >= 64) {
+            for (hipStream_t st : {gstream[0], stream}) if (st) hipAssert(hipStreamSynchronize(st));
+            drop_seam_tables();
+        }
+        std::vector<BlockSpan> DX(g.nx), DY(g.ny);
+        for (int i = 0, at = 0; i < g.nx; ++i) { DX[i] = direct_span_px(g.To, g.sx, g.nx, g.rx, g.outW, i, true, at); at = DX[i].b1; }
+        for (int j = 0, at = 0; j < g.ny; ++j) { DY[j] = direct_span_px(g.To, g.sy, g.ny, g.ry, g.outH, j, false, at); at = DY[j].b1; }
+        std::vector<SeamRect> rects;
+        int units = 0;
+        auto add = [&](int ax0, int ax1, int ay0, int ay1) {
+            ax0 = std::max(ax0, x0); ax1 = std::min(ax1, x1); ay0 = std::max(ay0, y0); ay1 = std::min(ay1, y1);
+            if (ax0 >= ax1 || ay0 >= ay1) return;
+            const int gw = (ax1 - ax0 + 3) / 4;
+            int tw = 1; while (tw < gw && tw < 64) tw *= 2;
+            const int cu = (gw + tw - 1) / tw, rows_per_unit = 64 / tw * kSeamRows, ru = (ay1 - ay0 + rows_per_unit - 1) / rows_per_unit;
+            rects.push_back(SeamRect{ax0, ax1, ay0, ay1, tw, cu, units, 0});
+            units += cu * ru;
+        };
+        for (int k = 0; k <= g.nx; ++k) add(k ? DX[k - 1].b1 : 0, k < g.nx ? DX[k].b0 : g.outW, 0, g.outH);
+        for (int i = 0; i < g.nx; ++i) if (DX[i].b1 > DX[i].b0)
+            for (int m = 0; m <= g.ny; ++m) add(DX[i].b0, DX[i].b1, m ? DY[m - 1].b1 : 0, m < g.ny ? DY[m].b0 : g.outH);
+        SeamTable t;
+        t.nrect = (int)rects.size(); t.units = units;
+        if (t.nrect) {
+            hipAssert(hipMalloc((void**)&t.d, rects.size() * sizeof(SeamRect)));
+            if (hipError_t e = hipMemcpy(t.d, rects.data(), rects.size() * sizeof(SeamRect), hipMemcpyHostToDevice); e != hipSuccess) { (void)hipFree(t.d); hipAssert(e); }
+        }
+        return seam_tables.emplace(key, t).first->second;
     }
     float *d_rampx = nullptr, *d_rampy = nullptr;
     int ovx = 0, ovy = 0;
@@ -322,7 +404,7 @@
         }
         ensure(d_slots, slots_cap, stepCount * sizeof(TileSlot));
         hipAssert(hipMemcpy(d_slots, h_slots.data(), stepCount * sizeof(TileSlot), hipMemcpyHostToDevice));
-        upload_live(last_grid, stepCount, stream);
+        upload_live(last_grid, stepCount, stream, last_rows, last_cols);
         hipAssert(hipStreamSynchronize(stream));
         ensure(d_slab, slab_cap, stepCount * plan.Tout * plan.Tout * 4 * plan.elt);
         one_part_stale = false;
@@ -333,6 +415,7 @@
     float last_ms = 0.f;
 
     static constexpr int kRgbaKey = 64;
+    static constexpr int kDirectKey = 128;
     using GraphKey = std::tuple<const void*, const void*, const void*, const void*, int, int, int, int>;
     struct PassGraphs { hipGraphExec_t g[4] = {nullptr, nullptr, nullptr, nullptr}; int n = 0; };
     std::map<GraphKey, PassGraphs> graphs;
@@ -379,6 +462,8 @@
             if (*p) { (void)hipFree(*p); *p = nullptr; }
         frame_cap = out_cap = slab_cap = slab2_cap = slots_cap = 0;
         live_cap = live_stride = 0; live_cache.clear();
+        if (d_direct) { (void)hipFree(d_direct); d_direct = nullptr; }
+        direct_cap = 0; direct_on = false; direct_which = 0; head_direct = false; drop_seam_tables();
         shard_rows = shard_cols = 0; shard_halo_slots = 0; rolling = false; one_part_stale = false;
         last_rows = last_cols = last_batches = 0;
         if (ev0) { (void)hipEventDestroy(ev0); ev0 = nullptr; }
@@ -701,6 +786,7 @@
                     const GemmParams g = gp(L.last);
                     MlpParams p = mlp_params(op, live, tp);
                     p.live = lv(L.last);
+                    if (direct_on && ext && L.last == final_op) p.direct = d_direct + (size_t)direct_which * live_stride + (ext - d_live);
                     p.ti_w = g.wt_frag; p.ti_b = g.bias; p.ti_out = g.out.p; p.ti_Hs = g.out.Hs; p.ti_Ws = g.out.Ws; p.ti_Mrows = g.Mrows; p.ti_aW = g.aW;
                     p.ti_clip = g.has_clip; p.ti_lo = g.clip_lo; p.ti_hi = g.clip_hi;
                     issue([&] { return launch_mlp(p, s); });
@@ -857,6 +943,7 @@
         if (which == 1) { std::swap(d_slab, d_slab2); std::swap(slab_cap, slab2_cap); }
         rolling = true;
         hipAssert(hipStreamWaitEvent(stream, ev_cmp[which], 0));
+        if (direct_on && out_free) hipAssert(hipStreamWaitEvent(stream, out_free, 0));
         run_passes(rows, cols, sp.tile_count, 0, false, 0, true);
         hipAssert(hipEventRecord(ev_g0[which], stream));
         hipStream_t s2 = gstream[0];
@@ -957,7 +1044,7 @@
             auto run_eager = [&] { if (per_group) { fork(); for (int grp = 0; grp < NG; ++grp) run_group(grp); if (!no_join) join(); } else { if (rolling && gstream[0]) { join(); } run_pass(); } };
             if (!graphable) run_eager();
             else {
-                const GraphKey key{d_frame, d_slots + slots_off + (size_t)bi * B, slab_out, arena_base, rows, cols, live, rgba ? kRgbaKey : yuv ? yuv->key : deep ? 1 : 0};
+                const GraphKey key{d_frame, d_slots + slots_off + (size_t)bi * B, slab_out, arena_base, rows, cols, live, (rgba ? kRgbaKey : yuv ? yuv->key : deep ? 1 : 0) + (direct_on ? kDirectKey * (1 + direct_which) : 0)};
                 auto replay = [&](const PassGraphs& pg) {
                     if (pg.n == 1) { if (rolling && gstream[0]) join(); hipAssert(hipGraphLaunch(pg.g[0], stream)); return; }
                     fork();
@@ -1017,6 +1104,14 @@
         cp.ovx = overlapping ? ovx : 0; cp.ovy = overlapping ? ovy : 0;
         cp.ramp_x = d_rampx; cp.ramp_y = d_rampy; cp.tta = cfg.tta ? 1 : 0; cp.tta_bug_compat = cfg.ttaBugCompat ? 1 : 0;
         cp.x0 = x0; cp.x1 = x1; cp.y0 = y0; cp.y1 = y1; cp.first_tile = first_tile;
+        if (direct_on) {
+            const SeamTable& st = seam_table(direct_geom(rows, cols, grid), x0, x1 > 0 ? x1 : cp.outW, y0, y1 > 0 ? y1 : cp.outH);
+            if (!st.units) return;
+            stamp_begin(4, 0);
+            hipAssert(launch_compose_seam(cp, st.d, st.nrect, st.units, on ? on : stream));
+            stamp_end();
+            return;
+        }
         stamp_begin(4, 0);
         hipAssert(launch_compose(cp, on ? on : stream));
         stamp_end();
@@ -1075,7 +1170,7 @@
         rp.alpha_value = value;
         hipAssert(launch_compose_rgba(rp, stream));
     }
-    void sequence_slots(const TileGrid& grid, const StripPlan& sp) {
+    void sequence_slots(const TileGrid& grid, const StripPlan& sp, int direct_rows = 0, int direct_cols = 0) {
         const int steps = cfg.tta ? 8 : 1, B = plan.B, S = plan.B / plan.userB;
         const int batchCount = (int)std::lround(std::ceil((double)(sp.tile_count * steps) / plan.userB));
         const int stepCount = ((batchCount + S - 1) / S) * B;
@@ -1088,7 +1183,7 @@
         }
         ensure(d_slots, slots_cap, (size_t)stepCount * sizeof(TileSlot));
         hipAssert(hipMemcpyAsync(d_slots, h_slots.data(), (size_t)stepCount * sizeof(TileSlot), hipMemcpyHostToDevice, stream));
-        upload_live(grid, (size_t)stepCount, stream);
+        upload_live(grid, (size_t)stepCount, stream, direct_rows, direct_cols);
         ensure(d_slab, slab_cap, (size_t)stepCount * plan.Tout * plan.Tout * 4 * plan.elt);
         hipAssert(hipStreamSynchronize(stream));
     }
@@ -1096,7 +1191,7 @@
     float run_sequence(int count, int rows, int cols, const TileGrid& grid, const StripPlan& sp, const Up& up, const Down& down) {
         uint8_t* const frames[2] = {d_frame, d_frame2};
         uint8_t* const outs[2] = {d_out, d_out2};
-        struct Restore { Impl* im; uint8_t* f; uint8_t* o; ~Restore() { im->d_frame = f; im->d_out = o; } } restore{this, frames[0], outs[0]};
+        struct Restore { Impl* im; uint8_t* f; uint8_t* o; ~Restore() { im->d_frame = f; im->d_out = o; im->direct_which = 0; } } restore{this, frames[0], outs[0]};
         const bool roll = count > 1 && can_roll(sp.tile_count);
         if (roll) ensure(d_slab2, slab2_cap, slab_cap);
         hipAssert(hipStreamSynchronize(stream));
@@ -1107,7 +1202,7 @@
             up(i, frames[b], s_up);
             hipAssert(hipEventRecord(ev_up[b], s_up));
             hipAssert(hipStreamWaitEvent(stream, ev_up[b], 0));
-            d_frame = frames[b]; d_out = outs[b];
+            d_frame = frames[b]; d_out = outs[b]; direct_which = b;
             if (roll) {
                 run_rolling_frame(rows, cols, grid, sp, b, i >= 2 ? ev_dn[b] : nullptr);
                 hipAssert(hipEventRecord(ev_comp[b], gstream[0]));
@@ -1352,6 +1447,12 @@
         return false;
     }
     impl->cfg = config;
+    impl->head_direct = false;
+    if (plan.elt == 2 && !impl->launches.empty() && impl->final_op >= 0) {
+        const Impl::Launch& L = impl->launches.back();
+        const GemmParams& g = impl->gemm[impl->final_op];
+        impl->head_direct = L.kind == Impl::L_HEAD && L.last == impl->final_op && g.out.Hs == plan.Tout && g.out.Ws == plan.Tout && g.out.x0 == 0 && g.out.y0 == 0;
+    }
     int folds[Impl::L_ATTN32 + 1] = {};
     for (const Impl::Launch& L : impl->launches) ++folds[L.kind];
     W2X_LOG(info, "Loaded \"" + enginePath + "\": " + std::to_string(plan.ops.size()) + " ops, " + std::to_string(plan.B) + " tiles per pass, activation arena " +
@@ -1463,7 +1564,7 @@
     }
     impl->ensure(impl->d_slots, impl->slots_cap, stepTotal * sizeof(TileSlot));
     hipAssert(hipMemcpyAsync(impl->d_slots, impl->h_slots.data(), stepTotal * sizeof(TileSlot), hipMemcpyHostToDevice, stream));
-    impl->upload_live(grid, stepTotal, stream);
+    impl->upload_live(grid, stepTotal, stream, parts == 1 ? rows : 0, parts == 1 ? cols : 0);
     const size_t one_part_steps = (size_t)(((int)std::lround(std::ceil((double)(sp.tile_count * steps) / plan.userB)) + S - 1) / S) * B;
     impl->ensure(impl->d_slab, impl->slab_cap, std::max((size_t)first_of[npart - 1] * steps + (stepTotal - slots_off[npart - 1]), one_part_steps) * plan.Tout * plan.Tout * 4 * plan.elt);
 
@@ -1801,7 +1902,7 @@
     if (grid.count <= 0) { W2X_LOG_AS(who, error, "Tile grid is empty."); return false; }
     for (const Rect& r : grid.out) if (r.w <= 0 || r.h <= 0) { W2X_LOG_AS(who, error, "Tile grid does not fit the output (scaling does not match the model)."); return false; }
     const StripPlan sp = strip_plan(grid, cols * s, plan.Tout, 0, 1);
-    impl->sequence_slots(grid, sp);
+    impl->sequence_slots(grid, sp, resized ? 0 : rows, resized ? 0 : cols);
 
     struct ResizeScope { Img2Img::Impl* e; ~ResizeScope() { e->rs = nullptr; } } resize_scope{impl.get()};
     if (resized) {
diff --git a/waifu2x-tensorrt_amd/csrc/k_mlp96q.hip b/waifu2x-tensorrt_amd/csrc/k_mlp96q.hip
--- a/waifu2x-tensorrt_amd/csrc/k_mlp96q.hip
+++ b/waifu2x-tensorrt_amd/csrc/k_mlp96q.hip
@@ -1,4 +1,5 @@
 #include "kernels.h"
+#include "prepost_device.h"
 #ifndef W2X_GELU_DEG
 #define W2X_GELU_DEG 4
 #endif
@@ -336,6 +337,10 @@
             const int oy0 = ml0 / p.ti_aW, ox0 = ml0 - oy0 * p.ti_aW;
             _Float16* __restrict__ Og = (_Float16*)p.ti_out + (size_t)bimg * p.ti_Hs * p.ti_Ws * 4;
             const half2v lo2 = {(_Float16)p.ti_lo, (_Float16)p.ti_lo}, hi2 = {(_Float16)p.ti_hi, (_Float16)p.ti_hi};
+            const bool dh = p.direct != nullptr;
+            DirectSlot de = {};
+            if (dh) de = direct_slot_load(p.direct, bimg);
+            const __amdgpu_buffer_rsrc_t DB = make_rsrc((const void*)de.base, de.limit);
 #pragma unroll
             for (int th = 0; th < 2; ++th) {
                 half8 wf[2][3];
@@ -363,6 +368,7 @@
                     int ox = ox0 + tt * 16 + fr16, oy = oy0;
                     if (ox >= p.ti_aW) { ox -= p.ti_aW; ++oy; }
                     const bool ok = row0 + tt * 16 + fr16 < p.M;
+                    const bool direct = dh && ok && ox >= (int)de.bx0 && ox < (int)de.bx1 && oy >= (int)de.by0 && oy < (int)de.by1;
 #pragma unroll
                     for (int t = 0; t < 2; ++t) {
                         half2v v01 = {(_Float16)acc[t][tt][0], (_Float16)acc[t][tt][1]}, v23 = {(_Float16)acc[t][tt][2], (_Float16)acc[t][tt][3]};
@@ -371,7 +377,15 @@
                             asm("v_pk_max_f16 %0, %1, %2\n\tv_pk_min_f16 %0, %0, %3" : "=&v"(v23) : "v"(v23), "v"(lo2), "v"(hi2));
                         }
                         const half4 px = {v01[0], v01[1], v23[0], v23[1]};
-                        if (ok) *(half4*)(Og + ((size_t)(oy * 4 + 2 * th + t) * p.ti_Ws + ox * 4 + g4) * 4) = px;
+                        if (dh) {
+                            const unsigned q = quantize_bgr((float)px[0], (float)px[1], (float)px[2]);
+                            const unsigned s16 = (unsigned)__builtin_amdgcn_ds_swizzle((int)q, 0x401F);
+                            const unsigned s48 = __builtin_amdgcn_permlane32_swap(s16, s16, false, false)[1];
+                            const unsigned dw = g4 == 0 ? (q | s16 << 24) : g4 == 1 ? (q >> 8 | s48 << 16) : (q >> 16 | s16 << 8);
+                            const unsigned doff = (unsigned)(oy * 4) * de.step + (unsigned)(ox * 3 + g4) * 4u;
+                            if (direct && g4 < 3) __builtin_amdgcn_raw_buffer_store_b32(dw, DB, doff, (unsigned)(2 * th + t) * de.step, 0);
+                        }
+                        if (ok && !direct) *(half4*)((char*)Og + (unsigned)(((oy * 4 + 2 * th + t) * p.ti_Ws + ox * 4 + g4) * 8)) = px;
                     }
                 }
             }
@@ -399,7 +413,7 @@
 
 }
 
-bool mlp96q_supported(const MlpParams& p) { return p.C == C && p.w1_frag && p.w2_frag && p.frag32 && (!p.ti_w || (p.ti_b && p.ti_out && !p.stats_out && p.ti_Mrows > 0 && p.ti_Mrows % RW == 0 && p.ti_aW >= RW && p.M < 0x7FFFFFFFl &&
+bool mlp96q_supported(const MlpParams& p) { return p.C == C && p.w1_frag && p.w2_frag && p.frag32 && (!p.ti_w || (p.ti_b && p.ti_out && !p.stats_out && p.ti_Mrows > 0 && p.ti_Mrows % RW == 0 && p.ti_aW >= RW && p.M < 0x7FFFFFFFl && (long)p.ti_Hs * p.ti_Ws * 8 < 0x7FFFFFFFl &&
                                                                  (!p.ti_clip || ((float)(_Float16)p.ti_lo == p.ti_lo && (float)(_Float16)p.ti_hi == p.ti_hi)))); }
 
 hipError_t launch_mlp96q(const MlpParams& p, hipStream_t s) {
diff --git a/waifu2x-tensorrt_amd/csrc/k_prepost.hip b/waifu2x-tensorrt_amd/csrc/k_prepost.hip
--- a/waifu2x-tensorrt_amd/csrc/k_prepost.hip
+++ b/waifu2x-tensorrt_amd/csrc/k_prepost.hip
@@ -49,21 +49,14 @@
 #endif
 constexpr int kComposeRows = W2X_COMPOSE_ROWS, kComposeThreads = W2X_COMPOSE_THREADS;
 template <typename P>
-__global__ __launch_bounds__(kComposeThreads) void compose_kernel(const ComposeParams p) {
+__device__ __forceinline__ void compose_group_rows(const ComposeParams& p, const int X, const int np, const int Y0, const int Y1) {
     constexpr bool kHalf = sizeof(P) == 8;
-    const int x1 = p.x1 > 0 ? p.x1 : p.outW, sw = x1 - p.x0;
-    const int gw = (sw + 3) >> 2;
-    const int xg = blockIdx.x * kComposeThreads + threadIdx.x;
-    if (xg >= gw) return;
     const P* tiles = (const P*)p.tiles;
     const int To = p.To, n = To - 1;
-    const int X = p.x0 + 4 * xg;
-    const int np = min(4, x1 - X);
     int a0 = X - To + 1; a0 = a0 <= 0 ? 0 : (a0 + p.stride_x - 1) / p.stride_x;
     int b0 = X + 3 - To + 1; b0 = b0 <= 0 ? 0 : (b0 + p.stride_x - 1) / p.stride_x;
     const int a1 = min(p.nx - 1, X / p.stride_x), b1 = min(p.nx - 1, (X + 3) / p.stride_x);
     const bool fast_col = kHalf && np == 4 && !p.tta && !p.deep && a0 == b0 && a1 == b1;
-    const int Y0 = p.y0 + blockIdx.y * kComposeRows, Y1 = min(p.y1 > 0 ? p.y1 : p.outH, Y0 + kComposeRows);
     for (int Y = Y0; Y < Y1; ++Y) {
         uint8_t* d = p.dst + (size_t)Y * p.dst_step + (size_t)X * 3;
         unsigned px[4] = {0u, 0u, 0u, 0u};
@@ -124,6 +117,29 @@
             }
         }
     }
+}
+template <typename P>
+__global__ __launch_bounds__(kComposeThreads) void compose_kernel(const ComposeParams p) {
+    const int x1 = p.x1 > 0 ? p.x1 : p.outW, sw = x1 - p.x0;
+    const int gw = (sw + 3) >> 2;
+    const int xg = blockIdx.x * kComposeThreads + threadIdx.x;
+    if (xg >= gw) return;
+    const int X = p.x0 + 4 * xg;
+    const int Y0 = p.y0 + blockIdx.y * kComposeRows, Y1 = min(p.y1 > 0 ? p.y1 : p.outH, Y0 + kComposeRows);
+    compose_group_rows<P>(p, X, min(4, x1 - X), Y0, Y1);
+}
+
+__global__ __launch_bounds__(64) void compose_seam_kernel(const ComposeParams p, const SeamRect* __restrict__ rects, int nrect) {
+    const int u = blockIdx.x;
+    int lo = 0, hi = nrect - 1;
+    while (lo < hi) { const int mid = (lo + hi + 1) >> 1; if (rects[mid].unit0 <= u) lo = mid; else hi = mid - 1; }
+    const SeamRect r = rects[lo];
+    const int lu = u - r.unit0, ru = lu / r.cu, cu = lu - ru * r.cu;
+    const int tx = threadIdx.x % r.tw, ty = threadIdx.x / r.tw;
+    const int X = r.x0 + 4 * (cu * r.tw + tx);
+    const int Y0 = r.y0 + (ru * (64 / r.tw) + ty) * kSeamRows;
+    if (X >= r.x1 || Y0 >= r.y1) return;
+    compose_group_rows<half4>(p, X, min(4, r.x1 - X), Y0, min(r.y1, Y0 + kSeamRows));
 }
 
 template <typename P>
@@ -377,6 +393,12 @@
     else hipLaunchKernelGGL(compose_kernel<half4>, grid, dim3(kComposeThreads), 0, s, p);
     return hipGetLastError();
 }
+hipError_t launch_compose_seam(const ComposeParams& p, const SeamRect* rects, int nrect, int units, hipStream_t s) {
+    if (nrect <= 0 || units <= 0) return hipSuccess;
+    if (p.fp32 || p.deep || p.tta || !rects) return hipErrorInvalidValue;
+    hipLaunchKernelGGL(compose_seam_kernel, dim3((unsigned)units), dim3(64), 0, s, p, rects, nrect);
+    return hipGetLastError();
+}
 hipError_t launch_compose_canvas(const ComposeParams& p, float* canvas, hipStream_t s) {
     const int w = (p.x1 > 0 ? p.x1 : p.outW) - p.x0, h = (p.y1 > 0 ? p.y1 : p.outH) - p.y0;
     if (w <= 0 || h <= 0) return hipSuccess;
diff --git a/waifu2x-tensorrt_amd/csrc/kernels.h b/waifu2x-tensorrt_amd/csrc/kernels.h
--- a/waifu2x-tensorrt_amd/csrc/kernels.h
+++ b/waifu2x-tensorrt_amd/csrc/kernels.h
@@ -57,6 +57,26 @@
         left -= x1 - x0; r += x1 - x0;
     }
     return false;
+}
+#endif
+
+struct DirectSlot {
+    unsigned long long base;
+    unsigned step;
+    unsigned short bx0, bx1, by0, by1;
+    unsigned limit;
+    unsigned pad[2];
+};
+static_assert(sizeof(DirectSlot) == 32, "one s_load_dwordx8");
+#ifdef __HIPCC__
+__device__ __forceinline__ DirectSlot direct_slot_load(const DirectSlot* t, int slot) {
+    typedef unsigned uint4c __attribute__((ext_vector_type(4)));
+    typedef const uint4c __attribute__((address_space(4)))* cptr;
+    const uint4c v = ((cptr)(unsigned long long)t)[2 * slot], w = ((cptr)(unsigned long long)t)[2 * slot + 1];
+    DirectSlot e;
+    e.base = (unsigned long long)v[0] | (unsigned long long)v[1] << 32; e.step = v[2];
+    e.bx0 = (unsigned short)v[3]; e.bx1 = (unsigned short)(v[3] >> 16); e.by0 = (unsigned short)w[0]; e.by1 = (unsigned short)(w[0] >> 16); e.limit = w[1];
+    return e;
 }
 #endif
 
@@ -116,6 +136,7 @@
     long ti_row0 = 0;
     const LiveExt* live = nullptr; int live_W = 0, live_H = 0;
     long live_row0 = 0;
+    const DirectSlot* direct = nullptr;
 };
 
 struct SwinAttnParams {
@@ -223,6 +244,9 @@
 hipError_t launch_scale(void* x, const float* scale, int B, int HW, int Cs, bool fp32, hipStream_t s);
 hipError_t launch_gather(const GatherParams& p, hipStream_t s);
 hipError_t launch_compose(const ComposeParams& p, hipStream_t s);
+struct SeamRect { int x0, x1, y0, y1; int tw, cu, unit0, pad; };
+constexpr int kSeamRows = 4;
+hipError_t launch_compose_seam(const ComposeParams& p, const SeamRect* rects, int nrect, int units, hipStream_t s);
 hipError_t launch_compose_canvas(const ComposeParams& p, float* canvas, hipStream_t s);
 struct ResampleParams {
     const float* canvas = nullptr; int inW = 0, inH = 0;
diff --git a/waifu2x-tensorrt_amd/csrc/prepost_device.h b/waifu2x-tensorrt_amd/csrc/prepost_device.h
--- a/waifu2x-tensorrt_amd/csrc/prepost_device.h
+++ b/waifu2x-tensorrt_amd/csrc/prepost_device.h
@@ -2,6 +2,25 @@
 #include "kernels.h"
 
 namespace w2x {
+
+struct BlockSpan { int b0, b1; };
+__host__ __device__ inline BlockSpan direct_span(int To, int stride, int n, int ramp, int out, int i, bool align4) {
+    const int org = i * stride;
+    if (stride <= 0 || To <= 0 || i < 0 || i >= n || org >= out || (align4 && (org & 3))) return BlockSpan{0, 0};
+    int lo = 0;
+    if (i > 0) { lo = To - stride; if (ramp > lo) lo = ramp; if (lo < 0) lo = 0; }
+    const int rw = org + To > out ? out - org : To;
+    int hi = rw;
+    if (i + 1 < n && stride < hi) hi = stride;
+    if (org + rw < out && To - ramp < hi) hi = To - ramp;
+    const int b0 = (lo + 3) >> 2, b1 = hi > 0 ? hi >> 2 : 0;
+    return b1 > b0 ? BlockSpan{b0, b1} : BlockSpan{0, 0};
+}
+__host__ __device__ inline BlockSpan direct_span_px(int To, int stride, int n, int ramp, int out, int i, bool align4, int at) {
+    const BlockSpan b = direct_span(To, stride, n, ramp, out, i, align4);
+    return b.b1 > b.b0 ? BlockSpan{i * stride + 4 * b.b0, i * stride + 4 * b.b1} : BlockSpan{at, at};
+}
+
 namespace {
 
 typedef _Float16 half4 __attribute__((ext_vector_type(4)));
diff --git a/waifu2x-tensorrt_amd/csrc/support.cpp b/waifu2x-tensorrt_amd/csrc/support.cpp
--- a/waifu2x-tensorrt_amd/csrc/support.cpp
+++ b/waifu2x-tensorrt_amd/csrc/support.cpp
@@ -47,6 +47,7 @@
     {"no_stem", nullptr, &Switches::no_stem, nullptr, 0, 1},
     {"attn_valu", nullptr, &Switches::attn_valu, nullptr, 0, 1},
     {"no_dead_skip", nullptr, &Switches::no_dead_skip, nullptr, 0, 1},
+    {"no_direct_head", nullptr, &Switches::no_direct_head, nullptr, 0, 1},
 };
 void assign(Switches& s, const Field& f, long v) {
     v = std::min<long>(f.hi, std::max<long>(f.lo, v));
diff --git a/waifu2x-tensorrt_amd/csrc/switches.h b/waifu2x-tensorrt_amd/csrc/switches.h
--- a/waifu2x-tensorrt_amd/csrc/switches.h
+++ b/waifu2x-tensorrt_amd/csrc/switches.h
@@ -22,6 +22,7 @@
     bool no_pixgemm = false, no_conv3 = false, no_conv3h = false, no_conv48 = false, no_stem = false;
     bool attn_valu = false;
     bool no_dead_skip = false;
+    bool no_direct_head = false;
 };
 
 Switches& switches();
diff --git a/waifu2x-tensorrt_amd/engine.py b/waifu2x-tensorrt_amd/engine.py
--- a/waifu2x-tensorrt_amd/engine.py
+++ b/waifu2x-tensorrt_amd/engine.py
@@ -180,6 +180,7 @@
     L.w2x_version.restype = C.c_char_p
     L.w2x_debug_set.argtypes = [C.c_char_p, C.c_int]; L.w2x_debug_set.restype = C.c_int
     L.w2x_dead_skip_extents.argtypes = [C.c_char_p] + [C.c_int] * 5 + [C.c_double, C.c_double, C.c_int, C.c_int, vp, C.c_int]; L.w2x_dead_skip_extents.restype = C.c_int
+    L.w2x_direct_span.argtypes = [C.c_int] * 7 + [vp, vp]; L.w2x_direct_span.restype = C.c_int
     _lib = L
     return L
 
@@ -189,7 +190,7 @@
     "w2x_render", "w2x_render16", "w2x_infer", "w2x_output_tile_size", "w2x_plan_flops", "w2x_pass_tiles", "w2x_last_render_ms", "w2x_bench_resident", "w2x_resident_output", "w2x_profile_frame", "w2x_op_times",
     "w2x_render_resized", "w2x_render16_resized", "w2x_render_sequence_resized", "w2x_resize_weights",
     "w2x_render_yuv", "w2x_render_sequence_yuv", "w2x_yuv_plane_sizes", "w2x_render_yuv_resized", "w2x_render_sequence_yuv_resized",
-    "w2x_render_rgba", "w2x_alpha_bleed_device", "w2x_alpha_bleed", "w2x_dead_skip_extents",
+    "w2x_render_rgba", "w2x_alpha_bleed_device", "w2x_alpha_bleed", "w2x_dead_skip_extents", "w2x_direct_span",
     "w2x_render_strip", "w2x_strip_plan", "w2x_render_sharded", "w2x_shard_plan", "w2x_shard_compute", "w2x_shard_slab", "w2x_shard_finish", "w2x_ipc_export", "w2x_ipc_open", "w2x_ipc_close", "w2x_render_sequence", "w2x_alloc_host", "w2x_free_host", "w2x_pin_host", "w2x_unpin_host", "w2x_calculate_tiles", "w2x_tile_weights", "w2x_describe_plan", "w2x_describe_plan_precision", "w2x_write_engine_file", "w2x_validate_engine_file", "w2x_device_pci_bus_id", "w2x_sha256_hex", "w2x_version", "w2x_debug_set"]
 
 
@@ -737,6 +738,13 @@
     return [dict(zip(EXTENT_FIELDS, (int(v) for v in row))) for row in out]
 
 
+def direct_span(tile_out, stride, n, ramp, out, index, align4) -> tuple[int, int]:
+    b = np.zeros(2, np.int32)
+    if not lib().w2x_direct_span(int(tile_out), int(stride), int(n), int(ramp), int(out), int(index), int(bool(align4)), b.ctypes.data, b.ctypes.data + 4):
+        raise W2xError("w2x_direct_span failed")
+    return int(b[0]), int(b[1])
+
+
 def write_engine_file(onnx_path, batch, tile, out_path) -> bool:
     return bool(lib().w2x_write_engine_file(os.fsencode(onnx_path), batch, tile, os.fsencode(out_path)))
 
```

Measured after the change: 4675 MPix/s, median of 6. No clear change (+0.7%).
